# BGI-Qingdao/HAST

Hardware: AMD Instinct MI355X
Metric: classified read-bp/sec at k=21, 150bp reads, 200M unique-mers/hap (higher is better)
Workload: dtype u64; 1 GPU; C3 human-trio scale: 200M+200M synthetic 21-mers, 10M barcodes, 150bp reads; k=21, read_len=150, keys_per_hap=200000000, barcodes=10000000, batch_reads=48000000, reads_total=5760000000, minimizer=16, keys=random, collective=none (D2H of counters in timed region), resident_batches=12

## Files before the change

hast_amd/csrc/hast_api.cpp:

```cpp
#include <dlfcn.h>
#include <fcntl.h>
#include <sys/stat.h>
#include <unistd.h>
#include <hip/hip_runtime.h>

#include <algorithm>
#include <chrono>
#include <atomic>
#include <cstdarg>
#include <cstdio>
#include <cstdlib>
#include <cstring>
#include <functional>
#include <map>
#include <mutex>
#include <new>
#include <string>
#include <vector>

#include "../../include/hast.h"
#include "hast_common.h"
#include "hast_device.h"
#include "kc_device.h"
#include "fq_device.h"
#include "hast_internal.h"
#include "worker_pool.h"

using namespace hast;

namespace {

thread_local char g_err[512] = "";

struct Staging {
    uint8_t *h_bases = nullptr, *d_bases = nullptr;
    uint64_t *h_off = nullptr, *d_off = nullptr;
    uint32_t *h_ids = nullptr, *d_ids = nullptr;
    size_t cap_bases = 0, cap_reads = 0;
    hipEvent_t done = nullptr;
    bool in_flight = false;
};

}

struct hast_ctx {
    int device = 0;
    int k = 0;
    int m = 0;
    int n_cu = 256;
    hipStream_t stream = nullptr;
    uint64_t *d_slots = nullptr;
    uint32_t nbuckets = 0;
    unsigned long long *d_counts = nullptr;
    uint32_t *h_errword = nullptr;
    unsigned long long *d_pack = nullptr;
    size_t pack_words = 0;
    size_t n_barcodes = 0;
    bool counts_owned = false;
    uint32_t *d_err = nullptr;
    unsigned long long *d_cnt = nullptr;
    void *d_scratch = nullptr;
    size_t scratch_bytes = 0;
    Staging stage[2];
    unsigned batch_no = 0;
    void *d_seg = nullptr;
    size_t seg_bytes = 0;
    std::vector<hipEvent_t> t_ev;
    size_t t_slots = 0, t_next = 0, t_count = 0;
    uint32_t *d_votes_scratch = nullptr;
    size_t votes_bytes = 0;
    void *d_part = nullptr;
    size_t part_bytes = 0;
    char *sf_h[2] = {nullptr, nullptr}, *sf_d[2] = {nullptr, nullptr};
    hipEvent_t sf_done[2] = {nullptr, nullptr};
    void *d_filter = nullptr;
    size_t filter_bytes = 0;
    FilterGeom fg{};
    bool filter_valid = false;
    bool use_filter = true;
    size_t filter_fallback_bytes = 0;
    bool test_filter_oom = false;
    int filter_m = 0, filter_t = 0, filter_kp = 0;
    int filter_exact = -1;
    int text_acgt_only = 0;
    bool exact_env_off = false;
    bool exact_env_once = false;
    int commit_mode = 0;
    int kernel_geo = 1, kernel_rl = 1;
    size_t tile_lds = 0;
    bool part_oom = false;
};

namespace {

TableGeom geom(const hast_ctx *c) { return TableGeom{c->nbuckets, c->k, c->m, c->k == 32}; }
size_t table_slots(const hast_ctx *c) { return (size_t)c->nbuckets * kSlotsPerBucket * (c->k == 32 ? 2 : 1); }

int default_minimizer_plain(int k) { return k <= 16 ? k : std::max(16, k - 8); }
int default_minimizer(int k) {
    if (const char *e = getenv("HAST_MINIMIZER")) {
        int v = atoi(e);
        if (v >= 1 && v <= k) return v;
    }
    return default_minimizer_plain(k);
}

hast_status use(hast_ctx *c) {
    if (!c) return set_error(HAST_ERR_INVALID, "null context");
    HAST_HIP_TRY(hipSetDevice(c->device));
    return HAST_OK;
}

hast_status ensure_scratch(hast_ctx *c, size_t bytes) {
    if (c->scratch_bytes >= bytes) return HAST_OK;
    if (c->d_scratch) HAST_HIP_TRY(hipFree(c->d_scratch));
    c->d_scratch = nullptr;
    c->scratch_bytes = 0;
    HAST_HIP_TRY(dev_malloc(&c->d_scratch, bytes));
    c->scratch_bytes = bytes;
    return HAST_OK;
}

constexpr size_t kChunkBytes = 64u << 20;

hast_status check_err_word(hast_ctx *c, hipStream_t s) {
    uint32_t e = 0;
    HAST_HIP_TRY(hipMemcpyAsync(&e, c->d_err, sizeof(e), hipMemcpyDeviceToHost, s));
    HAST_HIP_TRY(hipStreamSynchronize(s));
    if (e) HAST_HIP_TRY(hipMemsetAsync(c->d_err, 0, sizeof(uint32_t), s));
    if (e & 2) return set_error(HAST_ERR_FORMAT, "k-mer text: a line is not exactly K=%d bytes", c->k);
    if (e & 4) return set_error(HAST_ERR_FORMAT, "k-mer text: a byte other than upper-case A/C/G/T");
    if (e & 1) return set_error(HAST_ERR_TABLE_FULL, "k-mer table full: reserve more keys");
    return HAST_OK;
}

hast_status check_classify_err(hast_ctx *c, hipStream_t hs) {
    if (!hs) hs = c->stream;
    *c->h_errword = 0;
    HAST_HIP_TRY(hipMemcpyAsync(c->h_errword, c->d_err + 1, sizeof(uint32_t), hipMemcpyDeviceToHost, hs));
    HAST_HIP_TRY(hipStreamSynchronize(hs));
    if (!*c->h_errword) return HAST_OK;
    HAST_HIP_TRY(hipMemsetAsync(c->d_err + 1, 0, sizeof(uint32_t), hs));
    HAST_HIP_TRY(hipStreamSynchronize(hs));
    return set_error(HAST_ERR_INVALID, "read offsets overlap or are not monotonic (their lengths add up to more than bases_bytes): rows were dropped");
}

SynthParams resolve(const hast_synth_params *p) {
    SynthParams r;
    r.seed_k = p->seed_k ? p->seed_k : 0x4841535401ull;
    r.seed_r = p->seed_r ? p->seed_r : 0x4841535402ull;
    r.seed_b = p->seed_b ? p->seed_b : 0x4841535403ull;
    r.n_keys_per_hap = p->n_keys_per_hap;
    r.n_barcodes = p->n_barcodes ? p->n_barcodes : 1;
    r.read_len = p->read_len;
    r.k = p->k;
    r.reserved = p->reserved;
    return r;
}

hast_status check_synth(const hast_synth_params *p) {
    if (!p) return set_error(HAST_ERR_INVALID, "null synth params");
    if (p->k < 1 || p->k > 32) return set_error(HAST_ERR_INVALID, "synth k=%u out of [1,32]", p->k);
    return HAST_OK;
}

}

namespace hast {
hast_status set_error(hast_status st, const char *fmt, ...) {
    va_list ap;
    va_start(ap, fmt);
    vsnprintf(g_err, sizeof(g_err), fmt, ap);
    va_end(ap);
    return st;
}
namespace {
struct Parked {
    std::mutex mu;
    std::vector<void *> device, pinned;
    size_t bytes = 0;
};
Parked &parked() {
    static Parked *p = new Parked();
    return *p;
}
size_t park_limit() {
    static const size_t limit = [] {
        const char *e = getenv("HAST_PARK_GB");
        return (size_t)((e ? atof(e) : 32.0) * 1073741824.0);
    }();
    return limit;
}
int park_sites() {
    static const int sites = [] {
        const char *e = getenv("HAST_PARK_SITES");
        return e ? atoi(e) : -1;
    }();
    return sites;
}
}
size_t parked_bytes() {
    Parked &pk = parked();
    std::lock_guard<std::mutex> lk(pk.mu);
    return pk.bytes;
}
hipError_t dev_malloc(void **p, size_t bytes) {
    hipError_t e = hipMalloc(p, bytes);
    if (e == hipErrorOutOfMemory && parked_bytes()) {
        (void)hipGetLastError();
        release_parked();
        e = hipMalloc(p, bytes);
    }
    return e;
}
hipError_t pinned_malloc(void **p, size_t bytes, unsigned flags) {
    hipError_t e = hipHostMalloc(p, bytes, flags);
    if (e == hipErrorOutOfMemory && parked_bytes()) {
        (void)hipGetLastError();
        release_parked();
        e = hipHostMalloc(p, bytes, flags);
    }
    return e;
}
void release_parked() {
    std::vector<void *> d, h;
    {
        Parked &pk = parked();
        std::lock_guard<std::mutex> lk(pk.mu);
        d.swap(pk.device);
        h.swap(pk.pinned);
        pk.bytes = 0;
    }
    for (void *p : d) (void)hipFree(p);
    for (void *p : h) (void)hipHostFree(p);
}
static void park(void *p, size_t bytes, bool pinned, int site) {
    if (!p) return;
    size_t limit = park_limit();
    if (!((park_sites() >> site) & 1)) limit = 0;
    if (limit == 0) {
        (void)(pinned ? hipHostFree(p) : hipFree(p));
        return;
    }
    bool over = false;
    {
        Parked &pk = parked();
        std::lock_guard<std::mutex> lk(pk.mu);
        (pinned ? pk.pinned : pk.device).push_back(p);
        pk.bytes += bytes;
        over = pk.bytes > limit;
    }
    if (over) release_parked();
}
void park_device(void *p, size_t bytes, int site) { park(p, bytes, false, site); }
void park_pinned(void *p, size_t bytes, int site) { park(p, bytes, true, site); }
int default_minimizer_for(int k) { return default_minimizer(k); }
}

extern "C" {

const char *hast_version(void) { return "hast-mi355x 0.1 (gfx950)"; }
const char *hast_last_error(void) { return g_err; }


hast_status hast_ctx_create(int device, int k, hast_ctx **out) {
    if (!out) return set_error(HAST_ERR_INVALID, "out is null");
    *out = nullptr;
    if (k < 1 || k > 32) return set_error(HAST_ERR_INVALID, "K=%d out of [1,32]", k);
    const bool trace = getenv("HAST_TRACE_INIT") != nullptr;
    auto now_s = [] { return std::chrono::duration<double>(std::chrono::steady_clock::now().time_since_epoch()).count(); };
    double t_tr = now_s();
    auto tr = [&](const char *what) {
        if (trace) fprintf(stderr, "__trace_init__ device %d: %s %.4f s\n", device, what, now_s() - t_tr);
        t_tr = now_s();
    };
    int n = 0;
    hipError_t e = hipGetDeviceCount(&n);
    tr("hipGetDeviceCount (loads the runtime)");
    if (e != hipSuccess || n <= 0)
        return set_error(HAST_ERR_NO_DEVICE, "no HIP device (%s); libhast has no CPU path", hipGetErrorString(e));
    if (device < 0 || device >= n) return set_error(HAST_ERR_NO_DEVICE, "device %d not in [0,%d)", device, n);
    HAST_HIP_TRY(hipSetDevice(device));
    tr("hipSetDevice");
    hast_ctx *c = new (std::nothrow) hast_ctx();
    if (!c) return set_error(HAST_ERR_OOM, "host allocation failed");
    c->device = device;
    c->k = k;
    c->m = default_minimizer(k);
    if (const char *e = getenv("HAST_CLASSIFY")) c->use_filter = strcmp(e, "exact") != 0;
    if (const char *e = getenv("HAST_TEST_FILTER_OOM")) c->test_filter_oom = atoi(e) != 0;
    if (const char *e = getenv("HAST_FILTER_M")) c->filter_m = atoi(e);
    if (const char *e = getenv("HAST_FILTER_T")) c->filter_t = atoi(e);
    if (const char *e = getenv("HAST_FILTER_KP")) c->filter_kp = atoi(e);
    if (const char *e = getenv("HAST_FILTER_EXACT")) {
        if (!strcmp(e, "once")) c->exact_env_once = true;
        else c->exact_env_off = atoi(e) == 0;
    }
    if (c->exact_env_off) c->filter_exact = 0;
    else if (c->exact_env_once) c->filter_exact = 1;
    if (const char *e = getenv("HAST_COMMIT")) c->commit_mode = !strcmp(e, "atomic") ? 1 : !strcmp(e, "partition") ? 2 : 0;
    if (const char *e = getenv("HAST_F_GEO")) c->kernel_geo = e[0] != '0';
    if (const char *e = getenv("HAST_F_RL")) c->kernel_rl = e[0] != '0';
    if (const char *e = getenv("HAST_TILE_LDS")) {
        const long v = atol(e);
        if (v >= 4096 && v <= 160 * 1024) c->tile_lds = (size_t)v;
    }
    hipDeviceProp_t prop;
    if (hipGetDeviceProperties(&prop, device) == hipSuccess) c->n_cu = prop.multiProcessorCount;
    tr("hipGetDeviceProperties");
    hast_status st = HAST_OK;
    auto bail = [&](hipError_t he, const char *what) {
        if (he != hipSuccess && st == HAST_OK) st = set_error(HAST_ERR_HIP, "%s: %s", what, hipGetErrorString(he));
    };
    bail(hipStreamCreateWithFlags(&c->stream, hipStreamNonBlocking), "hipStreamCreate");
    tr("hipStreamCreate");
    bail(dev_malloc(&c->d_err, 4 * sizeof(uint32_t)), "dev_malloc(err)");
    tr("first hipMalloc");
    bail(dev_malloc(&c->d_cnt, 8 * sizeof(unsigned long long)), "dev_malloc(cnt)");
    bail(pinned_malloc(reinterpret_cast<void **>(&c->h_errword), 64, hipHostMallocDefault), "pinned_malloc(err word)");
    if (st == HAST_OK) bail(hipMemsetAsync(c->d_err, 0, 4 * sizeof(uint32_t), c->stream), "hipMemset");
    if (st == HAST_OK) bail(hipStreamSynchronize(c->stream), "hipStreamSynchronize");
    tr("first fill + synchronize");
    for (auto &s : c->stage)
        if (st == HAST_OK) bail(hipEventCreateWithFlags(&s.done, hipEventDisableTiming), "hipEventCreate");
    tr("events");
    if (st != HAST_OK) {
        hast_ctx_destroy(c);
        return st;
    }
    *out = c;
    return HAST_OK;
}

void hast_release_parked(void) { release_parked(); }

void hast_ctx_destroy(hast_ctx *c) {
    if (!c) return;
    (void)hipSetDevice(c->device);
    if (c->stream) (void)hipStreamSynchronize(c->stream);
    release_parked();
    for (auto &s : c->stage) {
        if (s.h_bases) (void)hipHostFree(s.h_bases);
        if (s.h_off) (void)hipHostFree(s.h_off);
        if (s.h_ids) (void)hipHostFree(s.h_ids);
        if (s.d_bases) (void)hipFree(s.d_bases);
        if (s.d_off) (void)hipFree(s.d_off);
        if (s.d_ids) (void)hipFree(s.d_ids);
        if (s.done) (void)hipEventDestroy(s.done);
    }
    if (c->d_slots) (void)hipFree(c->d_slots);
    if (c->counts_owned && c->d_counts) (void)hipFree(c->d_counts);
    if (c->d_pack) (void)hipFree(c->d_pack);
    if (c->h_errword) (void)hipHostFree(c->h_errword);
    if (c->d_err) (void)hipFree(c->d_err);
    if (c->d_cnt) (void)hipFree(c->d_cnt);
    if (c->d_scratch) (void)hipFree(c->d_scratch);
    if (c->d_seg) (void)hipFree(c->d_seg);
    if (c->d_votes_scratch) (void)hipFree(c->d_votes_scratch);
    if (c->d_part) (void)hipFree(c->d_part);
    for (int i = 0; i < 2; ++i) {
        if (c->sf_done[i]) (void)hipEventDestroy(c->sf_done[i]);
        if (c->sf_d[i]) (void)hipFree(c->sf_d[i]);
        if (c->sf_h[i]) (void)hipHostFree(c->sf_h[i]);
    }
    if (c->d_filter) (void)hipFree(c->d_filter);
    for (hipEvent_t e : c->t_ev) (void)hipEventDestroy(e);
    if (c->stream) (void)hipStreamDestroy(c->stream);
    delete c;
}

int hast_ctx_k(const hast_ctx *c) { return c ? c->k : 0; }
int hast_ctx_minimizer(const hast_ctx *c) { return c ? c->m : 0; }

hast_status hast_ctx_set_minimizer(hast_ctx *c, int m) {
    if (!c) return set_error(HAST_ERR_INVALID, "null context");
    if (m < 1 || m > c->k) return set_error(HAST_ERR_INVALID, "minimizer length %d out of [1,%d]", m, c->k);
    if (c->d_slots) return set_error(HAST_ERR_INVALID, "minimizer length is fixed once the table exists");
    c->m = m;
    return HAST_OK;
}
int hast_ctx_device(const hast_ctx *c) { return c ? c->device : -1; }
hast_stream hast_ctx_stream(const hast_ctx *c) { return c ? (hast_stream)c->stream : nullptr; }

hast_status hast_stream_sync(hast_ctx *c, hast_stream s) {
    if (hast_status st = use(c)) return st;
    HAST_HIP_TRY(hipStreamSynchronize(s ? (hipStream_t)s : c->stream));
    return check_classify_err(c, s ? (hipStream_t)s : c->stream);
}

hast_status hast_dev_alloc(hast_ctx *c, size_t bytes, void **d_out) {
    if (hast_status st = use(c)) return st;
    if (!d_out) return set_error(HAST_ERR_INVALID, "d_out is null");
    HAST_HIP_TRY(dev_malloc(d_out, bytes ? bytes : 1));
    return HAST_OK;
}
hast_status hast_dev_free(hast_ctx *c, void *p) {
    if (hast_status st = use(c)) return st;
    if (p) HAST_HIP_TRY(hipFree(p));
    return HAST_OK;
}
hast_status hast_dev_mem_info(hast_ctx *c, size_t *free_bytes, size_t *total_bytes, size_t *parked) {
    if (hast_status st = use(c)) return st;
    size_t f = 0, t = 0;
    HAST_HIP_TRY(hipMemGetInfo(&f, &t));
    if (free_bytes) *free_bytes = f;
    if (total_bytes) *total_bytes = t;
    if (parked) *parked = parked_bytes();
    return HAST_OK;
}
hast_status hast_memcpy_h2d(hast_ctx *c, void *d, const void *s, size_t n) {
    if (hast_status st = use(c)) return st;
    if (n) HAST_HIP_TRY(hipMemcpy(d, s, n, hipMemcpyHostToDevice));
    return HAST_OK;
}
hast_status hast_memcpy_d2h(hast_ctx *c, void *d, const void *s, size_t n) {
    if (hast_status st = use(c)) return st;
    HAST_HIP_TRY(hipStreamSynchronize(c->stream));
    if (n) HAST_HIP_TRY(hipMemcpy(d, s, n, hipMemcpyDeviceToHost));
    return HAST_OK;
}
hast_status hast_memset_d(hast_ctx *c, void *d, int byte, size_t n, hast_stream s) {
    if (hast_status st = use(c)) return st;
    if (n) HAST_HIP_TRY(hipMemsetAsync(d, byte, n, s ? (hipStream_t)s : c->stream));
    return HAST_OK;
}

hast_status hast_table_reserve(hast_ctx *c, uint64_t max_keys, double lf) {
    if (hast_status st = use(c)) return st;
    if (lf <= 0) lf = 0.2;
    if (lf > 0.9) return set_error(HAST_ERR_INVALID, "load factor %.3f > 0.9", lf);
    double want = (double)(max_keys ? max_keys : 1) / lf / kSlotsPerBucket;
    uint64_t nb = (uint64_t)want + 1;
    if (nb < 64) nb = 64;
    nb += nb & 1;
    if (nb >= (1ull << 32)) return set_error(HAST_ERR_INVALID, "table of %llu buckets exceeds 2^32", (unsigned long long)nb);
    HAST_HIP_TRY(hipStreamSynchronize(c->stream));
    if (c->d_slots) HAST_HIP_TRY(hipFree(c->d_slots));
    c->d_slots = nullptr;
    c->nbuckets = 0;
    c->filter_valid = false;
    size_t bytes = (size_t)nb * kSlotsPerBucket * sizeof(uint64_t) * (c->k == 32 ? 2 : 1);
    HAST_HIP_TRY(dev_malloc(&c->d_slots, bytes));
    HAST_HIP_TRY(hipMemsetAsync(c->d_slots, 0xFF, bytes, c->stream));
    HAST_HIP_TRY(hipStreamSynchronize(c->stream));
    c->nbuckets = (uint32_t)nb;
    return HAST_OK;
}

static hast_status ensure_filter(hast_ctx *c, hipStream_t hs);
static void table_changed(hast_ctx *c) { c->filter_valid = false; }

static hast_status need_table(hast_ctx *c, int hap) {
    if (hast_status st = use(c)) return st;
    if (!c->d_slots) return set_error(HAST_ERR_INVALID, "call hast_table_reserve first");
    if (hap != 0 && hap != 1) return set_error(HAST_ERR_INVALID, "hap must be 0 or 1");
    return HAST_OK;
}

hast_status hast_ctx_set_text_check(hast_ctx *c, int acgt_only) {
    if (!c) return set_error(HAST_ERR_INVALID, "null context");
    c->text_acgt_only = acgt_only ? 1 : 0;
    return HAST_OK;
}

hast_status hast_table_insert_keys_device(hast_ctx *c, int hap, const uint64_t *d_keys, size_t n, hast_stream s) {
    if (hast_status st = need_table(c, hap)) return st;
    hipStream_t hs = s ? (hipStream_t)s : c->stream;
    table_changed(c);
    HAST_HIP_TRY(launch_insert_keys(c->d_slots, geom(c), d_keys, n, (uint32_t)hap, c->d_err, hs));
    return check_err_word(c, hs);
}

hast_status hast_table_insert_keys(hast_ctx *c, int hap, const uint64_t *keys, size_t n) {
    if (hast_status st = need_table(c, hap)) return st;
    if (n && !keys) return set_error(HAST_ERR_INVALID, "keys is null");
    table_changed(c);
    const size_t per = kChunkBytes / sizeof(uint64_t);
    if (hast_status st = ensure_scratch(c, std::min(n, per) * sizeof(uint64_t) + 16)) return st;
    for (size_t i = 0; i < n; i += per) {
        size_t m = std::min(per, n - i);
        HAST_HIP_TRY(hipMemcpyAsync(c->d_scratch, keys + i, m * sizeof(uint64_t), hipMemcpyHostToDevice, c->stream));
        HAST_HIP_TRY(launch_insert_keys(c->d_slots, geom(c), (const uint64_t *)c->d_scratch, m, (uint32_t)hap, c->d_err, c->stream));
        HAST_HIP_TRY(hipStreamSynchronize(c->stream));
    }
    return check_err_word(c, c->stream);
}

hast_status hast_table_insert_text(hast_ctx *c, int hap, const char *text, size_t nbytes, uint64_t *lines_out) {
    if (hast_status st = need_table(c, hap)) return st;
    if (lines_out) *lines_out = 0;
    if (nbytes && !text) return set_error(HAST_ERR_INVALID, "text is null");
    table_changed(c);
    const size_t stride = (size_t)c->k + 1;
    size_t n_lines = nbytes / stride;
    size_t rem = nbytes - n_lines * stride;
    if (rem && memchr(text + n_lines * stride, '\n', rem)) return set_error(HAST_ERR_FORMAT, "k-mer text: ragged last line");
    const size_t per = (kChunkBytes / stride);
    if (hast_status st = ensure_scratch(c, std::min(n_lines, per) * stride + 16)) return st;
    for (size_t i = 0; i < n_lines; i += per) {
        size_t m = std::min(per, n_lines - i);
        HAST_HIP_TRY(hipMemcpyAsync(c->d_scratch, text + i * stride, m * stride, hipMemcpyHostToDevice, c->stream));
        HAST_HIP_TRY(launch_insert_text(c->d_slots, geom(c), (const char *)c->d_scratch, m, (uint32_t)hap, c->text_acgt_only, c->d_err, c->stream));
        HAST_HIP_TRY(hipStreamSynchronize(c->stream));
    }
    if (hast_status st = check_err_word(c, c->stream)) return st;
    if (lines_out) *lines_out = n_lines;
    return HAST_OK;
}

static hast_status stream_file_region(hast_ctx *c, int fd, const char *path, uint64_t file_off, uint64_t n_units, size_t unit,
                                      const std::function<hipError_t(char *, size_t, uint64_t)> &use) {
    constexpr size_t kPieceBytes = 16u << 20;
    const uint64_t per = std::max<uint64_t>(1, kPieceBytes / unit);
    char **h_buf = c->sf_h, **d_buf = c->sf_d;
    hipEvent_t *done = c->sf_done;
    hipError_t e = hipSuccess;
    bool short_read = false;
    for (int i = 0; i < 2 && e == hipSuccess; ++i) {
        if (!h_buf[i]) e = pinned_malloc((void **)&h_buf[i], kPieceBytes, hipHostMallocDefault);
        if (e == hipSuccess && !d_buf[i]) e = dev_malloc((void **)&d_buf[i], kPieceBytes + 16);
        if (e == hipSuccess && !done[i]) e = hipEventCreateWithFlags(&done[i], hipEventDisableTiming);
    }
    if (e == hipSuccess) {
        const int nthreads = 8;
        WorkerPool pool(nthreads);
        size_t i = 0;
        for (uint64_t first = 0; first < n_units && e == hipSuccess; first += per, ++i) {
            const int b = (int)(i & 1);
            const size_t m = (size_t)std::min<uint64_t>(per, n_units - first), bytes = m * unit;
            if (i >= 2) e = hipEventSynchronize(done[b]);
            if (e != hipSuccess) break;
            const size_t share = ((bytes / nthreads) + 4095) & ~(size_t)4095;
            std::atomic<bool> bad{false};
            pool.run([&](int t) {
                const size_t from = std::min(bytes, share * (size_t)t), to = std::min(bytes, from + share);
                size_t got = 0;
                while (from + got < to) {
                    const ssize_t r = pread(fd, h_buf[b] + from + got, to - from - got, (off_t)(file_off + first * unit + from + got));
                    if (r <= 0) { bad = true; break; }
                    got += (size_t)r;
                }
            });
            if (bad) { short_read = true; break; }
            e = hipMemcpyAsync(d_buf[b], h_buf[b], bytes, hipMemcpyHostToDevice, c->stream);
            if (e == hipSuccess) e = use(d_buf[b], m, first);
            if (e == hipSuccess) e = hipEventRecord(done[b], c->stream);
        }
        const hipError_t e2 = hipStreamSynchronize(c->stream);
        if (e == hipSuccess) e = e2;
    }
    if (e != hipSuccess) return set_error(HAST_ERR_HIP, "%s: %s", path, hipGetErrorString(e));
    if (short_read) return set_error(HAST_ERR_IO, "%s is shorter than its size says (truncated, or changed while it was read)", path);
    return HAST_OK;
}

hast_status hast_table_insert_text_file(hast_ctx *c, int hap, const char *path, uint64_t *lines_out) {
    if (hast_status st = need_table(c, hap)) return st;
    if (lines_out) *lines_out = 0;
    if (!path) return set_error(HAST_ERR_INVALID, "path is null");
    const int fd = open(path, O_RDONLY);
    if (fd < 0) return set_error(HAST_ERR_IO, "cannot read %s", path);
    struct stat sb;
    if (fstat(fd, &sb) != 0 || !S_ISREG(sb.st_mode)) {
        close(fd);
        return set_error(HAST_ERR_IO, "%s is not a regular file", path);
    }
    const size_t nbytes = (size_t)sb.st_size, stride = (size_t)c->k + 1;
    const size_t n_lines = nbytes / stride, rem = nbytes - n_lines * stride;
    if (rem) {
        char tail[64];
        if (pread(fd, tail, rem, (off_t)(n_lines * stride)) != (ssize_t)rem) { close(fd); return set_error(HAST_ERR_IO, "cannot read %s", path); }
        if (memchr(tail, '\n', rem)) { close(fd); return set_error(HAST_ERR_FORMAT, "k-mer text: ragged last line"); }
    }
    table_changed(c);
    const hast_status st = stream_file_region(c, fd, path, 0, n_lines, stride, [&](char *d_piece, size_t m, uint64_t) {
        return launch_insert_text(c->d_slots, geom(c), d_piece, m, (uint32_t)hap, c->text_acgt_only, c->d_err, c->stream);
    });
    close(fd);
    if (st != HAST_OK) return st;
    if (hast_status s2 = check_err_word(c, c->stream)) return s2;
    if (lines_out) *lines_out = n_lines;
    return HAST_OK;
}

hast_status hast_table_erase(hast_ctx *c, const uint64_t *keys, size_t n, uint8_t *out_hit) {
    if (hast_status st = need_table(c, 0)) return st;
    if (n == 0) return HAST_OK;
    if (!keys) return set_error(HAST_ERR_INVALID, "keys is null");
    size_t kb = n * sizeof(uint64_t);
    if (hast_status st = ensure_scratch(c, kb + n + 16)) return st;
    uint8_t *d_hit = (uint8_t *)c->d_scratch + kb;
    HAST_HIP_TRY(hipMemcpyAsync(c->d_scratch, keys, kb, hipMemcpyHostToDevice, c->stream));
    HAST_HIP_TRY(launch_erase_keys(c->d_slots, geom(c), (const uint64_t *)c->d_scratch, n, d_hit, c->stream));
    table_changed(c);
    std::vector<uint8_t> hit(n);
    HAST_HIP_TRY(hipMemcpyAsync(hit.data(), d_hit, n, hipMemcpyDeviceToHost, c->stream));
    HAST_HIP_TRY(hipStreamSynchronize(c->stream));
    if (out_hit) memcpy(out_hit, hit.data(), n);
    return HAST_OK;
}

hast_status hast_table_lookup(hast_ctx *c, const uint64_t *keys, size_t n, uint8_t *out_tags) {
    if (hast_status st = need_table(c, 0)) return st;
    if (n == 0) return HAST_OK;
    if (!keys || !out_tags) return set_error(HAST_ERR_INVALID, "null argument");
    size_t kb = n * sizeof(uint64_t);
    if (hast_status st = ensure_scratch(c, kb + n + 16)) return st;
    uint8_t *d_tags = (uint8_t *)c->d_scratch + kb;
    HAST_HIP_TRY(hipMemcpyAsync(c->d_scratch, keys, kb, hipMemcpyHostToDevice, c->stream));
    HAST_HIP_TRY(launch_lookup_keys(c->d_slots, geom(c), (const uint64_t *)c->d_scratch, n, d_tags, c->stream));
    HAST_HIP_TRY(hipMemcpyAsync(out_tags, d_tags, n, hipMemcpyDeviceToHost, c->stream));
    HAST_HIP_TRY(hipStreamSynchronize(c->stream));
    return HAST_OK;
}

hast_status hast_table_sizes(hast_ctx *c, uint64_t *n0, uint64_t *n1) {
    if (hast_status st = need_table(c, 0)) return st;
    unsigned long long h[2] = {0, 0};
    HAST_HIP_TRY(hipMemsetAsync(c->d_cnt, 0, sizeof(h), c->stream));
    HAST_HIP_TRY(launch_count_tags(c->d_slots, geom(c), c->d_cnt, c->stream));
    HAST_HIP_TRY(hipMemcpyAsync(h, c->d_cnt, sizeof(h), hipMemcpyDeviceToHost, c->stream));
    HAST_HIP_TRY(hipStreamSynchronize(c->stream));
    if (n0) *n0 = h[0];
    if (n1) *n1 = h[1];
    return HAST_OK;
}

namespace {
struct CacheHeader {
    char magic[8];
    uint32_t version, k;
    uint64_t n_slots;
    uint64_t reserved;
};
}

hast_status hast_table_save(hast_ctx *c, const char *path) {
    if (hast_status st = need_table(c, 0)) return st;
    if (c->k == 32) return set_error(HAST_ERR_INVALID, "the key-set cache stores tag bits next to the key: not available for K=32");
    if (!path) return set_error(HAST_ERR_INVALID, "path is null");
    uint64_t n0 = 0, n1 = 0;
    if (hast_status st = hast_table_sizes(c, &n0, &n1)) return st;
    const size_t cap = (size_t)(n0 + n1) + 16;
    uint64_t *d_out = nullptr;
    HAST_HIP_TRY(dev_malloc((void **)&d_out, cap * sizeof(uint64_t)));
    unsigned long long n = 0;
    hipError_t e = hipMemsetAsync(c->d_cnt, 0, sizeof(unsigned long long), c->stream);
    if (e == hipSuccess) e = launch_export_slots(c->d_slots, (size_t)c->nbuckets * kSlotsPerBucket, d_out, cap, c->d_cnt, c->stream);
    if (e == hipSuccess) e = hipMemcpyAsync(&n, c->d_cnt, sizeof(n), hipMemcpyDeviceToHost, c->stream);
    if (e == hipSuccess) e = hipStreamSynchronize(c->stream);
    std::vector<uint64_t> host;
    if (e == hipSuccess && n <= cap) {
        uint64_t *d_sorted = nullptr;
        void *d_tmp = nullptr;
        size_t tmp_bytes = 0;
        if (n) e = kc_sort_keys(nullptr, &tmp_bytes, (unsigned long long *)d_out, nullptr, (size_t)n, 32, c->stream);
        if (e == hipSuccess && n) e = dev_malloc((void **)&d_sorted, (size_t)n * sizeof(uint64_t));
        if (e == hipSuccess && n) e = dev_malloc(&d_tmp, tmp_bytes ? tmp_bytes : 16);
        if (e == hipSuccess && n) e = kc_sort_keys(d_tmp, &tmp_bytes, (unsigned long long *)d_out, (unsigned long long *)d_sorted, (size_t)n, 32, c->stream);
        if (e == hipSuccess) e = hipStreamSynchronize(c->stream);
        host.resize((size_t)n);
        if (e == hipSuccess && n) e = hipMemcpy(host.data(), d_sorted, (size_t)n * sizeof(uint64_t), hipMemcpyDeviceToHost);
        (void)hipFree(d_sorted);
        (void)hipFree(d_tmp);
    }
    (void)hipFree(d_out);
    if (e != hipSuccess) return set_error(HAST_ERR_HIP, "table export: %s", hipGetErrorString(e));
    if (n > cap) return set_error(HAST_ERR_INVALID, "table export overflow");
    FILE *f = fopen(path, "wb");
    if (!f) return set_error(HAST_ERR_IO, "cannot write %s", path);
    CacheHeader h;
    memcpy(h.magic, "HASTKEYS", 8);
    h.version = 1;
    h.k = (uint32_t)c->k;
    h.n_slots = n;
    h.reserved = 0;
    bool ok = fwrite(&h, sizeof(h), 1, f) == 1 && (n == 0 || fwrite(host.data(), sizeof(uint64_t), (size_t)n, f) == (size_t)n);
    ok = (fclose(f) == 0) && ok;
    if (!ok) return set_error(HAST_ERR_IO, "short write to %s", path);
    return HAST_OK;
}

hast_status hast_table_file_info(const char *path, int *k_out, uint64_t *n_keys_out) {
    if (!path) return set_error(HAST_ERR_INVALID, "path is null");
    FILE *f = fopen(path, "rb");
    if (!f) return set_error(HAST_ERR_IO, "cannot read %s", path);
    CacheHeader h;
    const bool ok = fread(&h, sizeof(h), 1, f) == 1 && memcmp(h.magic, "HASTKEYS", 8) == 0 && h.version == 1;
    fclose(f);
    if (!ok) return set_error(HAST_ERR_FORMAT, "%s is not a HASTKEYS v1 file", path);
    if (k_out) *k_out = (int)h.k;
    if (n_keys_out) *n_keys_out = h.n_slots;
    return HAST_OK;
}

hast_status hast_table_load(hast_ctx *c, const char *path, double load_factor) {
    if (hast_status st = use(c)) return st;
    if (!path) return set_error(HAST_ERR_INVALID, "path is null");
    FILE *f = fopen(path, "rb");
    if (!f) return set_error(HAST_ERR_IO, "cannot read %s", path);
    CacheHeader h;
    if (fread(&h, sizeof(h), 1, f) != 1 || memcmp(h.magic, "HASTKEYS", 8) != 0 || h.version != 1) {
        fclose(f);
        return set_error(HAST_ERR_FORMAT, "%s is not a HASTKEYS v1 file", path);
    }
    if (h.k == 32 || (int)h.k != c->k) {
        fclose(f);
        return set_error(HAST_ERR_INVALID, "%s holds %u-mers, the context is K=%d", path, h.k, c->k);
    }
    hast_status st = hast_table_reserve(c, h.n_slots + 1, load_factor);
    struct stat sb;
    if (st == HAST_OK && fstat(fileno(f), &sb) == 0 && S_ISREG(sb.st_mode)) {
        st = stream_file_region(c, fileno(f), path, sizeof(CacheHeader), h.n_slots, sizeof(uint64_t), [&](char *d_piece, size_t m, uint64_t) {
            return launch_import_slots(c->d_slots, geom(c), (const uint64_t *)d_piece, m, c->d_err, c->stream);
        });
        if (st == HAST_ERR_IO) st = set_error(HAST_ERR_IO, "%s is truncated", path);
    } else {
        const size_t per = kChunkBytes / sizeof(uint64_t);
        std::vector<uint64_t> buf(std::min<uint64_t>(per, h.n_slots ? h.n_slots : 1));
        if (st == HAST_OK) st = ensure_scratch(c, buf.size() * sizeof(uint64_t) + 16);
        for (uint64_t i = 0; st == HAST_OK && i < h.n_slots; i += per) {
            const size_t m = (size_t)std::min<uint64_t>(per, h.n_slots - i);
            if (fread(buf.data(), sizeof(uint64_t), m, f) != m) { st = set_error(HAST_ERR_IO, "%s is truncated", path); break; }
            hipError_t e = hipMemcpyAsync(c->d_scratch, buf.data(), m * sizeof(uint64_t), hipMemcpyHostToDevice, c->stream);
            if (e == hipSuccess) e = launch_import_slots(c->d_slots, geom(c), (const uint64_t *)c->d_scratch, m, c->d_err, c->stream);
            if (e == hipSuccess) e = hipStreamSynchronize(c->stream);
            if (e != hipSuccess) st = set_error(HAST_ERR_HIP, "table import: %s", hipGetErrorString(e));
        }
    }
    fclose(f);
    if (st != HAST_OK) return st;
    return check_err_word(c, c->stream);
}

hast_status hast_table_clone(hast_ctx *dst, hast_ctx *src) {
    if (!dst || !src || dst == src) return set_error(HAST_ERR_INVALID, "clone needs two different contexts");
    if (dst->k != src->k) return set_error(HAST_ERR_INVALID, "clone: K differs (%d vs %d)", dst->k, src->k);
    if (hast_status st = need_table(src, 0)) return st;
    if (src->use_filter)
        if (hast_status st = ensure_filter(src, src->stream)) return st;
    HAST_HIP_TRY(hipStreamSynchronize(src->stream));
    if (hast_status st = use(dst)) return st;
    HAST_HIP_TRY(hipStreamSynchronize(dst->stream));
    if (dst->d_slots) HAST_HIP_TRY(hipFree(dst->d_slots));
    dst->d_slots = nullptr;
    dst->nbuckets = 0;
    dst->filter_valid = false;
    dst->m = src->m;
    const size_t bytes = table_slots(src) * sizeof(uint64_t);
    HAST_HIP_TRY(dev_malloc(&dst->d_slots, bytes));
    HAST_HIP_TRY(hipMemcpyPeerAsync(dst->d_slots, dst->device, src->d_slots, src->device, bytes, dst->stream));
    dst->nbuckets = src->nbuckets;
    if (src->filter_valid && dst->use_filter) {
        if (dst->filter_bytes != src->filter_bytes) {
            if (dst->d_filter) HAST_HIP_TRY(hipFree(dst->d_filter));
            dst->d_filter = nullptr;
            dst->filter_bytes = 0;
            if (dst->test_filter_oom || dev_malloc(&dst->d_filter, src->filter_bytes) != hipSuccess) {
                (void)hipGetLastError();
                dst->d_filter = nullptr;
                dst->use_filter = false;
                dst->filter_fallback_bytes = src->filter_bytes;
                HAST_HIP_TRY(hipStreamSynchronize(dst->stream));
                return HAST_OK;
            }
            dst->filter_bytes = src->filter_bytes;
        }
        HAST_HIP_TRY(hipMemcpyPeerAsync(dst->d_filter, dst->device, src->d_filter, src->device, src->filter_bytes, dst->stream));
        dst->fg = src->fg;
        dst->filter_m = src->filter_m;
        dst->filter_exact = src->filter_exact;
        dst->filter_t = src->filter_t;
        dst->filter_kp = src->filter_kp;
        dst->filter_valid = true;
    }
    HAST_HIP_TRY(hipStreamSynchronize(dst->stream));
    return HAST_OK;
}

hast_status hast_table_info(const hast_ctx *c, uint64_t *n_buckets, uint64_t *bytes) {
    if (!c) return set_error(HAST_ERR_INVALID, "null context");
    if (n_buckets) *n_buckets = c->nbuckets;
    if (bytes) *bytes = (uint64_t)table_slots(c) * sizeof(uint64_t);
    return HAST_OK;
}

hast_status hast_counts_resize(hast_ctx *c, size_t n) {
    if (hast_status st = use(c)) return st;
    HAST_HIP_TRY(hipStreamSynchronize(c->stream));
    if (c->counts_owned && c->d_counts) HAST_HIP_TRY(hipFree(c->d_counts));
    c->d_counts = nullptr;
    c->n_barcodes = 0;
    c->counts_owned = false;
    size_t bytes = (n ? n : 1) * 4 * sizeof(unsigned long long);
    HAST_HIP_TRY(dev_malloc(reinterpret_cast<void **>(&c->d_counts), bytes));
    c->counts_owned = true;
    c->n_barcodes = n;
    HAST_HIP_TRY(hipMemsetAsync(c->d_counts, 0, bytes, c->stream));
    HAST_HIP_TRY(hipStreamSynchronize(c->stream));
    return HAST_OK;
}

hast_status hast_counts_permute(hast_ctx *c, const uint32_t *perm, size_t n_perm, size_t n_new) {
    if (hast_status st = use(c)) return st;
    if (!c->d_counts || !c->counts_owned) return set_error(HAST_ERR_INVALID, "hast_counts_permute: library-owned counters only (hast_counts_resize)");
    if (n_perm > c->n_barcodes || (n_perm && !perm)) return set_error(HAST_ERR_INVALID, "hast_counts_permute: %zu ids > %zu counters", n_perm, c->n_barcodes);
    for (size_t i = 0; i < n_perm; i++)
        if (perm[i] >= n_new && perm[i] != 0xFFFFFFFFu) return set_error(HAST_ERR_INVALID, "hast_counts_permute: perm[%zu] = %u is outside the %zu new records", i, perm[i], n_new);
    HAST_HIP_TRY(hipStreamSynchronize(c->stream));
    unsigned long long *d_new = nullptr;
    uint32_t *d_perm = nullptr;
    const size_t bytes = (n_new ? n_new : 1) * 4 * sizeof(unsigned long long);
    HAST_HIP_TRY(dev_malloc(reinterpret_cast<void **>(&d_new), bytes));
    hipError_t e = dev_malloc(reinterpret_cast<void **>(&d_perm), (n_perm ? n_perm : 1) * sizeof(uint32_t));
    if (e == hipSuccess) e = hipMemsetAsync(d_new, 0, bytes, c->stream);
    if (e == hipSuccess && n_perm) e = hipMemcpyAsync(d_perm, perm, n_perm * sizeof(uint32_t), hipMemcpyHostToDevice, c->stream);
    if (e == hipSuccess) e = launch_counts_permute(d_new, c->d_counts, d_perm, n_perm, c->n_barcodes, n_new, c->stream);
    if (e == hipSuccess) e = hipStreamSynchronize(c->stream);
    if (d_perm) (void)hipFree(d_perm);
    if (e != hipSuccess) {
        (void)hipFree(d_new);
        return set_error(e == hipErrorOutOfMemory ? HAST_ERR_OOM : HAST_ERR_HIP, "hast_counts_permute: %s", hipGetErrorString(e));
    }
    HAST_HIP_TRY(hipFree(c->d_counts));
    c->d_counts = d_new;
    c->n_barcodes = n_new;
    return HAST_OK;
}

hast_status hast_counts_bind(hast_ctx *c, uint64_t *d_counts, size_t n) {
    if (hast_status st = use(c)) return st;
    if (!d_counts) return set_error(HAST_ERR_INVALID, "d_counts is null");
    if ((uintptr_t)d_counts & 31) return set_error(HAST_ERR_INVALID, "d_counts must be 32-byte aligned (one record = 4 x u64)");
    HAST_HIP_TRY(hipStreamSynchronize(c->stream));
    if (c->counts_owned && c->d_counts) HAST_HIP_TRY(hipFree(c->d_counts));
    c->d_counts = reinterpret_cast<unsigned long long *>(d_counts);
    c->counts_owned = false;
    c->n_barcodes = n;
    return HAST_OK;
}

hast_status hast_counts_zero(hast_ctx *c, hast_stream s) {
    if (hast_status st = use(c)) return st;
    if (!c->d_counts) return set_error(HAST_ERR_INVALID, "no counters: call hast_counts_resize/bind");
    HAST_HIP_TRY(hipMemsetAsync(c->d_counts, 0, c->n_barcodes * 4 * sizeof(unsigned long long), s ? (hipStream_t)s : c->stream));
    return HAST_OK;
}

static hast_status ensure_pack(hast_ctx *c, size_t n) {
    if (c->pack_words >= 3 * n) return HAST_OK;
    if (c->d_pack) HAST_HIP_TRY(hipFree(c->d_pack));
    c->d_pack = nullptr;
    c->pack_words = 0;
    HAST_HIP_TRY(dev_malloc((void **)&c->d_pack, std::max<size_t>(3 * n, 1) * sizeof(unsigned long long)));
    c->pack_words = 3 * n;
    return HAST_OK;
}

hast_status hast_counts_pack(hast_ctx *c, uint64_t *d_packed, size_t n, hast_stream s) {
    if (hast_status st = use(c)) return st;
    if (!c->d_counts || !d_packed) return set_error(HAST_ERR_INVALID, "no counters");
    if (n > c->n_barcodes) return set_error(HAST_ERR_INVALID, "n_barcodes %zu > %zu", n, c->n_barcodes);
    HAST_HIP_TRY(launch_counts_pack(c->d_counts, reinterpret_cast<unsigned long long *>(d_packed), n, s ? (hipStream_t)s : c->stream));
    return HAST_OK;
}
hast_status hast_counts_unpack(hast_ctx *c, const uint64_t *d_packed, size_t n, hast_stream s) {
    if (hast_status st = use(c)) return st;
    if (!c->d_counts || !d_packed) return set_error(HAST_ERR_INVALID, "no counters");
    if (n > c->n_barcodes) return set_error(HAST_ERR_INVALID, "n_barcodes %zu > %zu", n, c->n_barcodes);
    HAST_HIP_TRY(launch_counts_unpack(c->d_counts, reinterpret_cast<const unsigned long long *>(d_packed), n, s ? (hipStream_t)s : c->stream));
    return HAST_OK;
}

hast_status hast_counts_read_range(hast_ctx *c, size_t first, size_t n, uint64_t *c0, uint64_t *c1, uint64_t *neg) {
    if (hast_status st = use(c)) return st;
    if (!c->d_counts) return set_error(HAST_ERR_INVALID, "no counters");
    if (first > c->n_barcodes || n > c->n_barcodes - first) return set_error(HAST_ERR_INVALID, "records [%zu, %zu) of %zu counters", first, first + n, c->n_barcodes);
    HAST_HIP_TRY(hipStreamSynchronize(c->stream));
    if (hast_status st = check_classify_err(c, c->stream)) return st;
    if (!n) return HAST_OK;
    if (hast_status st = ensure_pack(c, n)) return st;
    HAST_HIP_TRY(launch_counts_pack(c->d_counts + 4 * first, c->d_pack, n, c->stream));
    uint64_t *dst[3] = {c0, c1, neg};
    for (int a = 0; a < 3; a++)
        if (dst[a]) HAST_HIP_TRY(hipMemcpyAsync(dst[a], c->d_pack + (size_t)a * n, n * sizeof(uint64_t), hipMemcpyDeviceToHost, c->stream));
    HAST_HIP_TRY(hipStreamSynchronize(c->stream));
    return HAST_OK;
}
hast_status hast_counts_read(hast_ctx *c, uint64_t *c0, uint64_t *c1, uint64_t *neg, size_t n) { return hast_counts_read_range(c, 0, n, c0, c1, neg); }

hast_status hast_counts_allreduce(hast_ctx *const *ctxs, int n) {
    if (!ctxs || n < 1) return set_error(HAST_ERR_INVALID, "no contexts");
    for (int i = 0; i < n; i++)
        if (!ctxs[i] || !ctxs[i]->d_counts || ctxs[i]->n_barcodes != ctxs[0]->n_barcodes) return set_error(HAST_ERR_INVALID, "contexts need equal-size counters");
    const size_t nbc = ctxs[0]->n_barcodes, nw = nbc * 4;
    std::vector<hast_ctx *> lead;
    std::vector<std::vector<hast_ctx *>> members;
    for (int i = 0; i < n; i++) {
        size_t l = 0;
        while (l < lead.size() && lead[l]->device != ctxs[i]->device) ++l;
        if (l == lead.size()) {
            lead.push_back(ctxs[i]);
            members.emplace_back();
        } else {
            for (hast_ctx *m : members[l]) if (m == ctxs[i]) return set_error(HAST_ERR_INVALID, "hast_counts_allreduce: a context is named twice");
            if (lead[l] == ctxs[i]) return set_error(HAST_ERR_INVALID, "hast_counts_allreduce: a context is named twice");
            members[l].push_back(ctxs[i]);
        }
    }
    for (size_t l = 0; l < lead.size(); l++) {
        if (members[l].empty()) continue;
        if (hast_status st = use(lead[l])) return st;
        HAST_HIP_TRY(hipStreamSynchronize(lead[l]->stream));
        for (hast_ctx *m : members[l]) HAST_HIP_TRY(hipStreamSynchronize(m->stream));
        for (hast_ctx *m : members[l]) HAST_HIP_TRY(launch_add_u64(lead[l]->d_counts, m->d_counts, nw, lead[l]->stream));
    }
    auto hand_back = [&]() -> hast_status {
        for (size_t l = 0; l < lead.size(); l++) {
            if (members[l].empty()) continue;
            if (hast_status st = use(lead[l])) return st;
            for (hast_ctx *m : members[l])
                HAST_HIP_TRY(hipMemcpyAsync(m->d_counts, lead[l]->d_counts, nw * sizeof(unsigned long long), hipMemcpyDeviceToDevice, lead[l]->stream));
            HAST_HIP_TRY(hipStreamSynchronize(lead[l]->stream));
        }
        return HAST_OK;
    };
    const int nl = (int)lead.size();
    if (nl == 1 && !getenv("HAST_FORCE_RCCL")) return hand_back();
    typedef void *comm_t;
    typedef int (*init_all_t)(comm_t *, int, const int *);
    typedef int (*allreduce_t)(const void *, void *, size_t, int, int, comm_t, hipStream_t);
    typedef int (*group_t)(void);
    typedef int (*destroy_t)(comm_t);
    static void *lib = nullptr;
    if (!lib) lib = dlopen("librccl.so.1", RTLD_NOW | RTLD_GLOBAL);
    if (!lib) lib = dlopen("librccl.so", RTLD_NOW | RTLD_GLOBAL);
    if (!lib) return set_error(HAST_ERR_RCCL, "cannot load librccl: %s", dlerror());
    auto init_all = (init_all_t)dlsym(lib, "ncclCommInitAll");
    auto allreduce = (allreduce_t)dlsym(lib, "ncclAllReduce");
    auto gstart = (group_t)dlsym(lib, "ncclGroupStart");
    auto gend = (group_t)dlsym(lib, "ncclGroupEnd");
    auto destroy = (destroy_t)dlsym(lib, "ncclCommDestroy");
    if (!init_all || !allreduce || !gstart || !gend || !destroy) return set_error(HAST_ERR_RCCL, "librccl lacks symbols");
    std::vector<int> devs(nl);
    for (int i = 0; i < nl; i++) devs[i] = lead[(size_t)i]->device;
    static std::mutex comm_mu;
    static std::map<std::vector<int>, std::vector<comm_t>> comm_cache;
    std::lock_guard<std::mutex> lock(comm_mu);
    auto it = comm_cache.find(devs);
    if (it == comm_cache.end()) {
        std::vector<comm_t> fresh(nl);
        if (int rc = init_all(fresh.data(), nl, devs.data())) return set_error(HAST_ERR_RCCL, "ncclCommInitAll failed (%d)", rc);
        it = comm_cache.emplace(devs, std::move(fresh)).first;
    }
    const std::vector<comm_t> &comms = it->second;
    const int kUint64 = 5, kSum = 0;
    for (int i = 0; i < nl; i++) {
        hast_ctx *c = lead[(size_t)i];
        if (hast_status st = use(c)) return st;
        if (hast_status st = ensure_pack(c, nbc)) return st;
        HAST_HIP_TRY(launch_counts_pack(c->d_counts, c->d_pack, nbc, c->stream));
    }
    int rc = gstart();
    for (int i = 0; i < nl && !rc; i++) {
        hast_ctx *c = lead[(size_t)i];
        (void)hipSetDevice(c->device);
        rc = allreduce(c->d_pack, c->d_pack, nbc * 3, kUint64, kSum, comms[(size_t)i], c->stream);
    }
    int rc2 = gend();
    for (int i = 0; i < nl; i++) {
        hast_ctx *c = lead[(size_t)i];
        (void)hipSetDevice(c->device);
        if (!rc && !rc2 && launch_counts_unpack(c->d_counts, c->d_pack, nbc, c->stream) != hipSuccess) rc2 = -1;
        (void)hipStreamSynchronize(c->stream);
    }
    if (rc || rc2) {
        for (auto cm : comms) destroy(cm);
        comm_cache.erase(it);
    }
    if (rc || rc2) return set_error(HAST_ERR_RCCL, "ncclAllReduce failed (%d/%d)", rc, rc2);
    return hand_back();
}

static hast_status ensure_filter(hast_ctx *c, hipStream_t hs) {
    if (c->filter_valid) return HAST_OK;
    unsigned long long h[2] = {0, 0};
    HAST_HIP_TRY(hipMemsetAsync(c->d_cnt, 0, sizeof(h), hs));
    HAST_HIP_TRY(launch_count_tags(c->d_slots, geom(c), c->d_cnt, hs));
    HAST_HIP_TRY(hipMemcpyAsync(h, c->d_cnt, sizeof(h), hipMemcpyDeviceToHost, hs));
    HAST_HIP_TRY(hipStreamSynchronize(hs));
    FilterGeom fg = filter_geom_for(c->k, h[0] + h[1], c->filter_m, c->filter_t, c->filter_kp, c->k == 32 ? 0 : c->filter_exact);
    size_t bytes = (size_t)filter_nblocks(fg) * 128;
    if (bytes != c->filter_bytes) {
        if (c->d_filter) HAST_HIP_TRY(hipFree(c->d_filter));
        c->d_filter = nullptr;
        c->filter_bytes = 0;
        hipError_t got = c->test_filter_oom ? hipErrorOutOfMemory : dev_malloc(&c->d_filter, bytes);
        if (got != hipSuccess && !c->filter_m && fg.m == kFilterMaxM) {
            (void)hipGetLastError();
            fg = filter_geom_for(c->k, h[0] + h[1], kFilterMaxM - 1, c->filter_t, c->filter_kp, c->k == 32 ? 0 : c->filter_exact);
            bytes = (size_t)filter_nblocks(fg) * 128;
            got = dev_malloc(&c->d_filter, bytes);
        }
        if (got != hipSuccess) {
            (void)hipGetLastError();
            c->d_filter = nullptr;
            c->use_filter = false;
            c->filter_fallback_bytes = bytes;
            return HAST_OK;
        }
        c->filter_bytes = bytes;
    }
    HAST_HIP_TRY(hipMemsetAsync(c->d_filter, 0, bytes, hs));
    HAST_HIP_TRY(launch_filter_build(c->d_slots, geom(c), c->d_filter, fg, hs));
    c->fg = fg;
    c->filter_valid = true;
    return HAST_OK;
}

static constexpr uint32_t kSegWindows = 482;
static constexpr uint32_t kLongRead = 4096;

static hast_status commit_votes(hast_ctx *c, const uint32_t *d_votes, const uint32_t *d_ids, size_t n_reads, uint32_t max_votes,
                                bool atomic_only, hipStream_t hs) {
    const int mode = c->commit_mode;
    if (mode != 1 && !atomic_only && !c->part_oom && commit_partition_usable(n_reads, c->n_barcodes, max_votes, mode == 2)) {
        const size_t need = commit_partition_scratch_bytes(n_reads, c->n_barcodes, nullptr, nullptr);
        if (c->part_bytes < need) {
            HAST_HIP_TRY(hipStreamSynchronize(hs));
            if (c->d_part) HAST_HIP_TRY(hipFree(c->d_part));
            c->d_part = nullptr;
            c->part_bytes = 0;
            if (dev_malloc(&c->d_part, need + need / 8) == hipSuccess) c->part_bytes = need + need / 8;
            else {
                (void)hipGetLastError();
                c->d_part = nullptr;
                c->part_oom = true;
            }
        }
        if (c->d_part) {
            HAST_HIP_TRY(launch_commit_partitioned(d_votes, d_ids, c->d_counts, c->n_barcodes, n_reads, c->d_part, hs));
            return HAST_OK;
        }
    }
    HAST_HIP_TRY(launch_commit_votes(d_votes, d_ids, c->d_counts, nullptr, n_reads, hs));
    return HAST_OK;
}

static hast_status classify_rows(hast_ctx *c, const uint8_t *d_bases, size_t bases_bytes, const uint64_t *d_offsets,
                                 const uint32_t *d_lens, const uint32_t *d_seg_read, int strict, uint32_t read_len,
                                 const uint32_t *d_barcode_ids, uint32_t *d_votes, size_t n_reads, hast_stream s,
                                 const unsigned long long *d_n_rows = nullptr) {
    if (hast_status st = need_table(c, 0)) return st;
    if (n_reads == 0) return HAST_OK;
    if (!d_bases) return set_error(HAST_ERR_INVALID, "d_bases is null");
    if (d_barcode_ids && !c->d_counts) return set_error(HAST_ERR_INVALID, "barcode ids given but no counters bound");
    if (read_len == 0 || read_len > (1u << 24)) return set_error(HAST_ERR_INVALID, "read_len %u out of range", read_len);
    if (read_len > kLongRead && c->use_filter) return set_error(HAST_ERR_INVALID, "internal: a row of %u bases reached the filter kernel", read_len);
    if (!d_offsets && (uint64_t)n_reads * read_len > bases_bytes)
        return set_error(HAST_ERR_INVALID, "bases_bytes too small for %zu reads of %u", n_reads, read_len);
    ClassifyArgs a;
    a.bases = d_bases;
    a.bases_bytes = bases_bytes;
    a.offsets = d_offsets;
    a.lens = d_lens;
    a.seg_read = d_seg_read;
    a.strict = strict;
    if (reinterpret_cast<uintptr_t>(d_votes) & 7) return set_error(HAST_ERR_INVALID, "d_votes must be 8-byte aligned (a row is stored as one 64-bit word)");
    uint32_t *votes_buf = d_votes;
    if (d_barcode_ids && !votes_buf) {
        const size_t need = n_reads * 2 * sizeof(uint32_t);
        if (c->votes_bytes < need) {
            HAST_HIP_TRY(hipStreamSynchronize(s ? (hipStream_t)s : c->stream));
            if (c->d_votes_scratch) HAST_HIP_TRY(hipFree(c->d_votes_scratch));
            c->d_votes_scratch = nullptr;
            c->votes_bytes = 0;
            HAST_HIP_TRY(dev_malloc(reinterpret_cast<void **>(&c->d_votes_scratch), need + need / 8));
            c->votes_bytes = need + need / 8;
        }
        votes_buf = c->d_votes_scratch;
    }
    a.votes = votes_buf;
    a.slots = c->d_slots;
    a.n_reads = n_reads;
    a.n_rows_ptr = d_n_rows;
    a.nbuckets = c->nbuckets;
    a.read_len = read_len;
    a.k = c->k;
    a.wide = c->k == 32;
    a.m = c->m;
    a.max_pos = read_len >= (uint32_t)c->k ? read_len - c->k + 1 : 0;
    a.mh_stride = read_len >= (uint32_t)c->m ? read_len - c->m + 1 : 0;
    a.w64 = (read_len + 31) / 32;
    hipStream_t hs = s ? (hipStream_t)s : c->stream;
    if (c->use_filter)
        if (hast_status st = ensure_filter(c, hs)) return st;
    const bool filt = c->use_filter;
    size_t per_read, pad;
    if (filt) {
        a.filter = c->d_filter;
        a.fg = c->fg;
        a.l1_stride = c->fg.dense ? 0 : ((read_len >= (uint32_t)c->fg.t ? read_len - (uint32_t)c->fg.t + 1 : 0) + 1 + 3) & ~3u;
        per_read = (size_t)(a.w64 + 1) * 8 + 8 + 8 + 4 + 4 + (size_t)a.l1_stride * 4 + (strict ? (size_t)(2 * a.w64 + 1) * 4 : 0);
        pad = 16 + classify_f_queue_bytes() + 64 * 4 + 64;
    } else {
        const uint32_t wlen = (uint32_t)(c->k - c->m + 1);
        a.filter = nullptr;
        a.fg = FilterGeom{};
        a.l1_stride = 0;
        per_read = (size_t)(a.w64 + 1) * 8 + 8 + 8 + 4 + 4 + (size_t)a.mh_stride * 4 + (strict ? (size_t)(2 * a.w64 + 1) * 4 : 0);
        pad = (size_t)wlen * 4 + 64 + 64 + 16;
    }
    const size_t lds_budget = c->tile_lds ? c->tile_lds : (filt ? (size_t)32000 - (size_t)kTmerLevelTableWords * 4 : (size_t)19968);
    const uint32_t tr_max = (uint32_t)std::min<size_t>(64, std::max<size_t>(1, lds_budget > pad + per_read ? (lds_budget - pad) / per_read : 1));
    uint32_t tr = tr_max;
    if (a.max_pos > 0) {
        double best = -1;
        for (uint32_t t = tr_max; t >= 1 && t + 8 > tr_max; --t) {
            const uint64_t q = (uint64_t)t * a.max_pos, blocks = (q + 63) / 64, slots = filt ? (blocks + 3) / 4 * 4 : (blocks + 7) / 8 * 8;
            const double eff = (double)q / (double)(slots * 64);
            if (eff > best + 1e-9) { best = eff; tr = t; }
        }
    }
    a.tile_reads = tr;
    const size_t smem = per_read * tr + pad;
    if (smem + (filt ? (size_t)kTmerLevelTableWords * 4 : 0) > (160u << 10)) return set_error(HAST_ERR_INVALID, "read_len %u needs %zu B of LDS", read_len, smem);
    auto magic = [](uint64_t qmax, uint32_t d) -> uint32_t {
        if (d <= 1 || qmax * d >= (1ull << 32)) return 0;
        return (uint32_t)((1ull << 32) / d) + 1;
    };
    a.div_magic = magic((uint64_t)tr * a.max_pos + 1024, a.max_pos);
    a.div_mh = magic((uint64_t)tr * a.mh_stride + 1024, a.mh_stride);
    a.div_hw = magic((uint64_t)tr * a.w64 * 2 + 1024, a.w64 * 2);
    a.div_l1g = magic((uint64_t)tr * (a.l1_stride / 4) + 1024, a.l1_stride / 4);
    const uint64_t n_tiles = (n_reads + tr - 1) / tr;
    const int grid = (int)std::min<uint64_t>(n_tiles, (uint64_t)c->n_cu * 8);
    a.tile_queue = c->d_cnt + 3;
    HAST_HIP_TRY(hipMemsetAsync(a.tile_queue, 0, sizeof(unsigned long long), hs));
    hipEvent_t *ev = c->t_slots ? &c->t_ev[3 * (c->t_next % c->t_slots)] : nullptr;
    if (ev) HAST_HIP_TRY(hipEventRecord(ev[0], hs));
    HAST_HIP_TRY(filt ? launch_classify_f(a, grid, smem, (c->kernel_geo ? 1 : 0) | (c->kernel_rl ? 2 : 0), hs) : launch_classify(a, grid, smem, hs));
    if (ev) HAST_HIP_TRY(hipEventRecord(ev[1], hs));
    if (d_barcode_ids) {
        if (hast_status st = commit_votes(c, votes_buf, d_barcode_ids, n_reads, a.max_pos, d_seg_read != nullptr, hs)) return st;
    }
    if (ev) {
        HAST_HIP_TRY(hipEventRecord(ev[2], hs));
        c->t_next++;
        c->t_count = std::min(c->t_count + 1, c->t_slots);
    }
    return HAST_OK;
}

static hast_status classify_segmented(hast_ctx *c, const uint8_t *d_bases, size_t bases_bytes, const uint64_t *d_offsets, const uint32_t *d_lens,
                                      uint32_t fixed_len, size_t n_reads, int strict, const uint32_t *d_barcode_ids, uint32_t *d_votes_out,
                                      hipStream_t hs);

hast_status hast_ctx_set_filter(hast_ctx *c, int enable, int m, int t, int kp) {
    if (!c) return set_error(HAST_ERR_INVALID, "null context");
    if (m < 0 || m > c->k || m > kFilterMaxM) return set_error(HAST_ERR_INVALID, "filter m=%d out of [0,%d]", m, std::min(c->k, kFilterMaxM));
    if (t < 0 || (m && t > m)) return set_error(HAST_ERR_INVALID, "filter t=%d out of [0,m]", t);
    if (kp < 0 || kp > c->k || (kp && m && (kp < m || kp - m >= 32))) return set_error(HAST_ERR_INVALID, "filter kp=%d out of [m,K]", kp);
    c->use_filter = enable != 0;
    c->filter_fallback_bytes = 0;
    c->filter_exact = (enable == 2 || c->exact_env_off) ? 0 : (c->exact_env_once || c->filter_exact == 1) ? 1 : -1;
    c->filter_m = m;
    c->filter_t = t;
    c->filter_kp = kp;
    c->filter_valid = false;
    return HAST_OK;
}

hast_status hast_ctx_set_option(hast_ctx *c, const char *name, long value) {
    if (!c || !name) return set_error(HAST_ERR_INVALID, "null argument");
    if (!strcmp(name, "commit")) {
        if (value < 0 || value > 2) return set_error(HAST_ERR_INVALID, "commit: 0 = by batch size, 1 = atomic, 2 = partitioned");
        c->commit_mode = (int)value;
    } else if (!strcmp(name, "kernel_geo")) c->kernel_geo = value != 0;
    else if (!strcmp(name, "kernel_rl")) c->kernel_rl = value != 0;
    else if (!strcmp(name, "tile_lds")) {
        if (value && (value < 4096 || value > 160 * 1024)) return set_error(HAST_ERR_INVALID, "tile_lds %ld out of [4096, 163840]", value);
        c->tile_lds = (size_t)value;
    } else if (!strcmp(name, "filter_exact_once")) {
        if (c->filter_exact != 0) c->filter_exact = value ? 1 : (c->exact_env_once ? 1 : -1);
        c->filter_valid = false;
    } else return set_error(HAST_ERR_INVALID, "unknown option %s", name);
    return HAST_OK;
}
hast_status hast_ctx_options(const hast_ctx *c, char *out, size_t cap) {
    if (!c || !out || !cap) return set_error(HAST_ERR_INVALID, "null argument");
    std::string s;
    auto add = [&](const char *n, long v) { s += (s.empty() ? "" : " "); s += n; s += "=" + std::to_string(v); };
    if (!c->use_filter) add("filter", 0);
    if (c->filter_fallback_bytes) add("filter_fallback_table_only_no_room_for_bytes", (long)c->filter_fallback_bytes);
    if (c->filter_exact == 0) add("filter_exact", 0);
    if (c->filter_exact == 1) add("filter_exact_once", 1);
    if (c->filter_m) add("filter_m", c->filter_m);
    if (c->filter_t) add("filter_t", c->filter_t);
    if (c->filter_kp) add("filter_kp", c->filter_kp);
    if (c->commit_mode) add("commit", c->commit_mode);
    if (!c->kernel_geo) add("kernel_geo", 0);
    if (!c->kernel_rl) add("kernel_rl", 0);
    if (c->tile_lds) add("tile_lds", (long)c->tile_lds);
    if (c->m != default_minimizer_plain(c->k)) add("minimizer", c->m);
    snprintf(out, cap, "%s", s.c_str());
    return HAST_OK;
}

hast_status hast_filter_build(hast_ctx *c) {
    if (hast_status st = need_table(c, 0)) return st;
    if (!c->use_filter) return HAST_OK;
    if (hast_status st = ensure_filter(c, c->stream)) return st;
    HAST_HIP_TRY(hipStreamSynchronize(c->stream));
    return HAST_OK;
}

hast_status hast_filter_info(const hast_ctx *c, int *enabled, int *m, int *t, int *kp, uint64_t *bytes) {
    if (!c) return set_error(HAST_ERR_INVALID, "null context");
    if (enabled) *enabled = !c->use_filter ? 0 : (c->filter_valid && c->fg.exact) ? 2 : 1;
    if (m) *m = c->filter_valid ? c->fg.m : 0;
    if (t) *t = c->filter_valid ? c->fg.t : 0;
    if (kp) *kp = c->filter_valid ? c->fg.kp : 0;
    if (bytes) *bytes = c->filter_valid ? c->filter_bytes : 0;
    return HAST_OK;
}

hast_status hast_filter_dense(const hast_ctx *c, int *dense) {
    if (!c || !dense) return set_error(HAST_ERR_INVALID, "null argument");
    *dense = (c->use_filter && c->filter_valid && c->fg.dense) ? 1 : 0;
    return HAST_OK;
}

hast_status hast_filter_request_ceiling(hast_ctx *c, double *requests_per_s) {
    if (hast_status st = need_table(c, 0)) return st;
    if (!requests_per_s) return set_error(HAST_ERR_INVALID, "null argument");
    if (!c->use_filter) return set_error(HAST_ERR_INVALID, "the filter is off");
    if (hast_status st = ensure_filter(c, c->stream)) return st;
    if (!c->use_filter || !c->d_filter) return set_error(HAST_ERR_INVALID, "no filter (HBM too small for it)");
    const uint64_t nblocks = filter_nblocks(c->fg);
    const int grid = c->n_cu * 8;
    const uint32_t iters = 256;
    uint32_t *d_sink = reinterpret_cast<uint32_t *>(c->d_cnt + 2);
    hipEvent_t e0 = nullptr, e1 = nullptr;
    hipError_t e = hipEventCreate(&e0);
    if (e == hipSuccess) e = hipEventCreate(&e1);
    float best = 0;
    for (int rep = 0; rep < 3 && e == hipSuccess; ++rep) {
        e = hipEventRecord(e0, c->stream);
        if (e == hipSuccess) e = launch_request_ceiling(c->d_filter, nblocks, iters, grid, d_sink, c->stream);
        if (e == hipSuccess) e = hipEventRecord(e1, c->stream);
        if (e == hipSuccess) e = hipEventSynchronize(e1);
        float ms = 0;
        if (e == hipSuccess) e = hipEventElapsedTime(&ms, e0, e1);
        if (e == hipSuccess && rep && (best == 0 || ms < best)) best = ms;
    }
    if (e0) (void)hipEventDestroy(e0);
    if (e1) (void)hipEventDestroy(e1);
    if (e != hipSuccess) return set_error(HAST_ERR_HIP, "request ceiling: %s", hipGetErrorString(e));
    *requests_per_s = (double)grid * 32.0 * 4.0 * (double)iters / ((double)best * 1e-3);
    return HAST_OK;
}

hast_status hast_classify_timing(hast_ctx *c, int n_slots) {
    if (hast_status st = use(c)) return st;
    for (hipEvent_t e : c->t_ev) (void)hipEventDestroy(e);
    c->t_ev.clear();
    c->t_slots = c->t_next = c->t_count = 0;
    if (n_slots <= 0) return HAST_OK;
    c->t_ev.resize(3 * (size_t)n_slots);
    for (hipEvent_t &e : c->t_ev) HAST_HIP_TRY(hipEventCreate(&e));
    c->t_slots = (size_t)n_slots;
    return HAST_OK;
}
hast_status hast_classify_times(hast_ctx *c, float *classify_ms, float *commit_ms, int max, int *n_out) {
    if (hast_status st = use(c)) return st;
    if (!n_out || (max > 0 && (!classify_ms || !commit_ms))) return set_error(HAST_ERR_INVALID, "null argument");
    int n = 0;
    const size_t first = c->t_next - c->t_count;
    for (size_t i = 0; i < c->t_count && n < max; ++i, ++n) {
        hipEvent_t *ev = &c->t_ev[3 * ((first + i) % c->t_slots)];
        HAST_HIP_TRY(hipEventSynchronize(ev[2]));
        HAST_HIP_TRY(hipEventElapsedTime(&classify_ms[n], ev[0], ev[1]));
        HAST_HIP_TRY(hipEventElapsedTime(&commit_ms[n], ev[1], ev[2]));
    }
    *n_out = n;
    c->t_count = 0;
    return HAST_OK;
}

hast_status hast_classify_device(hast_ctx *c, const uint8_t *d_bases, size_t bases_bytes, const uint64_t *d_offsets,
                                 uint32_t read_len, const uint32_t *d_barcode_ids, uint32_t *d_votes, size_t n_reads,
                                 hast_stream s) {
    if (read_len > kLongRead && c && c->d_slots && n_reads) {
        if (d_barcode_ids && !c->d_counts) return set_error(HAST_ERR_INVALID, "barcode ids given but no counters bound");
        if (!d_bases) return set_error(HAST_ERR_INVALID, "d_bases is null");
        if (!d_offsets && (uint64_t)n_reads * read_len > bases_bytes)
            return set_error(HAST_ERR_INVALID, "bases_bytes too small for %zu reads of %u", n_reads, read_len);
        if (hast_status st = use(c)) return st;
        return classify_segmented(c, d_bases, bases_bytes, d_offsets, nullptr, read_len, n_reads, 0, d_barcode_ids, d_votes, s ? (hipStream_t)s : c->stream);
    }
    return classify_rows(c, d_bases, bases_bytes, d_offsets, nullptr, nullptr, 0, read_len, d_barcode_ids, d_votes, n_reads, s);
}

hast_status hast_counts_add_votes(hast_ctx *c, const uint32_t *d_votes, const uint32_t *d_barcode_ids, size_t n_reads, uint32_t max_votes,
                                  hast_stream s) {
    if (hast_status st = use(c)) return st;
    if (!c->d_counts) return set_error(HAST_ERR_INVALID, "no counters: call hast_counts_resize/bind");
    if (n_reads == 0) return HAST_OK;
    if (!d_votes || !d_barcode_ids) return set_error(HAST_ERR_INVALID, "null argument");
    if (reinterpret_cast<uintptr_t>(d_votes) & 7) return set_error(HAST_ERR_INVALID, "d_votes must be 8-byte aligned");
    return commit_votes(c, d_votes, d_barcode_ids, n_reads, max_votes, false, s ? (hipStream_t)s : c->stream);
}

static hast_status classify_segmented(hast_ctx *c, const uint8_t *d_bases, size_t bases_bytes, const uint64_t *d_offsets, const uint32_t *d_lens,
                                      uint32_t fixed_len, size_t n_reads, int strict, const uint32_t *d_barcode_ids, uint32_t *d_votes_out,
                                      hipStream_t hs) {
    const size_t max_seg = n_reads + bases_bytes / kSegWindows + 1;
    const size_t votes_b = ((n_reads * 2 * sizeof(uint32_t) + 255) & ~(size_t)255), flags_b = ((n_reads + 255) & ~(size_t)255);
    const size_t need = max_seg * (sizeof(uint64_t) + 2 * sizeof(uint32_t)) + votes_b + flags_b + 256;
    if (c->seg_bytes < need) {
        HAST_HIP_TRY(hipStreamSynchronize(hs));
        if (c->d_seg) HAST_HIP_TRY(hipFree(c->d_seg));
        c->d_seg = nullptr;
        c->seg_bytes = 0;
        HAST_HIP_TRY(dev_malloc(&c->d_seg, need + need / 4));
        c->seg_bytes = need + need / 4;
    }
    uint32_t *acc = (uint32_t *)c->d_seg;
    uint8_t *has_n = (uint8_t *)c->d_seg + votes_b;
    const size_t cap = (c->seg_bytes - votes_b - flags_b - 256) / (sizeof(uint64_t) + 2 * sizeof(uint32_t));
    uint64_t *seg_off = (uint64_t *)((uint8_t *)c->d_seg + votes_b + flags_b);
    uint32_t *seg_len = (uint32_t *)(seg_off + cap);
    uint32_t *seg_read = seg_len + cap;
    uint32_t *target = strict ? d_votes_out : acc;
    unsigned long long *d_nseg = c->d_cnt + 4;
    HAST_HIP_TRY(hipMemsetAsync(d_nseg, 0, sizeof(unsigned long long), hs));
    HAST_HIP_TRY(hipMemsetAsync(target, 0, n_reads * 2 * sizeof(uint32_t), hs));
    if (!strict) HAST_HIP_TRY(launch_scan_n(d_bases, d_offsets, d_lens, fixed_len, n_reads, has_n, hs));
    HAST_HIP_TRY(launch_build_segments(d_offsets, d_lens, fixed_len, n_reads, c->k, kSegWindows, seg_off, seg_len, seg_read, d_nseg,
                                  strict ? nullptr : has_n, (uint64_t)max_seg, (uint64_t)bases_bytes, c->d_err + 1, hs));
    if (max_seg > cap) return set_error(HAST_ERR_INVALID, "segment table too small (%zu > %zu)", max_seg, cap);
    if (hast_status st = classify_rows(c, d_bases, bases_bytes, seg_off, seg_len, seg_read, strict, kSegWindows + (uint32_t)c->k - 1,
                                       nullptr, target, max_seg, hs, d_nseg))
        return st;
    if (!strict) HAST_HIP_TRY(launch_commit_votes(acc, d_barcode_ids, c->d_counts, d_votes_out, n_reads, hs));
    return HAST_OK;
}

hast_status hast_classify_perread_device(hast_ctx *c, const uint8_t *d_bases, size_t bases_bytes, const uint64_t *d_offsets,
                                         size_t n_reads, uint32_t *d_votes, hast_stream s) {
    if (hast_status st = need_table(c, 0)) return st;
    if (n_reads == 0) return HAST_OK;
    if (!d_bases || !d_offsets || !d_votes) return set_error(HAST_ERR_INVALID, "null argument");
    return classify_segmented(c, d_bases, bases_bytes, d_offsets, nullptr, 0, n_reads, 1, nullptr, d_votes, s ? (hipStream_t)s : c->stream);
}

hast_status hast_classify_perread(hast_ctx *c, const uint8_t *bases, const uint64_t *offsets, size_t n_reads,
                                  uint32_t *votes_out) {
    if (hast_status st = need_table(c, 0)) return st;
    if (n_reads == 0) return HAST_OK;
    if (!bases || !offsets || !votes_out) return set_error(HAST_ERR_INVALID, "null argument");
    const size_t nbytes = offsets[n_reads] - offsets[0];
    const size_t ob = (n_reads + 1) * sizeof(uint64_t), vb = n_reads * 2 * sizeof(uint32_t);
    const size_t total = ((nbytes + 255) & ~(size_t)255) + ((ob + 255) & ~(size_t)255) + vb + 256;
    if (hast_status st = ensure_scratch(c, total)) return st;
    uint8_t *d_b = (uint8_t *)c->d_scratch;
    uint64_t *d_o = (uint64_t *)(d_b + ((nbytes + 255) & ~(size_t)255));
    uint32_t *d_v = (uint32_t *)((uint8_t *)d_o + ((ob + 255) & ~(size_t)255));
    std::vector<uint64_t> rel(n_reads + 1);
    for (size_t i = 0; i <= n_reads; i++) rel[i] = offsets[i] - offsets[0];
    if (nbytes) HAST_HIP_TRY(hipMemcpyAsync(d_b, bases + offsets[0], nbytes, hipMemcpyHostToDevice, c->stream));
    HAST_HIP_TRY(hipMemcpyAsync(d_o, rel.data(), ob, hipMemcpyHostToDevice, c->stream));
    HAST_HIP_TRY(hipStreamSynchronize(c->stream));
    if (hast_status st = hast_classify_perread_device(c, d_b, nbytes ? nbytes : 1, d_o, n_reads, d_v, c->stream)) return st;
    HAST_HIP_TRY(hipMemcpyAsync(votes_out, d_v, vb, hipMemcpyDeviceToHost, c->stream));
    HAST_HIP_TRY(hipStreamSynchronize(c->stream));
    return check_classify_err(c, c->stream);
}

static hast_status stage_reserve(hast_ctx *c, Staging &s, size_t nbytes, size_t nreads) {
    (void)c;
    if (s.cap_bases < nbytes) {
        if (s.h_bases) HAST_HIP_TRY(hipHostFree(s.h_bases));
        if (s.d_bases) HAST_HIP_TRY(hipFree(s.d_bases));
        s.h_bases = s.d_bases = nullptr;
        s.cap_bases = 0;
        size_t cap = nbytes + nbytes / 4 + 64;
        HAST_HIP_TRY(pinned_malloc((void **)&s.h_bases, cap, hipHostMallocDefault));
        HAST_HIP_TRY(dev_malloc((void **)&s.d_bases, cap));
        s.cap_bases = cap;
    }
    if (s.cap_reads < nreads) {
        if (s.h_off) HAST_HIP_TRY(hipHostFree(s.h_off));
        if (s.h_ids) HAST_HIP_TRY(hipHostFree(s.h_ids));
        if (s.d_off) HAST_HIP_TRY(hipFree(s.d_off));
        if (s.d_ids) HAST_HIP_TRY(hipFree(s.d_ids));
        s.h_off = s.d_off = nullptr;
        s.h_ids = s.d_ids = nullptr;
        s.cap_reads = 0;
        size_t cap = nreads + nreads / 4 + 16;
        HAST_HIP_TRY(pinned_malloc((void **)&s.h_off, (cap + 1) * sizeof(uint64_t), hipHostMallocDefault));
        HAST_HIP_TRY(pinned_malloc((void **)&s.h_ids, cap * sizeof(uint32_t), hipHostMallocDefault));
        HAST_HIP_TRY(dev_malloc((void **)&s.d_off, (cap + 1) * sizeof(uint64_t)));
        HAST_HIP_TRY(dev_malloc((void **)&s.d_ids, cap * sizeof(uint32_t)));
        s.cap_reads = cap;
    }
    return HAST_OK;
}

hast_status hast_batch_begin(hast_ctx *c, size_t bases_capacity, size_t reads_capacity, uint8_t **bases,
                             uint64_t **offsets, uint32_t **ids) {
    if (hast_status st = need_table(c, 0)) return st;
    if (!bases || !offsets || !ids) return set_error(HAST_ERR_INVALID, "null argument");
    if (!c->d_counts) return set_error(HAST_ERR_INVALID, "no counters bound");
    Staging &s = c->stage[c->batch_no & 1];
    if (s.in_flight) {
        HAST_HIP_TRY(hipEventSynchronize(s.done));
        s.in_flight = false;
    }
    if (hast_status st = stage_reserve(c, s, bases_capacity, reads_capacity)) return st;
    *bases = s.h_bases;
    *offsets = s.h_off;
    *ids = s.h_ids;
    return HAST_OK;
}

hast_status hast_batch_submit(hast_ctx *c, size_t n_reads, uint32_t max_read_len) {
    if (hast_status st = need_table(c, 0)) return st;
    Staging &s = c->stage[c->batch_no & 1];
    if (n_reads == 0) return HAST_OK;
    if (n_reads > s.cap_reads) return set_error(HAST_ERR_INVALID, "batch of %zu reads exceeds the staged capacity", n_reads);
    const size_t nbytes = s.h_off[n_reads];
    if (nbytes > s.cap_bases || s.h_off[0] != 0) return set_error(HAST_ERR_INVALID, "bad staged offsets");
    c->batch_no++;
    if (nbytes) HAST_HIP_TRY(hipMemcpyAsync(s.d_bases, s.h_bases, nbytes, hipMemcpyHostToDevice, c->stream));
    HAST_HIP_TRY(hipMemcpyAsync(s.d_off, s.h_off, (n_reads + 1) * sizeof(uint64_t), hipMemcpyHostToDevice, c->stream));
    HAST_HIP_TRY(hipMemcpyAsync(s.d_ids, s.h_ids, n_reads * sizeof(uint32_t), hipMemcpyHostToDevice, c->stream));
    hast_status st = hast_classify_device(c, s.d_bases, nbytes ? nbytes : 1, s.d_off, max_read_len ? max_read_len : 1, s.d_ids,
                                          nullptr, n_reads, c->stream);
    HAST_HIP_TRY(hipEventRecord(s.done, c->stream));
    s.in_flight = true;
    return st;
}

hast_status hast_classify_batch(hast_ctx *c, const uint8_t *bases, const uint64_t *offsets, const uint32_t *ids,
                                size_t n_reads, uint32_t max_read_len) {
    if (n_reads == 0) return c ? HAST_OK : set_error(HAST_ERR_INVALID, "null context");
    if (!bases || !offsets || !ids) return set_error(HAST_ERR_INVALID, "null argument");
    const size_t nbytes = offsets[n_reads] - offsets[0];
    uint8_t *hb;
    uint64_t *ho;
    uint32_t *hi;
    if (hast_status st = hast_batch_begin(c, nbytes, n_reads, &hb, &ho, &hi)) return st;
    memcpy(hb, bases + offsets[0], nbytes);
    const uint64_t o0 = offsets[0];
    for (size_t i = 0; i <= n_reads; i++) ho[i] = offsets[i] - o0;
    memcpy(hi, ids, n_reads * sizeof(uint32_t));
    return hast_batch_submit(c, n_reads, max_read_len);
}

}

namespace hast {
hast_status classify_framed(hast_ctx *c, const uint8_t *d_buf, size_t buf_bytes, const uint64_t *d_off, const uint32_t *d_len, uint32_t max_len,
                            uint32_t *d_votes, size_t n_reads, hipStream_t hs) {
    if (hast_status st = need_table(c, 0)) return st;
    if (n_reads == 0) return HAST_OK;
    if (max_len > kLongRead) return classify_segmented(c, d_buf, buf_bytes, d_off, d_len, 0, n_reads, 0, nullptr, d_votes, hs);
    return classify_rows(c, d_buf, buf_bytes, d_off, d_len, nullptr, 0, max_len ? max_len : 1, nullptr, d_votes, n_reads, hs);
}
hast_status commit_framed(hast_ctx *c, const uint32_t *d_votes, const uint32_t *d_ids, size_t n_reads, hipStream_t hs) {
    if (hast_status st = use(c)) return st;
    if (!c->d_counts) return set_error(HAST_ERR_INVALID, "no counters bound");
    HAST_HIP_TRY(launch_commit_votes(d_votes, d_ids, c->d_counts, nullptr, n_reads, hs));
    return HAST_OK;
}
hipStream_t ctx_stream_of(hast_ctx *c) { return c->stream; }
size_t ctx_n_barcodes(const hast_ctx *c) { return c->n_barcodes; }
}

extern "C" {

void hast_parse_barcode(const char *head, size_t len, size_t *start, size_t *n) {
    ptrdiff_t s = -1, e = -1;
    for (size_t i = 0; i < len; i++) {
        if (head[i] == '#') s = (ptrdiff_t)i;
        else if (head[i] == '/') e = (ptrdiff_t)i;
    }
    size_t pos = (size_t)(s + 1);
    size_t avail = len - pos;
    ptrdiff_t cnt = e - s - 1;
    *start = pos;
    *n = (cnt < 0 || (size_t)cnt > avail) ? avail : (size_t)cnt;
}

int hast_get_hap(const char *bc, size_t blen, uint64_t c0, uint64_t c1, uint64_t n0, uint64_t n1, double w0, double w1) {
    if ((blen == 5 && !memcmp(bc, "0_0_0", 5)) || (blen == 3 && !memcmp(bc, "0_0", 3)) || (blen == 1 && bc[0] == '0'))
        return -1;
    if (c0 > 0 && c1 > 0) {
        double df0 = double(c0) / double(n0);
        double df1 = double(c1) / double(n1);
        df0 *= w0;
        df1 *= w1;
        if (df0 > df1) return 0;
        if (df1 > df0) return 1;
        return -1;
    }
    if (c0 > 0) return 0;
    if (c1 > 0) return 1;
    return -1;
}

uint64_t hast_canon_kmer(const char *s, int k) { return kmer_canon(kmer_pack(s, k), k); }

size_t hast_chop_read(const char *seq, size_t len, int k, uint64_t *out) {
    if (k < 1 || k > 32 || len < (size_t)k) return 0;
    const uint64_t mask = kmer_mask(k);
    uint64_t w = kmer_pack(seq, k);
    size_t n = 0;
    out[n++] = kmer_canon(w, k);
    for (size_t i = (size_t)k; i < len; i++) {
        w = ((w << 2) & mask) | base_code((uint8_t)seq[i]);
        out[n++] = kmer_canon(w, k);
    }
    return n;
}

void hast_kmer_to_str(uint64_t kmer, int k, char *out) {
    for (int i = 0; i < k; i++) {
        out[k - 1 - i] = "ACTG"[kmer & 3];
        kmer >>= 2;
    }
    out[k] = 0;
}

hast_status hast_synth_keys_host(const hast_synth_params *p, int hap, uint64_t first, size_t n, uint64_t *out) {
    if (hast_status st = check_synth(p)) return st;
    SynthParams sp = resolve(p);
    for (size_t i = 0; i < n; i++) out[i] = synth_key(sp, hap, first + i);
    return HAST_OK;
}

hast_status hast_synth_reads_host(const hast_synth_params *p, uint64_t first, size_t n, uint8_t *bases, uint32_t *ids) {
    if (hast_status st = check_synth(p)) return st;
    SynthParams sp = resolve(p);
    if (sp.read_len == 0) return set_error(HAST_ERR_INVALID, "read_len is 0");
    for (size_t i = 0; i < n; i++) {
        uint32_t bc;
        synth_read(sp, first + i, bases + i * (size_t)sp.read_len, &bc);
        if (ids) ids[i] = bc;
    }
    return HAST_OK;
}

hast_status hast_synth_keys_device(hast_ctx *c, const hast_synth_params *p, int hap, uint64_t first, size_t n,
                                   uint64_t *d_out, hast_stream s) {
    if (hast_status st = use(c)) return st;
    if (hast_status st = check_synth(p)) return st;
    HAST_HIP_TRY(launch_synth_keys(resolve(p), hap, first, n, d_out, s ? (hipStream_t)s : c->stream));
    return HAST_OK;
}

hast_status hast_synth_reads_device(hast_ctx *c, const hast_synth_params *p, uint64_t first, size_t n, uint8_t *d_bases,
                                    uint32_t *d_ids, hast_stream s) {
    if (hast_status st = use(c)) return st;
    if (hast_status st = check_synth(p)) return st;
    if (p->read_len == 0) return set_error(HAST_ERR_INVALID, "read_len is 0");
    HAST_HIP_TRY(launch_synth_reads(resolve(p), first, n, d_bases, d_ids, s ? (hipStream_t)s : c->stream));
    return HAST_OK;
}

hast_status hast_synth_table_build(hast_ctx *c, const hast_synth_params *p) {
    if (hast_status st = need_table(c, 0)) return st;
    if (hast_status st = check_synth(p)) return st;
    if ((int)p->k != c->k) return set_error(HAST_ERR_INVALID, "synth k=%u != context K=%d", p->k, c->k);
    table_changed(c);
    SynthParams sp = resolve(p);
    const size_t per = kChunkBytes / sizeof(uint64_t);
    if (hast_status st = ensure_scratch(c, std::min<uint64_t>(sp.n_keys_per_hap, per) * sizeof(uint64_t) + 16)) return st;
    for (int hap = 0; hap < 2; hap++)
        for (uint64_t i = 0; i < sp.n_keys_per_hap; i += per) {
            size_t m = (size_t)std::min<uint64_t>(per, sp.n_keys_per_hap - i);
            HAST_HIP_TRY(launch_synth_keys(sp, hap, i, m, (uint64_t *)c->d_scratch, c->stream));
            HAST_HIP_TRY(launch_insert_keys(c->d_slots, geom(c), (const uint64_t *)c->d_scratch, m, (uint32_t)hap, c->d_err, c->stream));
        }
    return check_err_word(c, c->stream);
}

}
```

hast_amd/csrc/hast_device.h:

```cpp
#pragma once
#include <hip/hip_runtime.h>
#include <stddef.h>
#include <stdint.h>
#include "hast_common.h"

namespace hast {

struct TableGeom {
    uint32_t nbuckets;
    int k;
    int m;
    int wide;
};

struct ClassifyArgs {
    const uint8_t *bases;
    uint64_t bases_bytes;
    const uint64_t *offsets;
    const uint32_t *lens;
    const uint32_t *seg_read;
    uint32_t *votes;
    unsigned long long *tile_queue;
    const uint64_t *slots;
    uint64_t n_reads;
    const unsigned long long *n_rows_ptr;
    uint32_t nbuckets;
    uint32_t read_len;
    uint32_t max_pos;
    uint32_t w64;
    uint32_t tile_reads;
    uint32_t div_magic;
    uint32_t mh_stride;
    uint32_t div_mh;
    uint32_t div_hw;
    int k;
    int m;
    int wide;
    int strict;
    const void *filter;
    FilterGeom fg;
    uint32_t l1_stride;
    uint32_t div_l1g;
};

hipError_t launch_insert_keys(uint64_t *slots, TableGeom g, const uint64_t *d_keys, size_t n, uint32_t hap,
                              uint32_t *d_err, hipStream_t s);
hipError_t launch_insert_text(uint64_t *slots, TableGeom g, const char *d_text, size_t n_lines,
                              uint32_t hap, int acgt_only, uint32_t *d_err, hipStream_t s);
hipError_t launch_erase_keys(uint64_t *slots, TableGeom g, const uint64_t *d_keys, size_t n, uint8_t *d_hit, hipStream_t s);
hipError_t launch_lookup_keys(uint64_t *slots, TableGeom g, const uint64_t *d_keys, size_t n, uint8_t *d_tags, hipStream_t s);
hipError_t launch_export_slots(const uint64_t *slots, size_t nslots, uint64_t *d_out, size_t cap, unsigned long long *d_counter, hipStream_t s);
hipError_t launch_import_slots(uint64_t *slots, TableGeom g, const uint64_t *d_in, size_t n, uint32_t *d_err, hipStream_t s);
hipError_t launch_count_tags(const uint64_t *slots, TableGeom g, unsigned long long *d_out, hipStream_t s);
hipError_t launch_classify(const ClassifyArgs &a, int grid, size_t smem, hipStream_t s);
hipError_t launch_filter_build(const uint64_t *slots, TableGeom g, void *filter, FilterGeom fg, hipStream_t s);
hipError_t launch_classify_f(const ClassifyArgs &a, int grid, size_t smem, int variants, hipStream_t s);
hipError_t launch_request_ceiling(const void *filter, uint64_t nblocks, uint32_t iters, int grid, uint32_t *d_sink, hipStream_t s);
size_t classify_f_queue_bytes();
hipError_t launch_build_segments(const uint64_t *d_offsets, const uint32_t *d_lens, uint64_t fixed_len, size_t n_reads, int k, uint32_t seg_windows, uint64_t *seg_off,
                                 uint32_t *seg_len, uint32_t *seg_read, unsigned long long *d_counter, const uint8_t *d_skip,
                                 uint64_t cap, uint64_t bases_bytes, uint32_t *d_err, hipStream_t s);
hipError_t launch_scan_n(const uint8_t *d_bases, const uint64_t *d_offsets, const uint32_t *d_lens, uint64_t fixed_len, size_t n_reads, uint8_t *d_has_n, hipStream_t s);
hipError_t launch_commit_votes(const uint32_t *d_votes, const uint32_t *d_barcode_ids, unsigned long long *d_counts, uint32_t *d_votes_out,
                               size_t n_reads, hipStream_t s);
bool commit_partition_usable(size_t n_reads, size_t n_barcodes, uint32_t max_votes, bool forced);
size_t commit_partition_scratch_bytes(size_t n_reads, size_t n_barcodes, uint32_t *n_bins_out, uint32_t *cap_out);
hipError_t launch_commit_partitioned(const uint32_t *d_votes, const uint32_t *d_barcode_ids, unsigned long long *d_counts, size_t n_barcodes, size_t n_reads,
                                     void *d_scratch, hipStream_t s);
hipError_t launch_add_u64(unsigned long long *d_dst, const unsigned long long *d_src, size_t n, hipStream_t s);
hipError_t launch_counts_pack(const unsigned long long *d_counts, unsigned long long *d_packed, size_t n, hipStream_t s);
hipError_t launch_counts_unpack(unsigned long long *d_counts, const unsigned long long *d_packed, size_t n, hipStream_t s);
hipError_t launch_synth_keys(const SynthParams &p, int hap, uint64_t first, size_t n, uint64_t *d_out, hipStream_t s);
hipError_t launch_synth_reads(const SynthParams &p, uint64_t first, size_t n, uint8_t *d_bases, uint32_t *d_bc, hipStream_t s);

}
```

hast_amd/csrc/hast_filter.hip:

```cpp
#include "hast_common.h"
#include "hast_device.h"
#include "hast_devutil.h"

namespace hast {

__device__ __forceinline__ uint32_t sub_load(const uint32_t *w) {
    uint32_t n = 0;
    for (int i = 0; i < kFilterPrints / 2; ++i) {
        const uint32_t v = __hip_atomic_load(&w[i], __ATOMIC_RELAXED, __HIP_MEMORY_SCOPE_AGENT);
        n += (v & 0xFFFFu) != 0;
        n += (v >> 16) != 0;
    }
    return n;
}
__device__ __forceinline__ bool sub_insert(uint32_t *w, uint32_t fp) {
    for (int i = 0; i < kFilterPrints / 2;) {
        const uint32_t v = __hip_atomic_load(&w[i], __ATOMIC_RELAXED, __HIP_MEMORY_SCOPE_AGENT);
        const uint32_t lo = v & 0xFFFFu, hi = v >> 16;
        if (lo == fp || hi == fp) return true;
        uint32_t nv;
        if (lo == 0) nv = v | fp;
        else if (hi == 0) nv = v | (fp << 16);
        else { ++i; continue; }
        if (atomicCAS(&w[i], v, nv) == v) return true;
    }
    return false;
}
__device__ __forceinline__ void sub_mark_overflow(uint32_t *w) {
    uint32_t v = __hip_atomic_load(&w[kFilterPrints / 2 - 1], __ATOMIC_RELAXED, __HIP_MEMORY_SCOPE_AGENT);
    while ((v >> 16) != kFilterOverflowMark) {
        const uint32_t old = atomicCAS(&w[kFilterPrints / 2 - 1], v, (v & 0xFFFFu) | (kFilterOverflowMark << 16));
        if (old == v) break;
        v = old;
    }
}
__device__ __forceinline__ void filter_insert(uint32_t *filt, const FilterGeom g, uint64_t key, uint32_t tags) {
    for (int o = 0; o < 2; ++o) {
        const uint64_t s = o ? kmer_revcomp(key, g.k) : key;
        if (o && s == key) break;
        if (g.exact) {
            const uint32_t pm0 = g.dense ? 0u : filter_sample_pos(s, g), pm1 = g.dense ? filter_w(g) : pm0 + 1u;
            for (uint32_t pm = pm0; pm < pm1; ++pm) {
                const uint32_t blk = filter_block_of((uint32_t)(s >> (2 * (g.k - g.m - (int)pm))) & (uint32_t)kmer_mask(g.m), g.m);
                const uint32_t c17 = filter_exact_code(s, pm, g);
                uint32_t *w = filt + (size_t)blk * (kFilterSubs * kFilterPrints / 2) + filter_exact_sub(c17) * (kFilterPrints / 2);
                if (!sub_insert(w, filter_exact_entry(c17, tags))) sub_mark_overflow(w);
            }
            continue;
        }
        const uint32_t blk = filter_block_of_string(s, g);
        const uint32_t h = filter_keyhash(s), fp = filter_print_of(h);
        uint32_t *b = filt + (size_t)blk * (kFilterSubs * kFilterPrints / 2);
        uint32_t *w1 = b + filter_sub_of(h) * (kFilterPrints / 2), *w2 = b + filter_sub2_of(h) * (kFilterPrints / 2);
        if (g.choices == 1) {
            (void)sub_insert(w1, fp);
            continue;
        }
        bool there = false;
        for (int i = 0; i < kFilterPrints / 2 && !there; ++i) {
            const uint32_t v = __hip_atomic_load(&w2[i], __ATOMIC_RELAXED, __HIP_MEMORY_SCOPE_AGENT);
            there = (v & 0xFFFFu) == fp || (v >> 16) == fp;
        }
        if (there) continue;
        if (w1 != w2 && sub_load(w2) < sub_load(w1)) { uint32_t *t = w1; w1 = w2; w2 = t; }
        if (!sub_insert(w1, fp) && w1 != w2) (void)sub_insert(w2, fp);
    }
}

__global__ void __launch_bounds__(256) k_filter_build(const uint64_t *slots, size_t nslots, uint32_t *filt, FilterGeom g, int wide) {
    for (size_t i = blockIdx.x * (size_t)blockDim.x + threadIdx.x; i < nslots; i += (size_t)gridDim.x * blockDim.x) {
        const uint64_t s = slots[i];
        if (wide) {
            if (s < kTombSlot) filter_insert(filt, g, s, 0);
        } else if (s != kEmptySlot && (s & 3)) filter_insert(filt, g, s >> 2, (uint32_t)(s & 3));
    }
}

hipError_t launch_filter_build(const uint64_t *slots, TableGeom tg, void *filter, FilterGeom fg, hipStream_t s) {
    const size_t nslots = (size_t)tg.nbuckets * kSlotsPerBucket * (tg.wide ? 2 : 1);
    size_t grid = (nslots + 255) / 256;
    if (grid > 256 * 32) grid = 256 * 32;
    hipLaunchKernelGGL(k_filter_build, dim3((unsigned)grid), dim3(256), 0, s, slots, nslots, (uint32_t *)filter, fg, tg.wide);
    return hipGetLastError();
}

constexpr int kThreadsF = 256;
constexpr int kQCap = 128;
#ifndef HAST_F_MINWAVES
#define HAST_F_MINWAVES 5
#endif
#ifndef HAST_F_MINWAVES_DENSE
#define HAST_F_MINWAVES_DENSE 5
#endif
typedef unsigned long long u64x2f __attribute__((ext_vector_type(2)));
typedef unsigned int u32x4f __attribute__((ext_vector_type(4)));
typedef unsigned short u16x2f __attribute__((ext_vector_type(2)));

size_t classify_f_queue_bytes() { return (size_t)4 * kQCap * 3 * sizeof(uint32_t); }

__device__ __forceinline__ uint32_t pk_min_u16(uint32_t a, uint32_t b) {
    const u16x2f r = __builtin_elementwise_min(__builtin_bit_cast(u16x2f, a), __builtin_bit_cast(u16x2f, b));
    return __builtin_bit_cast(uint32_t, r);
}
__device__ __forceinline__ unsigned long long ballot64(bool p) { return __builtin_amdgcn_ballot_w64(p); }
__device__ __forceinline__ uint32_t pk_max_u16(uint32_t a, uint32_t b) {
    const u16x2f r = __builtin_elementwise_max(__builtin_bit_cast(u16x2f, a), __builtin_bit_cast(u16x2f, b));
    return __builtin_bit_cast(uint32_t, r);
}
__device__ __forceinline__ uint32_t tmer_level_of_word(uint32_t word, uint32_t tm) { return __builtin_amdgcn_ubfe(word, tm << 2, 4u); }
__device__ __forceinline__ uint32_t tmer_order_lds(const uint32_t *lvl, uint32_t tm, uint32_t pos) {
    return tmer_order_lvl(tm, pos, tmer_level_of_word(lvl[(tm >> 3) & 0x1FFu], tm));
}
__device__ __forceinline__ uint32_t lanes_below(unsigned long long mask) {
    return __builtin_amdgcn_mbcnt_hi((uint32_t)(mask >> 32), __builtin_amdgcn_mbcnt_lo((uint32_t)mask, 0u));
}

template <int GEO> struct GeoConst { static constexpr int k = 0, m = 0, t = 0, kp = 0; };
template <> struct GeoConst<1> { static constexpr int k = 21, m = 14, t = 6, kp = 21; };
template <> struct GeoConst<2> { static constexpr int k = 31, m = 15, t = 6, kp = 23; };

template <int NTC, bool FAST, bool STRICT, bool WIDE, bool EXACT, bool TWO, int GEO = 0, int RL = 0, bool DENSE = false>
__global__ void __launch_bounds__(kThreadsF, DENSE ? HAST_F_MINWAVES_DENSE : HAST_F_MINWAVES) k_classify_f(ClassifyArgs a) {
    static_assert(!DENSE || EXACT, "dense filing is a property of exact entries");
    extern __shared__ __align__(16) unsigned char smem[];
    __shared__ uint32_t s_lvl[kTmerLevelTableWords];
    typedef GeoConst<GEO> GC0;
    constexpr bool RLC = RL != 0 && GEO != 0;
    const uint32_t TR = a.tile_reads;
    const uint32_t W64 = RLC ? (uint32_t)((RL + 31) / 32) : a.w64;
    const uint32_t WS = W64 + 1;
    const uint32_t L1S = DENSE ? 0u : RLC ? (uint32_t)((RL - GC0::t + 1 + 1 + 3) & ~3) : a.l1_stride;
    unsigned long long *s_tile = reinterpret_cast<unsigned long long *>(smem);
    uint32_t *s_dirty = reinterpret_cast<uint32_t *>(s_tile + 1);
    uint32_t *s_l1 = reinterpret_cast<uint32_t *>(s_tile + 2);
    unsigned long long *s_pack = reinterpret_cast<unsigned long long *>(s_l1 + (size_t)TR * L1S + 64);
    unsigned long long *s_vote = s_pack + (size_t)TR * WS;
    unsigned long long *s_off = s_vote + TR;
    uint32_t *s_len = reinterpret_cast<uint32_t *>(s_off + TR);
    uint32_t *s_flag = s_len + TR;
    uint32_t *s_q = s_flag + TR;
    const uint32_t IW = 2 * W64 + 1;
    uint32_t *s_inv = s_q + 4 * 3 * kQCap;

    const uint32_t tid = threadIdx.x;
    const uint32_t lane = tid & 63;
    const uint32_t wave = (uint32_t)__builtin_amdgcn_readfirstlane((int)(tid >> 6));
    uint32_t *q_lo = s_q + wave * 3 * kQCap, *q_hi = q_lo + kQCap, *q_rd = q_hi + kQCap;
    typedef GeoConst<GEO> GC;
    FilterGeom fg = a.fg;
    if (GEO) {
        fg.k = GC::k; fg.m = GC::m; fg.t = GC::t; fg.kp = GC::kp;
        fg.g = 4;
        fg.wdiv = 65536u / (uint32_t)(GC::kp - GC::m + 1) + 1u;
    }
    const int K = GEO ? GC::k : a.k, M = fg.m, T = fg.t;
    const uint32_t G = (uint32_t)fg.g, W = filter_w(fg), NT = filter_nt(fg);
    const uint32_t ntc = NTC ? (uint32_t)NTC : (NT + G - 1) / G;
    const uint32_t kshift = 64 - 2 * K, tshift = 64 - 2 * T;
    const uint32_t mmask = (uint32_t)kmer_mask(M);
    const uint32_t nb = a.nbuckets;
    const uint64_t n_rows = a.n_rows_ptr ? min((uint64_t)*a.n_rows_ptr, (uint64_t)a.n_reads) : a.n_reads;
    const uint64_t n_tiles = (n_rows + TR - 1) / TR;
    const uintptr_t base_addr = reinterpret_cast<uintptr_t>(a.bases);
    const uintptr_t end_addr = (base_addr + a.bases_bytes + 3) & ~(uintptr_t)3;
    const u32x4f *filt = reinterpret_cast<const u32x4f *>(a.filter);
    const u64x2f *tab0 = reinterpret_cast<const u64x2f *>(a.slots);

    if (!DENSE)
        for (uint32_t i = tid; i < kTmerLevelTableWords; i += kThreadsF) s_lvl[i] = kTmerLevelWords[i];
    if (tid == 0) *s_tile = atomicAdd(a.tile_queue, 1ull);
    __syncthreads();
    for (;;) {
        const uint64_t tile = *s_tile;
        if (tile >= n_tiles) break;
        const uint64_t r0 = tile * TR;
        const uint32_t tra = (uint32_t)((n_rows - r0 < TR) ? (n_rows - r0) : TR);

        if (STRICT && tid == 0) *s_dirty = 0;
        if (tid < tra) {
            uint64_t off, len;
            const uint32_t rlen = RLC ? (uint32_t)RL : a.read_len;
            if (a.offsets) { off = a.offsets[r0 + tid]; len = a.lens ? a.lens[r0 + tid] : a.offsets[r0 + tid + 1] - off; }
            else           { off = (r0 + tid) * (uint64_t)rlen; len = rlen; }
            if (len > rlen) len = rlen;
            if (a.offsets && off > a.bases_bytes) len = 0;
            s_off[tid] = off;
            s_len[tid] = (uint32_t)len;
            s_flag[tid] = 0;
            s_vote[tid] = 0;
        }
        __syncthreads();
        if (tid == 0) *s_tile = atomicAdd(a.tile_queue, 1ull);

        const uint32_t HW = W64 * 2;
        for (uint32_t t = tid; t < tra * HW; t += kThreadsF) {
            const uint32_t r = RLC ? (t / HW) : FAST ? __umulhi(t, a.div_hw) : (t / HW);
            const uint32_t j = t - r * HW;
            const uint32_t len = s_len[r];
            if (16 * j >= len) continue;
            const uint32_t nbases = (len - 16 * j < 16) ? (len - 16 * j) : 16;
            const uintptr_t addr = base_addr + s_off[r] + 16 * j;
            const uintptr_t a4 = addr & ~(uintptr_t)3;
            const uint32_t bsh = (uint32_t)(addr & 3);
            uint32_t d[5];
#pragma unroll
            for (int i = 0; i < 5; ++i) {
                uintptr_t p = a4 + 4 * i;
                d[i] = (p < end_addr) ? *reinterpret_cast<const uint32_t *>(p) : 0x41414141u;
            }
            uint32_t packed = 0, nflag = 0, invalid = 0;
#pragma unroll
            for (int i = 0; i < 4; ++i) {
                uint32_t x = __builtin_amdgcn_alignbyte(d[i + 1], d[i], bsh);
                int vb = (int)nbases - 4 * i;
                if (vb < 4) {
                    uint32_t m = (vb <= 0) ? 0u : ((1u << (8 * vb)) - 1u);
                    x = (x & m) | (0x41414141u & ~m);
                }
                if (STRICT) invalid = (invalid << 4) | not_acgt4(x);
                else nflag |= has_byte_N(x);
                packed = (packed << 8) | pack4(x);
            }
            uint32_t *dst = reinterpret_cast<uint32_t *>(s_pack + (size_t)r * WS + (j >> 1)) + (1 - (j & 1));
            *dst = packed;
            if (STRICT) {
                uint16_t *di = reinterpret_cast<uint16_t *>(s_inv + (size_t)r * IW + (j >> 1)) + (1 - (j & 1));
                *di = (uint16_t)invalid;
                if (invalid) {
                    atomicOr(&s_flag[r], 1u);
                    *s_dirty = 1;
                }
            } else if (nflag) atomicOr(&s_flag[r], 1u);
        }
        __syncthreads();

        if (DENSE) {
        } else if (G == 4) {
            const uint32_t gpr = L1S >> 2, total = tra * gpr;
            const uint32_t t3shift = 64 - 2 * ((uint32_t)T + 3), tmask = (uint32_t)kmer_mask(T);
            for (uint32_t b0 = wave * 63; b0 < total; b0 += 4 * 63) {
                const uint32_t gi = b0 + lane;
                const bool in = gi < total;
                uint32_t r = RLC ? (gi / gpr) : FAST ? __umulhi(gi, a.div_l1g) : (gi / gpr);
                r = in ? r : 0;
                const uint32_t q0 = in ? 4 * (gi - r * gpr) : 0;
                const int nv = in ? (int)s_len[r] - T + 1 - (int)q0 : 0;
                const unsigned long long bits = window_bits(s_pack + (size_t)r * WS, nv > 0 ? q0 : 0, t3shift);
                uint32_t tm[4], lw[4], e[4];
#pragma unroll
                for (int i = 0; i < 4; ++i) {
                    tm[i] = (uint32_t)(bits >> (2 * (3 - i))) & tmask;
                    lw[i] = s_lvl[(tm[i] >> 3) & 0x1FFu];
                }
#pragma unroll
                for (int i = 0; i < 4; ++i) {
                    const uint32_t o = tmer_order_lvl(tm[i], q0 + i, tmer_level_of_word(lw[i], tm[i]));
                    e[i] = i < nv ? o : 0xFFFFFFFFu;
                }
                const uint32_t s2 = min(e[2], e[3]), s1 = min(e[1], s2), s0 = min(e[0], s1);
                const uint32_t p1 = min(e[0], e[1]), p2 = min(p1, e[2]);
                const uint32_t n0 = (uint32_t)__builtin_amdgcn_update_dpp(-1, (int)e[0], 0x130, 0xF, 0xF, false);
                const uint32_t n1 = (uint32_t)__builtin_amdgcn_update_dpp(-1, (int)p1, 0x130, 0xF, 0xF, false);
                const uint32_t n2 = (uint32_t)__builtin_amdgcn_update_dpp(-1, (int)p2, 0x130, 0xF, 0xF, false);
                if (lane < 63 && in)
                    *reinterpret_cast<u32x4f *>(s_l1 + (size_t)r * L1S + q0) = u32x4f{s0, min(s1, n0), min(s2, n1), min(e[3], n2)};
            }
        } else {
            const uint32_t total = tra * L1S, step = 64 - (G - 1);
            for (uint32_t b0 = wave * step; b0 < total; b0 += 4 * step) {
                const uint32_t idx = b0 + lane;
                uint32_t r = idx / L1S;
                uint32_t q = idx - r * L1S;
                const bool in = idx < total;
                r = in ? r : 0;
                const bool valid = in && (q + T <= s_len[r]);
                q = valid ? q : 0;
                const uint32_t tm = (uint32_t)window_bits(s_pack + (size_t)r * WS, q, tshift);
                const uint32_t e = valid ? tmer_order_lds(s_lvl, tm, q) : 0xFFFFFFFFu;
                uint32_t mn = e;
                if (G >= 2) mn = min(mn, (uint32_t)__shfl_down((int)e, 1));
                if (G >= 3) mn = min(mn, (uint32_t)__shfl_down((int)e, 2));
                if (lane < step && in) s_l1[idx] = mn;
            }
        }
        if (!DENSE) __syncthreads();
        if (!STRICT) {
            if (tid < tra && s_flag[tid]) s_len[tid] = 0;
            __syncthreads();
        }

        const uint32_t P = RLC ? (uint32_t)(RL - GC0::k + 1) : a.max_pos;
        const bool tile_dirty = STRICT && __builtin_amdgcn_readfirstlane((int)*s_dirty) != 0;
        uint32_t qn = 0;
        auto drain = [&](uint32_t cnt) {
            const bool act = lane < cnt;
            const uint32_t e = act ? qn - cnt + lane : 0;
            const unsigned long long key = kmer_canon(((unsigned long long)q_hi[e] << 32) | q_lo[e], K);
            const uint32_t rd = q_rd[e];
            qn -= cnt;
            for (int pass = 0; pass < (WIDE ? 2 : 1); ++pass) {
                const u64x2f *tab = tab0 + (WIDE ? (size_t)pass * nb * kPieces : 0);
                const unsigned long long want = WIDE ? key : (key << 2);
                uint32_t b = act ? home_bucket(key, K, a.m, nb) : 0;
                bool pending = act;
                uint32_t step = 0;
                while (__any(pending)) {
                    u64x2f s[kPieces];
#pragma unroll
                    for (int l = 0; l < kPieces; ++l) s[l] = u64x2f{kEmptySlot, kEmptySlot};
                    if (pending) {
#pragma unroll
                        for (int l = 0; l < kPieces; ++l) s[l] = tab[(size_t)b * kPieces + l];
                    }
                    unsigned long long hit_slot = 0;
                    bool hit = false;
#pragma unroll
                    for (int l = 0; l < kPieces; ++l) {
                        if ((WIDE ? s[l].x : (s[l].x & ~3ull)) == want) { hit_slot = s[l].x; hit = true; }
                        if ((WIDE ? s[l].y : (s[l].y & ~3ull)) == want) { hit_slot = s[l].y; hit = true; }
                    }
                    hit = hit && pending;
                    if (hit) {
                        const uint32_t tags = WIDE ? (1u << pass) : (uint32_t)(hit_slot & 3);
                        if (tags) atomicAdd(&s_vote[rd], (unsigned long long)(tags & 1) | ((unsigned long long)(tags >> 1) << 32));
                    }
                    if (pending && (hit || s[kPieces - 1].y == kEmptySlot || ++step >= nb)) pending = false;
                    if (pending) b = next_bucket(b, step, key, nb);
                }
            }
        };
        struct Blk {
            u32x4f v, v2;
            uint32_t klo, khi, fpw, meta;
        };
        uint32_t pos = 0, q_end = 0, last_fb = 0;
        uint32_t cr = 0, cp = 0;
        auto locate = [&]() {
            const uint32_t q = pos + lane;
            cr = RLC ? (q / P) : FAST ? __umulhi(q, a.div_magic) : (q / P);
            cp = q - cr * P;
        };
        auto start = [&](Blk &B) {
            const bool inq = lane < q_end - pos;
            const uint32_t r = min(cr, TR - 1), p = cp;
            const uint32_t len = s_len[r];
            const bool fits = p + K <= len;
            bool ok = inq & fits;
            unsigned long long okm = ballot64(inq) & ballot64(fits);
            if (STRICT) {
                if (tile_dirty && ballot64(s_flag[r] != 0)) {
                    const uint32_t *iw = s_inv + mul24(r, IW) + (p >> 5);
                    const unsigned long long bits = (((unsigned long long)iw[0] << 32) | iw[1]) << (p & 31);
                    const bool clean = (bits >> (64 - K)) == 0;
                    ok = ok & clean;
                    okm &= ballot64(clean);
                }
            }
            const unsigned long long fwd = window_bits(s_pack + mul24(r, WS), p, kshift);
            uint32_t pm;
            if (DENSE) {
                pm = filter_dense_pm(p, W);
            } else {
                const uint32_t *l1 = s_l1 + mul24(r, L1S) + p;
                uint32_t x = l1[0];
                if (NTC) {
#pragma unroll
                    for (int c = 1; c + 1 < (NTC ? NTC : 1); ++c) x = min(x, l1[c * 4]);
                } else {
                    for (uint32_t c = 1; c + 1 < ntc; ++c) x = min(x, l1[c * G]);
                }
                if (ntc > 1) x = min(x, l1[NT - G]);
                const uint32_t xr = ((x & 0xFFFu) - p) & 63u;
                pm = (GEO && (W & (W - 1)) == 0) ? (xr & (W - 1)) : xr - mul24(mul24(xr, fg.wdiv) >> 16, W);
            }
            const uint32_t mm = (uint32_t)(fwd >> (2 * ((uint32_t)(K - M) - pm))) & mmask;
            uint32_t fb = ok ? filter_block_of(mm, M) : 0xFFFFFFFFu;
            const uint32_t h = EXACT ? filter_exact_code(fwd, pm, fg) : filter_keyhash(fwd);
            const uint32_t anchor = okm ? (uint32_t)__builtin_amdgcn_readlane((int)fb, (int)__builtin_ctzll(okm)) : last_fb;
            last_fb = anchor;
            fb = ok ? fb : anchor;
            if (EXACT) {
                B.v = filt[(fb << 3) | filter_exact_sub(h)];
                B.fpw = mul24((h & 0x3FFFu) ^ 0x3FFFu, 0x00040004u);
            } else {
                B.v = filt[(size_t)fb * kFilterSubs + filter_sub_of(h)];
                if (TWO) B.v2 = filt[(size_t)fb * kFilterSubs + filter_sub2_of(h)];
                const uint32_t fp = filter_print_of(h);
                B.fpw = fp | (fp << 16);
            }
            B.klo = (uint32_t)fwd;
            B.khi = (uint32_t)(fwd >> 32);
            B.meta = r | (ok ? 0x80000000u : 0u);
            pos = pos + 64 < q_end ? pos + 64 : q_end;
            if (P >= 64) {
                cp += 64;
                const bool wrap = cp >= P;
                cp -= wrap ? P : 0u;
                cr += wrap ? 1u : 0u;
            } else locate();
        };
        auto finish = [&](Blk &B) {
            bool pos;
            if (EXACT) {
                const uint32_t mx = pk_max_u16(pk_max_u16(B.v.x ^ B.fpw, B.v.y ^ B.fpw), pk_max_u16(B.v.z ^ B.fpw, B.v.w ^ B.fpw));
                const uint32_t m16 = max(mx >> 16, mx & 0xFFFFu);
                const bool valid = (int)B.meta < 0;
                const bool hit = valid && m16 >= 0xFFFDu;
                if (hit) atomicAdd(&s_vote[B.meta & 0xFFFFu], (unsigned long long)(m16 & 1u) | ((unsigned long long)((m16 >> 1) & 1u) << 32));
                pos = valid && !hit && (B.v.w >> 16) == kFilterOverflowMark;
            } else {
            uint32_t acc = pk_min_u16(pk_min_u16(B.v.x ^ B.fpw, B.v.y ^ B.fpw), pk_min_u16(B.v.z ^ B.fpw, B.v.w ^ B.fpw));
            bool full = (B.v.w >> 16) != 0;
            if (TWO) {
                acc = pk_min_u16(acc, pk_min_u16(pk_min_u16(B.v2.x ^ B.fpw, B.v2.y ^ B.fpw), pk_min_u16(B.v2.z ^ B.fpw, B.v2.w ^ B.fpw)));
                full = full && (B.v2.w >> 16) != 0;
            }
            const bool match = ((acc - 0x00010001u) & ~acc & 0x80008000u) != 0;
            pos = (int)B.meta < 0 && (match || full);
            }
            const unsigned long long pmask = ballot64(pos);
            if (pmask) {
                const uint32_t at = qn + lanes_below(pmask);
                if (pos) {
                    q_lo[at] = B.klo;
                    q_hi[at] = B.khi;
                    q_rd[at] = B.meta & 0xFFFFu;
                }
                qn += (uint32_t)__popcll(pmask);
                if (qn >= 64) drain(64);
            }
        };
        {
            const uint32_t rpw = (tra + 3) >> 2;
            const uint32_t r_first = wave * rpw < tra ? wave * rpw : tra, r_last = r_first + rpw < tra ? r_first + rpw : tra;
            pos = r_first * P;
            q_end = r_last * P;
            locate();
            if (pos < q_end) {
                Blk A, B;
                start(A);
                while (pos < q_end) {
                    start(B);
                    finish(A);
                    start(A);
                    finish(B);
                }
                finish(A);
            }
            while (qn) drain(qn < 64 ? qn : 64);
        }
        __syncthreads();

        if (tid < tra) {
            const unsigned long long v = s_vote[tid];
            if (a.votes) {
                if (a.seg_read) {
                    uint32_t *row = a.votes + 2 * (size_t)a.seg_read[r0 + tid];
                    if ((uint32_t)v) atomicAdd(row, (uint32_t)v);
                    if ((uint32_t)(v >> 32)) atomicAdd(row + 1, (uint32_t)(v >> 32));
                } else {
                    reinterpret_cast<unsigned long long *>(a.votes)[r0 + tid] = v;
                }
            }
        }
    }
}

__global__ void __launch_bounds__(256) k_request_ceiling(const u32x4f *filt, uint64_t nblocks, uint32_t iters, uint32_t *sink) {
    const uint64_t gid = (blockIdx.x * (uint64_t)blockDim.x + threadIdx.x) >> 3;
    const uint32_t sub = threadIdx.x & 7;
    u32x4f acc = {0, 0, 0, 0};
    for (uint32_t it = 0; it < iters; ++it) {
        u32x4f v[4];
#pragma unroll
        for (int u = 0; u < 4; ++u) {
            const uint64_t h = splitmix64(gid * 0x10001ull + (uint64_t)it * 4 + (uint64_t)u);
            const uint64_t blk = (uint64_t)(((unsigned __int128)h * nblocks) >> 64);
            v[u] = filt[blk * kFilterSubs + sub];
        }
#pragma unroll
        for (int u = 0; u < 4; ++u) acc ^= v[u];
    }
    if ((acc.x ^ acc.y ^ acc.z ^ acc.w) == 0x9E3779B9u) sink[0] = 1;
}
hipError_t launch_request_ceiling(const void *filter, uint64_t nblocks, uint32_t iters, int grid, uint32_t *d_sink, hipStream_t s) {
    hipLaunchKernelGGL(k_request_ceiling, dim3(grid), dim3(256), 0, s, reinterpret_cast<const u32x4f *>(filter), nblocks, iters, d_sink);
    return hipGetLastError();
}

template <int NTC, bool FAST, bool STRICT, bool WIDE, bool EXACT, bool TWO, int GEO = 0, int RL = 0, bool DENSE = false>
static hipError_t launch_f_t(const ClassifyArgs &a, int grid, size_t smem, hipStream_t s) {
    if (smem > (48u << 10)) {
        hipError_t e = hipFuncSetAttribute(reinterpret_cast<const void *>(k_classify_f<NTC, FAST, STRICT, WIDE, EXACT, TWO, GEO, RL, DENSE>),
                                           hipFuncAttributeMaxDynamicSharedMemorySize, (int)smem);
        if (e != hipSuccess) return e;
    }
    hipLaunchKernelGGL((k_classify_f<NTC, FAST, STRICT, WIDE, EXACT, TWO, GEO, RL, DENSE>), dim3(grid), dim3(kThreadsF), smem, s, a);
    return hipGetLastError();
}
static bool rows_are(const ClassifyArgs &a, uint32_t rl, int k, int t) {
    return a.read_len == rl && a.w64 == (rl + 31) / 32 && a.max_pos == rl - (uint32_t)k + 1 &&
           a.l1_stride == (a.fg.dense ? 0u : ((rl - (uint32_t)t + 1 + 1 + 3) & ~3u));
}
static bool geo_is(const ClassifyArgs &a, int k, int m, int t, int kp) {
    return a.k == k && a.fg.k == k && a.fg.m == m && a.fg.t == t && a.fg.kp == kp && a.fg.g == 4;
}

template <bool STRICT>
static hipError_t launch_f_dense(const ClassifyArgs &a, int grid, size_t smem, int variants, hipStream_t s) {
    const bool fast = a.div_magic && a.div_hw;
    const bool geo_on = (variants & 1) != 0, rl_on = (variants & 2) != 0;
    if (fast && geo_on && !STRICT && geo_is(a, 21, 14, 6, 21)) {
        if (rl_on && rows_are(a, 150, 21, 6)) return launch_f_t<4, true, false, false, true, false, 1, 150, true>(a, grid, smem, s);
        if (rl_on && rows_are(a, 100, 21, 6)) return launch_f_t<4, true, false, false, true, false, 1, 100, true>(a, grid, smem, s);
        return launch_f_t<4, true, false, false, true, false, 1, 0, true>(a, grid, smem, s);
    }
    return fast ? launch_f_t<0, true, STRICT, false, true, false, 0, 0, true>(a, grid, smem, s)
                : launch_f_t<0, false, STRICT, false, true, false, 0, 0, true>(a, grid, smem, s);
}

template <bool STRICT, bool EXACT, bool TWO>
static hipError_t launch_f_s(const ClassifyArgs &a, int grid, size_t smem, int variants, hipStream_t s) {
    const bool fast = a.div_magic && a.div_l1g && a.div_hw;
    if (a.wide) return fast ? launch_f_t<0, true, STRICT, true, false, TWO>(a, grid, smem, s) : launch_f_t<0, false, STRICT, true, false, TWO>(a, grid, smem, s);
    if (!fast || a.fg.g != 4) return fast ? launch_f_t<0, true, STRICT, false, EXACT, TWO>(a, grid, smem, s) : launch_f_t<0, false, STRICT, false, EXACT, TWO>(a, grid, smem, s);
    const bool geo_on = (variants & 1) != 0, rl_on = (variants & 2) != 0;
    if (geo_on && !STRICT && EXACT && !TWO && geo_is(a, 21, 14, 6, 21)) {
        if (rl_on && rows_are(a, 150, 21, 6)) return launch_f_t<4, true, false, false, true, false, 1, 150>(a, grid, smem, s);
        if (rl_on && rows_are(a, 100, 21, 6)) return launch_f_t<4, true, false, false, true, false, 1, 100>(a, grid, smem, s);
        return launch_f_t<4, true, false, false, true, false, 1>(a, grid, smem, s);
    }
    if (geo_on && STRICT && !EXACT && !TWO && geo_is(a, 31, 15, 6, 23)) {
        if (rl_on && rows_are(a, 512, 31, 6)) return launch_f_t<5, true, true, false, false, false, 2, 512>(a, grid, smem, s);
        return launch_f_t<5, true, true, false, false, false, 2>(a, grid, smem, s);
    }
    switch ((filter_nt(a.fg) + 3) / 4) {
    case 1: return launch_f_t<1, true, STRICT, false, EXACT, TWO>(a, grid, smem, s);
    case 2: return launch_f_t<2, true, STRICT, false, EXACT, TWO>(a, grid, smem, s);
    case 3: return launch_f_t<3, true, STRICT, false, EXACT, TWO>(a, grid, smem, s);
    case 4: return launch_f_t<4, true, STRICT, false, EXACT, TWO>(a, grid, smem, s);
    case 5: return launch_f_t<5, true, STRICT, false, EXACT, TWO>(a, grid, smem, s);
    case 6: return launch_f_t<6, true, STRICT, false, EXACT, TWO>(a, grid, smem, s);
    default: return launch_f_t<0, true, STRICT, false, EXACT, TWO>(a, grid, smem, s);
    }
}

hipError_t launch_classify_f(const ClassifyArgs &a, int grid, size_t smem, int variants, hipStream_t s) {
    if (a.n_reads == 0) return hipSuccess;
    if (a.fg.exact && a.fg.dense && !a.wide) {
        const uint32_t w = filter_w(a.fg);
        if (a.l1_stride != 0 || (w & (w - 1)) != 0) return hipErrorInvalidValue;
        return a.strict ? launch_f_dense<true>(a, grid, smem, variants, s) : launch_f_dense<false>(a, grid, smem, variants, s);
    }
    if (a.fg.exact && !a.wide) return a.strict ? launch_f_s<true, true, false>(a, grid, smem, variants, s) : launch_f_s<false, true, false>(a, grid, smem, variants, s);
    if (a.fg.choices == 1) return a.strict ? launch_f_s<true, false, false>(a, grid, smem, variants, s) : launch_f_s<false, false, false>(a, grid, smem, variants, s);
    return a.strict ? launch_f_s<true, false, true>(a, grid, smem, variants, s) : launch_f_s<false, false, true>(a, grid, smem, variants, s);
}

}
```

hast_amd/csrc/hast_kernels.hip:

```cpp
#include "hast_common.h"
#include "hast_device.h"
#include "hast_devutil.h"

namespace hast {

__device__ __forceinline__ uint64_t *hap_table(uint64_t *slots, const TableGeom g, uint32_t hap) {
    return g.wide ? slots + (size_t)hap * g.nbuckets * kSlotsPerBucket : slots;
}
__device__ __forceinline__ bool slot_has_key(unsigned long long slot, uint64_t key, int wide) {
    return wide ? slot == key : (slot >> 2) == key;
}

__device__ __forceinline__ bool table_insert(uint64_t *slots, const TableGeom g, uint64_t key, uint32_t hap) {
    const uint32_t nbuckets = g.nbuckets;
    const uint32_t tag = 1u << hap;
    const uint64_t want = g.wide ? key : ((key << 2) | tag);
    uint64_t *tab = hap_table(slots, g, hap);
    uint32_t b = home_bucket(key, g.k, g.m, nbuckets);
    for (uint32_t probe = 0; probe < nbuckets; ++probe) {
        unsigned long long *bs = reinterpret_cast<unsigned long long *>(tab) + (size_t)b * kSlotsPerBucket;
        for (int i = 0; i < kSlotsPerBucket; ++i) {
            unsigned long long cur = __hip_atomic_load(&bs[i], __ATOMIC_RELAXED, __HIP_MEMORY_SCOPE_AGENT);
            for (;;) {
                if (cur == kEmptySlot) {
                    unsigned long long old = atomicCAS(&bs[i], (unsigned long long)kEmptySlot, (unsigned long long)want);
                    if (old == kEmptySlot) return true;
                    cur = old;
                    continue;
                }
                if (slot_has_key(cur, key, g.wide)) {
                    if (!g.wide && (cur & tag) == 0) atomicOr(&bs[i], (unsigned long long)tag);
                    return true;
                }
                break;
            }
        }
        b = next_bucket(b, probe + 1, key, nbuckets);
    }
    return false;
}

__device__ __forceinline__ unsigned long long *table_find(uint64_t *tab, const TableGeom g, uint64_t key) {
    const uint32_t nbuckets = g.nbuckets;
    uint32_t b = home_bucket(key, g.k, g.m, nbuckets);
    for (uint32_t probe = 0; probe < nbuckets; ++probe) {
        unsigned long long *bs = reinterpret_cast<unsigned long long *>(tab) + (size_t)b * kSlotsPerBucket;
        bool any_empty = false;
        for (int i = 0; i < kSlotsPerBucket; ++i) {
            unsigned long long cur = bs[i];
            if (cur == kEmptySlot) any_empty = true;
            else if (slot_has_key(cur, key, g.wide)) return &bs[i];
        }
        if (any_empty) return nullptr;
        b = next_bucket(b, probe + 1, key, nbuckets);
    }
    return nullptr;
}

__global__ void __launch_bounds__(256) k_insert_keys(uint64_t *slots, TableGeom g, const uint64_t *keys,
                                                     size_t n, uint32_t hap, uint32_t *err) {
    for (size_t i = blockIdx.x * (size_t)blockDim.x + threadIdx.x; i < n; i += (size_t)gridDim.x * blockDim.x)
        if (!table_insert(slots, g, keys[i], hap)) atomicOr(&err[0], 1u);
}

__global__ void __launch_bounds__(256) k_insert_text(uint64_t *slots, TableGeom g, const char *text,
                                                     size_t n_lines, uint32_t hap, int acgt_only, uint32_t *err) {
    const int k = g.k;
    for (size_t i = blockIdx.x * (size_t)blockDim.x + threadIdx.x; i < n_lines; i += (size_t)gridDim.x * blockDim.x) {
        const char *s = text + i * (size_t)(k + 1);
        uint64_t w = 0;
        bool bad = s[k] != '\n', other = false;
        for (int j = 0; j < k; ++j) {
            uint32_t c = (uint8_t)s[j];
            bad |= (c == '\n');
            other |= !(c == 'A' || c == 'C' || c == 'G' || c == 'T');
            w = (w << 2) | base_code(c);
        }
        if (bad) { atomicOr(&err[0], 2u); continue; }
        if (acgt_only && other) { atomicOr(&err[0], 4u); continue; }
        if (!table_insert(slots, g, kmer_canon(w, k), hap)) atomicOr(&err[0], 1u);
    }
}

__global__ void k_erase_keys(uint64_t *slots, TableGeom g, const uint64_t *keys, size_t n, uint8_t *hit) {
    size_t i = blockIdx.x * (size_t)blockDim.x + threadIdx.x;
    if (i >= n) return;
    if (!g.wide) {
        unsigned long long *p = table_find(slots, g, keys[i]);
        unsigned long long old = p ? atomicAnd(p, ~3ull) : 0ull;
        hit[i] = (uint8_t)(old & 3);
        return;
    }
    uint32_t h = 0;
    for (uint32_t hap = 0; hap < 2; ++hap) {
        unsigned long long *p = table_find(hap_table(slots, g, hap), g, keys[i]);
        if (p && atomicCAS(p, (unsigned long long)keys[i], (unsigned long long)kTombSlot) == keys[i]) h |= 1u << hap;
    }
    hit[i] = (uint8_t)h;
}

__global__ void k_lookup_keys(uint64_t *slots, TableGeom g, const uint64_t *keys, size_t n, uint8_t *tags) {
    size_t i = blockIdx.x * (size_t)blockDim.x + threadIdx.x;
    if (i >= n) return;
    if (!g.wide) {
        unsigned long long *p = table_find(slots, g, keys[i]);
        tags[i] = p ? (uint8_t)(*p & 3) : 0;
        return;
    }
    uint32_t t = 0;
    for (uint32_t hap = 0; hap < 2; ++hap)
        if (table_find(hap_table(slots, g, hap), g, keys[i])) t |= 1u << hap;
    tags[i] = (uint8_t)t;
}

__global__ void __launch_bounds__(256) k_export_slots(const uint64_t *slots, size_t nslots, uint64_t *out, size_t cap,
                                                      unsigned long long *counter) {
    for (size_t i = blockIdx.x * (size_t)blockDim.x + threadIdx.x; i < nslots; i += (size_t)gridDim.x * blockDim.x) {
        const uint64_t s = slots[i];
        if (s != kEmptySlot && (s & 3)) {
            const unsigned long long at = atomicAdd(counter, 1ull);
            if (at < cap) out[at] = s;
        }
    }
}
__global__ void __launch_bounds__(256) k_import_slots(uint64_t *slots, TableGeom g, const uint64_t *in, size_t n, uint32_t *err) {
    for (size_t i = blockIdx.x * (size_t)blockDim.x + threadIdx.x; i < n; i += (size_t)gridDim.x * blockDim.x) {
        const uint64_t s = in[i];
        if ((s & 3) == 0 || (s >> 2) >> (2 * g.k)) { atomicOr(&err[0], 2u); continue; }
        bool ok = true;
        if (s & 1) ok = table_insert(slots, g, s >> 2, 0);
        if (ok && (s & 2)) ok = table_insert(slots, g, s >> 2, 1);
        if (!ok) atomicOr(&err[0], 1u);
    }
}

__global__ void __launch_bounds__(256) k_count_tags(const uint64_t *slots, size_t nslots, unsigned long long *out, int wide) {
    unsigned long long c0 = 0, c1 = 0;
    const ulonglong2 *v = reinterpret_cast<const ulonglong2 *>(slots);
    size_t n2 = nslots / 2;
    for (size_t i = blockIdx.x * (size_t)blockDim.x + threadIdx.x; i < n2; i += (size_t)gridDim.x * blockDim.x) {
        ulonglong2 s = v[i];
        if (wide) {
            const unsigned long long live = (unsigned long long)(s.x < kTombSlot) + (unsigned long long)(s.y < kTombSlot);
            if (2 * i < nslots / 2) c0 += live; else c1 += live;
            continue;
        }
        if (s.x != kEmptySlot) { c0 += s.x & 1; c1 += (s.x >> 1) & 1; }
        if (s.y != kEmptySlot) { c0 += s.y & 1; c1 += (s.y >> 1) & 1; }
    }
    for (int off = 32; off > 0; off >>= 1) {
        c0 += __shfl_down(c0, off, 64);
        c1 += __shfl_down(c1, off, 64);
    }
    if ((threadIdx.x & 63) == 0) {
        if (c0) atomicAdd(&out[0], c0);
        if (c1) atomicAdd(&out[1], c1);
    }
}

constexpr int kThreads = 256;
#ifndef HAST_MINWAVES
#define HAST_MINWAVES 5
#endif
#ifndef HAST_LPB
#define HAST_LPB 2
#endif
constexpr int kLPB = HAST_LPB;
constexpr int kRounds = kLPB;
constexpr int kNLd = kPieces / kLPB;
constexpr uint32_t kGrpMask = (1u << kLPB) - 1;
typedef unsigned long long u64x2 __attribute__((ext_vector_type(2)));

template <int J>
__device__ __forceinline__ uint32_t group_bcast(uint32_t v) {
    constexpr int ctrl = kLPB == 4 ? J * 0x55 : (J | (J << 2) | ((2 + J) << 4) | ((2 + J) << 6));
    return (uint32_t)__builtin_amdgcn_mov_dpp((int)v, ctrl, 0xF, 0xF, true);
}

template <int WT, bool FAST, bool STRICT, bool WIDE>
__global__ void __launch_bounds__(kThreads, HAST_MINWAVES) k_classify(ClassifyArgs a) {
    extern __shared__ __align__(16) unsigned char smem[];
    const uint32_t TR = a.tile_reads;
    const uint32_t WS = a.w64 + 1;
    const uint32_t MS = a.mh_stride;
    unsigned long long *s_tile = reinterpret_cast<unsigned long long *>(smem);
    unsigned long long *s_pack = s_tile + 2;
    unsigned long long *s_vote = s_pack + (size_t)TR * WS;
    unsigned long long *s_off = s_vote + TR;
    uint32_t *s_len = reinterpret_cast<uint32_t *>(s_off + TR);
    uint32_t *s_flag = s_len + TR;
    uint32_t *s_mh = s_flag + TR;
    const uint32_t IW = 2 * a.w64 + 1;
    uint32_t *s_inv = s_mh + (size_t)TR * MS + 16;

    const uint32_t tid = threadIdx.x;
    const uint32_t lane = tid & 63;
    const uint32_t wave = tid >> 6;
    const uint32_t sub = tid & (kLPB - 1);
    const uint32_t wofs = 32 * (lane >> 5) + (32 / kLPB) * sub + ((lane & 31) / kLPB);
    const uint32_t gsh = lane & ~(uint32_t)(kLPB - 1);
    const int K = a.k, M = a.m;
    const uint32_t W = WT ? (uint32_t)WT : (uint32_t)(K - M + 1);
    const uint32_t kshift = 64 - 2 * K, mshift = 64 - 2 * M;
    const uint32_t nb = a.nbuckets;
    const uint64_t n_rows = a.n_rows_ptr ? min((uint64_t)*a.n_rows_ptr, (uint64_t)a.n_reads) : a.n_reads;
    const uint64_t n_tiles = (n_rows + TR - 1) / TR;
    const uintptr_t base_addr = reinterpret_cast<uintptr_t>(a.bases);
    const uintptr_t end_addr = (base_addr + a.bases_bytes + 3) & ~(uintptr_t)3;
    const u64x2 *tab0 = reinterpret_cast<const u64x2 *>(a.slots) + sub;

    if (tid == 0) *s_tile = atomicAdd(a.tile_queue, 1ull);
    __syncthreads();
    for (;;) {
        const uint64_t tile = *s_tile;
        if (tile >= n_tiles) break;
        const uint64_t r0 = tile * TR;
        const uint32_t tra = (uint32_t)((n_rows - r0 < TR) ? (n_rows - r0) : TR);

        if (tid < tra) {
            uint64_t off, len;
            if (a.offsets) { off = a.offsets[r0 + tid]; len = a.lens ? a.lens[r0 + tid] : a.offsets[r0 + tid + 1] - off; }
            else           { off = (r0 + tid) * (uint64_t)a.read_len; len = a.read_len; }
            if (len > a.read_len) len = a.read_len;
            if (a.offsets && off > a.bases_bytes) len = 0;
            s_off[tid] = off;
            s_len[tid] = (uint32_t)len;
            s_flag[tid] = 0;
            s_vote[tid] = 0;
        }
        __syncthreads();
        if (tid == 0) *s_tile = atomicAdd(a.tile_queue, 1ull);

        const uint32_t HW = a.w64 * 2;
        for (uint32_t t = tid; t < tra * HW; t += kThreads) {
            const uint32_t r = FAST ? __umulhi(t, a.div_hw) : (t / HW);
            const uint32_t j = t - r * HW;
            const uint32_t len = s_len[r];
            if (16 * j >= len) continue;
            const uint32_t nbases = (len - 16 * j < 16) ? (len - 16 * j) : 16;
            const uintptr_t addr = base_addr + s_off[r] + 16 * j;
            const uintptr_t a4 = addr & ~(uintptr_t)3;
            const uint32_t bsh = (uint32_t)(addr & 3);
            uint32_t d[5];
#pragma unroll
            for (int i = 0; i < 5; ++i) {
                uintptr_t p = a4 + 4 * i;
                d[i] = (p < end_addr) ? *reinterpret_cast<const uint32_t *>(p) : 0x41414141u;
            }
            uint32_t packed = 0, nflag = 0, invalid = 0;
#pragma unroll
            for (int i = 0; i < 4; ++i) {
                uint32_t x = __builtin_amdgcn_alignbyte(d[i + 1], d[i], bsh);
                int vb = (int)nbases - 4 * i;
                if (vb < 4) {
                    uint32_t m = (vb <= 0) ? 0u : ((1u << (8 * vb)) - 1u);
                    x = (x & m) | (0x41414141u & ~m);
                }
                if (STRICT) invalid = (invalid << 4) | not_acgt4(x);
                else nflag |= has_byte_N(x);
                packed = (packed << 8) | pack4(x);
            }
            uint32_t *dst = reinterpret_cast<uint32_t *>(s_pack + (size_t)r * WS + (j >> 1)) + (1 - (j & 1));
            *dst = packed;
            if (STRICT) {
                uint16_t *di = reinterpret_cast<uint16_t *>(s_inv + (size_t)r * IW + (j >> 1)) + (1 - (j & 1));
                *di = (uint16_t)invalid;
            } else if (nflag) atomicOr(&s_flag[r], 1u);
        }
        __syncthreads();

        for (uint32_t t = tid; t < tra * MS; t += kThreads) {
            const uint32_t r = FAST ? __umulhi(t, a.div_mh) : (t / MS);
            const uint32_t q = t - r * MS;
            const uint64_t mm = window_bits(s_pack + (size_t)r * WS, q, mshift);
            const uint32_t h = mmer_hash32(kmer_canon(mm, M));
            s_mh[t] = (q + M <= s_len[r]) ? h : 0xFFFFFFFFu;
        }
        __syncthreads();
        if (!STRICT) {
            if (tid < tra && s_flag[tid]) s_len[tid] = 0;
            __syncthreads();
        }

        const uint32_t P = a.max_pos;
        const uint32_t Q = tra * P;
        const uint32_t nblk = (Q + 63) >> 6;
        const u64x2 *tab = tab0;
        uint32_t pass_tags = 0;
        struct Blk {
            uint32_t klo, khi, bkt, meta;
            u64x2 sl[kRounds][kNLd];
        };
        auto start = [&](Blk &B, uint32_t blk) {
            const uint32_t q = blk * 64 + wofs;
            uint32_t r = FAST ? __umulhi(q, a.div_magic) : (q / P);
            const bool inq = q < Q;
            r = inq ? r : 0;
            const uint32_t p = inq ? q - r * P : 0;
            bool ok = inq && (p + K <= s_len[r]);
            if (STRICT) {
                const uint32_t *iw = s_inv + r * IW + (p >> 5);
                const unsigned long long bits = (((unsigned long long)iw[0] << 32) | iw[1]) << (p & 31);
                ok = ok && (bits >> (64 - K)) == 0;
            }
            const uint64_t ck = kmer_canon(window_bits(s_pack + (size_t)r * WS, p, kshift), K);
            const uint32_t *mh = s_mh + r * MS + p;
            uint32_t mn = mh[0];
            if (WT) {
#pragma unroll
                for (int j = 1; j < (WT ? WT : 1); ++j) mn = min(mn, mh[j]);
            } else {
                for (uint32_t j = 1; j < W; ++j) mn = min(mn, mh[j]);
            }
            B.klo = WIDE ? (uint32_t)ck : (uint32_t)(ck << 2);
            B.khi = WIDE ? (uint32_t)(ck >> 32) : (uint32_t)(ck >> 30);
            B.bkt = ok ? bucket_of(mn, ck, nb) : 0;
            B.meta = r | (ok ? 0x80000000u : 0u);
            uint32_t bk[kRounds];
            bk[0] = group_bcast<0>(B.bkt);
            bk[1] = group_bcast<1>(B.bkt);
            if (kRounds == 4) {
                bk[kRounds - 2] = group_bcast<kRounds == 4 ? 2 : 0>(B.bkt);
                bk[kRounds - 1] = group_bcast<kRounds == 4 ? 3 : 1>(B.bkt);
            }
#pragma unroll
            for (int j = 0; j < kRounds; ++j)
#pragma unroll
                for (int l = 0; l < kNLd; ++l) B.sl[j][l] = tab[(size_t)bk[j] * kPieces + l * kLPB];
        };
        auto finish = [&](Blk &B) {
            uint32_t kl[kRounds], kh[kRounds], mt[kRounds];
            kl[0] = group_bcast<0>(B.klo); kh[0] = group_bcast<0>(B.khi); mt[0] = group_bcast<0>(B.meta);
            kl[1] = group_bcast<1>(B.klo); kh[1] = group_bcast<1>(B.khi); mt[1] = group_bcast<1>(B.meta);
            if (kRounds == 4) {
                constexpr int J2 = kRounds == 4 ? 2 : 0, J3 = kRounds == 4 ? 3 : 1;
                kl[kRounds - 2] = group_bcast<J2>(B.klo); kh[kRounds - 2] = group_bcast<J2>(B.khi); mt[kRounds - 2] = group_bcast<J2>(B.meta);
                kl[kRounds - 1] = group_bcast<J3>(B.klo); kh[kRounds - 1] = group_bcast<J3>(B.khi); mt[kRounds - 1] = group_bcast<J3>(B.meta);
            }
            uint32_t hitmask = 0, fullmask = 0;
#pragma unroll
            for (int j = 0; j < kRounds; ++j) {
                const unsigned long long kq = ((unsigned long long)kh[j] << 32) | kl[j];
                const bool valid = (int)mt[j] < 0;
                bool m = false;
#pragma unroll
                for (int l = 0; l < kNLd; ++l) m = m || (WIDE ? B.sl[j][l].x : (B.sl[j][l].x & ~3ull)) == kq || (WIDE ? B.sl[j][l].y : (B.sl[j][l].y & ~3ull)) == kq;
                if (valid && m) hitmask |= 1u << j;
                if (valid && B.sl[j][kNLd - 1].y != kEmptySlot && sub == kLPB - 1) fullmask |= 1u << j;
            }
            if (hitmask) {
#pragma unroll
                for (int j = 0; j < kRounds; ++j)
                    if (hitmask & (1u << j)) {
                        const unsigned long long kq = ((unsigned long long)kh[j] << 32) | kl[j];
                        unsigned long long hit_slot = 0;
#pragma unroll
                        for (int l = 0; l < kNLd; ++l) {
                            if ((WIDE ? B.sl[j][l].x : (B.sl[j][l].x & ~3ull)) == kq) hit_slot = B.sl[j][l].x;
                            if ((WIDE ? B.sl[j][l].y : (B.sl[j][l].y & ~3ull)) == kq) hit_slot = B.sl[j][l].y;
                        }
                        const uint32_t tags = WIDE ? pass_tags : (uint32_t)(hit_slot & 3);
                        atomicAdd(&s_vote[mt[j] & 0xFFFF], (unsigned long long)(tags & 1) | ((unsigned long long)(tags >> 1) << 32));
                    }
            }
            if (__any(fullmask != 0)) {
                uint32_t moremask = 0;
#pragma unroll
                for (int j = 0; j < kRounds; ++j) {
                    const unsigned long long f = __ballot((fullmask >> j) & 1), h = __ballot((hitmask >> j) & 1);
                    if (((f >> gsh) & kGrpMask) != 0 && ((h >> gsh) & kGrpMask) == 0) moremask |= 1u << j;
                }
                while (__any(moremask != 0)) {
                    const bool act = moremask != 0;
                    const uint32_t j = act ? (uint32_t)__ffs(moremask) - 1 : 0;
                    const int src = (int)(gsh | j);
                    const unsigned long long kq = ((unsigned long long)__shfl((int)B.khi, src) << 32) | (uint32_t)__shfl((int)B.klo, src);
                    uint32_t b = (uint32_t)__shfl((int)B.bkt, src);
                    const uint32_t rd = (uint32_t)__shfl((int)B.meta, src) & 0xFFFF;
                    bool pending = act;
                    uint32_t guard = 0;
                    while (__any(pending)) {
                        u64x2 s2[kNLd];
#pragma unroll
                        for (int l = 0; l < kNLd; ++l) s2[l] = u64x2{kEmptySlot, kEmptySlot};
                        if (pending) {
                            b = next_bucket(b, guard + 1, WIDE ? kq : (kq >> 2), nb);
#pragma unroll
                            for (int l = 0; l < kNLd; ++l) s2[l] = tab[(size_t)b * kPieces + l * kLPB];
                        }
                        unsigned long long hit_slot = 0;
                        bool h2 = false;
#pragma unroll
                        for (int l = 0; l < kNLd; ++l) {
                            if ((WIDE ? s2[l].x : (s2[l].x & ~3ull)) == kq) { hit_slot = s2[l].x; h2 = true; }
                            if ((WIDE ? s2[l].y : (s2[l].y & ~3ull)) == kq) { hit_slot = s2[l].y; h2 = true; }
                        }
                        h2 = h2 && pending;
                        const unsigned long long m2 = __ballot(h2 || (pending && s2[kNLd - 1].y == kEmptySlot));
                        if (h2) {
                            const uint32_t tags = WIDE ? pass_tags : (uint32_t)(hit_slot & 3);
                            atomicAdd(&s_vote[rd], (unsigned long long)(tags & 1) | ((unsigned long long)(tags >> 1) << 32));
                        }
                        if (((m2 >> gsh) & kGrpMask) != 0 || ++guard >= nb) pending = false;
                    }
                    moremask &= moremask - 1;
                }
            }
        };
        for (int pass = 0; pass < (WIDE ? 2 : 1); ++pass) {
            if (WIDE) {
                tab = tab0 + (size_t)pass * nb * kPieces;
                pass_tags = 1u << pass;
            }
            Blk A, B;
            uint32_t blk = wave;
            bool va = blk < nblk;
            if (va) start(A, blk);
            blk += 4;
            while (va) {
                const bool vb = blk < nblk;
                if (vb) start(B, blk);
                blk += 4;
                finish(A);
                if (!vb) break;
                va = blk < nblk;
                if (va) start(A, blk);
                blk += 4;
                finish(B);
            }
        }
        __syncthreads();

        if (tid < tra) {
            const unsigned long long v = s_vote[tid];
            if (a.votes) {
                if (a.seg_read) {
                    uint32_t *row = a.votes + 2 * (size_t)a.seg_read[r0 + tid];
                    if ((uint32_t)v) atomicAdd(row, (uint32_t)v);
                    if ((uint32_t)(v >> 32)) atomicAdd(row + 1, (uint32_t)(v >> 32));
                } else {
                    reinterpret_cast<unsigned long long *>(a.votes)[r0 + tid] = v;
                }
            }
        }
    }
}

__global__ void k_synth_keys(SynthParams p, int hap, uint64_t first, size_t n, uint64_t *out) {
    for (size_t i = blockIdx.x * (size_t)blockDim.x + threadIdx.x; i < n; i += (size_t)gridDim.x * blockDim.x)
        out[i] = synth_key(p, hap, first + i);
}

__global__ void k_synth_reads(SynthParams p, uint64_t first, size_t n, uint8_t *bases, uint32_t *barcodes) {
    for (size_t i = blockIdx.x * (size_t)blockDim.x + threadIdx.x; i < n; i += (size_t)gridDim.x * blockDim.x) {
        uint32_t bc;
        synth_read(p, first + i, bases + i * (size_t)p.read_len, &bc);
        if (barcodes) barcodes[i] = bc;
    }
}

static inline int grid_for(size_t n, int block, int cap) {
    size_t g = (n + block - 1) / block;
    if (g < 1) g = 1;
    return (int)(g > (size_t)cap ? (size_t)cap : g);
}

hipError_t launch_insert_keys(uint64_t *slots, TableGeom g, const uint64_t *d_keys, size_t n, uint32_t hap,
                              uint32_t *d_err, hipStream_t s) {
    if (n == 0) return hipSuccess;
    hipLaunchKernelGGL(k_insert_keys, dim3(grid_for(n, 256, 256 * 32)), dim3(256), 0, s, slots, g, d_keys, n, hap, d_err);
    return hipGetLastError();
}
hipError_t launch_insert_text(uint64_t *slots, TableGeom g, const char *d_text, size_t n_lines,
                              uint32_t hap, int acgt_only, uint32_t *d_err, hipStream_t s) {
    if (n_lines == 0) return hipSuccess;
    hipLaunchKernelGGL(k_insert_text, dim3(grid_for(n_lines, 256, 256 * 32)), dim3(256), 0, s, slots, g, d_text, n_lines, hap, acgt_only, d_err);
    return hipGetLastError();
}
hipError_t launch_erase_keys(uint64_t *slots, TableGeom g, const uint64_t *d_keys, size_t n, uint8_t *d_hit, hipStream_t s) {
    if (n == 0) return hipSuccess;
    hipLaunchKernelGGL(k_erase_keys, dim3((unsigned)((n + 63) / 64)), dim3(64), 0, s, slots, g, d_keys, n, d_hit);
    return hipGetLastError();
}
hipError_t launch_lookup_keys(uint64_t *slots, TableGeom g, const uint64_t *d_keys, size_t n, uint8_t *d_tags, hipStream_t s) {
    if (n == 0) return hipSuccess;
    hipLaunchKernelGGL(k_lookup_keys, dim3((unsigned)((n + 255) / 256)), dim3(256), 0, s, slots, g, d_keys, n, d_tags);
    return hipGetLastError();
}
hipError_t launch_export_slots(const uint64_t *slots, size_t nslots, uint64_t *d_out, size_t cap, unsigned long long *d_counter, hipStream_t s) {
    hipLaunchKernelGGL(k_export_slots, dim3(grid_for(nslots, 256, 256 * 16)), dim3(256), 0, s, slots, nslots, d_out, cap, d_counter);
    return hipGetLastError();
}
hipError_t launch_import_slots(uint64_t *slots, TableGeom g, const uint64_t *d_in, size_t n, uint32_t *d_err, hipStream_t s) {
    if (n == 0) return hipSuccess;
    hipLaunchKernelGGL(k_import_slots, dim3(grid_for(n, 256, 256 * 32)), dim3(256), 0, s, slots, g, d_in, n, d_err);
    return hipGetLastError();
}
hipError_t launch_count_tags(const uint64_t *slots, TableGeom g, unsigned long long *d_out, hipStream_t s) {
    const size_t nslots = (size_t)g.nbuckets * kSlotsPerBucket * (g.wide ? 2 : 1);
    hipLaunchKernelGGL(k_count_tags, dim3(grid_for(nslots / 2, 256, 256 * 8)), dim3(256), 0, s, slots, nslots, d_out, g.wide);
    return hipGetLastError();
}
template <int WT, bool FAST, bool STRICT, bool WIDE = false>
static hipError_t launch_classify_t(const ClassifyArgs &a, int grid, size_t smem, hipStream_t s) {
    if (smem > (48u << 10)) {
        hipError_t e = hipFuncSetAttribute(reinterpret_cast<const void *>(k_classify<WT, FAST, STRICT, WIDE>),
                                           hipFuncAttributeMaxDynamicSharedMemorySize, (int)smem);
        if (e != hipSuccess) return e;
    }
    hipLaunchKernelGGL((k_classify<WT, FAST, STRICT, WIDE>), dim3(grid), dim3(kThreads), smem, s, a);
    return hipGetLastError();
}

template <bool STRICT>
static hipError_t launch_classify_s(const ClassifyArgs &a, int grid, size_t smem, hipStream_t s) {
    const int w = a.k - a.m + 1;
    const bool fast = a.div_magic && a.div_mh && a.div_hw;
    if (a.wide) return fast ? launch_classify_t<0, true, STRICT, true>(a, grid, smem, s) : launch_classify_t<0, false, STRICT, true>(a, grid, smem, s);
    if (!fast) return launch_classify_t<0, false, STRICT>(a, grid, smem, s);
    switch (w) {
    case 1: return launch_classify_t<1, true, STRICT>(a, grid, smem, s);
    case 2: return launch_classify_t<2, true, STRICT>(a, grid, smem, s);
    case 3: return launch_classify_t<3, true, STRICT>(a, grid, smem, s);
    case 4: return launch_classify_t<4, true, STRICT>(a, grid, smem, s);
    case 5: return launch_classify_t<5, true, STRICT>(a, grid, smem, s);
    case 6: return launch_classify_t<6, true, STRICT>(a, grid, smem, s);
    case 7: return launch_classify_t<7, true, STRICT>(a, grid, smem, s);
    case 8: return launch_classify_t<8, true, STRICT>(a, grid, smem, s);
    case 9: return launch_classify_t<9, true, STRICT>(a, grid, smem, s);
    default: return launch_classify_t<0, true, STRICT>(a, grid, smem, s);
    }
}

hipError_t launch_classify(const ClassifyArgs &a, int grid, size_t smem, hipStream_t s) {
    if (a.n_reads == 0) return hipSuccess;
    return a.strict ? launch_classify_s<true>(a, grid, smem, s) : launch_classify_s<false>(a, grid, smem, s);
}

__global__ void __launch_bounds__(256) k_build_segments(const uint64_t *offsets, const uint32_t *lens, size_t n_reads, int k, uint32_t seg_windows,
                                                        uint64_t *seg_off, uint32_t *seg_len, uint32_t *seg_read, unsigned long long *counter,
                                                        const uint8_t *skip, uint64_t fixed_len, uint64_t cap, uint64_t bases_bytes, uint32_t *err) {
    __shared__ unsigned long long s_off[256], s_len[256], s_first[256];
    __shared__ uint32_t s_nseg[256], s_wave[4];
    __shared__ unsigned long long s_base;
    const uint32_t tid = threadIdx.x, lane = tid & 63;
    const size_t i = blockIdx.x * (size_t)256 + tid;
    uint64_t off = 0, len = 0;
    uint32_t nseg = 0;
    if (i < n_reads) {
        off = offsets ? offsets[i] : i * fixed_len;
        len = (skip && skip[i]) ? 0 : !offsets ? fixed_len : (lens ? (uint64_t)lens[i] : offsets[i + 1] - off);
        if (off > bases_bytes || len > bases_bytes - off) { atomicOr(err, 1u); len = 0; }
        const uint64_t nwin = len >= (uint64_t)k ? len - k + 1 : 0;
        nseg = (uint32_t)(nwin ? (nwin + seg_windows - 1) / seg_windows : 1);
    }
    uint32_t incl = nseg;
    for (int o = 1; o < 64; o <<= 1) {
        const uint32_t t = __shfl_up(incl, o, 64);
        if (lane >= (uint32_t)o) incl += t;
    }
    if (lane == 63) s_wave[tid >> 6] = incl;
    __syncthreads();
    uint32_t before = incl - nseg;
    for (uint32_t w = 0; w < (tid >> 6); ++w) before += s_wave[w];
    if (tid == 255) s_base = atomicAdd(counter, (unsigned long long)(before + nseg));
    __syncthreads();
    s_off[tid] = off;
    s_len[tid] = len;
    s_nseg[tid] = nseg;
    s_first[tid] = s_base + before;
    __syncthreads();
    const uint32_t grp = tid >> 4, gl = tid & 15;
    for (uint32_t r = grp; r < 256; r += 16) {
        const uint32_t ns = s_nseg[r];
        const uint64_t o = s_off[r], l = s_len[r], first = s_first[r];
        const uint32_t read = (uint32_t)(blockIdx.x * (size_t)256 + r);
        for (uint32_t j = gl; j < ns; j += 16) {
            const uint64_t start = (uint64_t)j * seg_windows;
            const uint64_t rest = l - start;
            const uint64_t sl = rest < (uint64_t)seg_windows + k - 1 ? rest : (uint64_t)seg_windows + k - 1;
            if (first + j >= cap) { atomicOr(err, 1u); break; }
            seg_off[first + j] = o + start;
            seg_len[first + j] = (uint32_t)sl;
            seg_read[first + j] = read;
        }
    }
}

__global__ void __launch_bounds__(256) k_scan_n(const uint8_t *bases, const uint64_t *offsets, const uint32_t *lens, size_t n_reads, uint8_t *has_n, uint64_t fixed_len) {
    const size_t wave = (blockIdx.x * (size_t)blockDim.x + threadIdx.x) >> 6;
    const uint32_t lane = threadIdx.x & 63;
    if (wave >= n_reads) return;
    const uint64_t off = offsets ? offsets[wave] : wave * fixed_len, len = !offsets ? fixed_len : lens ? (uint64_t)lens[wave] : offsets[wave + 1] - off;
    bool found = false;
    for (uint64_t i = lane; i < len && !found; i += 64) found = bases[off + i] == 'N';
    const bool any = __any(found);
    if (lane == 0) has_n[wave] = any ? 1 : 0;
}
constexpr int kCommitSlots = 128;
constexpr uint32_t kCommitSpan = 8192, kCommitFlush = 2048, kNoBarcode = 0xFFFFFFFFu;
__global__ void __launch_bounds__(256) k_commit_votes(const uint32_t *votes, const uint32_t *barcode_ids, unsigned long long *counts,
                                                      uint32_t *votes_out, size_t n_reads_arg, const unsigned long long *n_ptr) {
    const size_t n_reads = n_ptr ? (size_t)*n_ptr : n_reads_arg;
    if ((size_t)blockIdx.x * kCommitSpan >= n_reads) return;
    __shared__ unsigned long long s_v0[kCommitSlots], s_v1[kCommitSlots];
    __shared__ uint32_t s_neg[kCommitSlots], s_id[kCommitSlots];
    const uint32_t tid = threadIdx.x;
    auto flush = [&]() {
        if (tid < kCommitSlots) {
            if (s_id[tid] != kNoBarcode) {
                unsigned long long *rec = counts + 4 * (size_t)s_id[tid];
                if (s_v0[tid]) atomicAdd(rec, s_v0[tid]);
                if (s_v1[tid]) atomicAdd(rec + 1, s_v1[tid]);
                if (s_neg[tid]) atomicAdd(rec + 2, (unsigned long long)s_neg[tid]);
            }
            s_id[tid] = kNoBarcode;
            s_v0[tid] = 0;
            s_v1[tid] = 0;
            s_neg[tid] = 0;
        }
    };
    if (tid < kCommitSlots) {
        s_id[tid] = kNoBarcode;
        s_v0[tid] = 0;
        s_v1[tid] = 0;
        s_neg[tid] = 0;
    }
    __syncthreads();
    const size_t span0 = (size_t)blockIdx.x * kCommitSpan;
    for (uint32_t j = 0; j < kCommitSpan; j += 256) {
        const size_t i = span0 + j + tid;
        if (i < n_reads) {
            const unsigned long long v = reinterpret_cast<const unsigned long long *>(votes)[i];
            if (votes_out) reinterpret_cast<unsigned long long *>(votes_out)[i] = v;
            if (barcode_ids) {
                const uint32_t id = barcode_ids[i];
                const unsigned long long v0 = (uint32_t)v, v1 = v >> 32;
                const uint32_t h = id * 0x9E3779B1u;
                uint32_t slot = h >> (32 - 7);
                uint32_t owner = atomicCAS(&s_id[slot], kNoBarcode, id);
                if (owner != kNoBarcode && owner != id) {
                    slot = (h >> 11) & (kCommitSlots - 1);
                    owner = atomicCAS(&s_id[slot], kNoBarcode, id);
                }
                if (owner == kNoBarcode || owner == id) {
                    if (v0) atomicAdd(&s_v0[slot], v0);
                    if (v1) atomicAdd(&s_v1[slot], v1);
                    if (!v) atomicAdd(&s_neg[slot], 1u);
                } else {
                    unsigned long long *rec = counts + 4 * (size_t)id;
                    if (v0) atomicAdd(rec, v0);
                    if (v1) atomicAdd(rec + 1, v1);
                    if (!v) atomicAdd(rec + 2, 1ull);
                }
            }
        }
        if (barcode_ids && (j + 256) % kCommitFlush == 0) {
            __syncthreads();
            flush();
            __syncthreads();
        }
    }
}
constexpr uint32_t kPartMaxSpanBits = 13;
constexpr uint32_t kPartRecs = 16384;
constexpr int kPartThreads = 1024;
constexpr uint32_t kPartMaxBins = 4096;
__global__ void __launch_bounds__(kPartThreads) k_commit_partition(const unsigned long long *votes, const uint32_t *ids, size_t n, uint32_t n_bins,
                                                                  uint32_t span_bits, uint32_t cap, uint32_t *bin_fill, uint32_t *bin_valid, uint32_t *bin_recs,
                                                                  unsigned long long *over_n, uint32_t *over_ids, unsigned long long *over_votes) {
    extern __shared__ __align__(16) unsigned char smem[];
    uint32_t *s_cnt = reinterpret_cast<uint32_t *>(smem);
    uint32_t *s_off = s_cnt + n_bins;
    uint32_t *s_dst = s_off + n_bins;
    uint32_t *s_rec = s_dst + n_bins;
    __shared__ uint32_t s_scan[kPartThreads / 64];
    const uint32_t tid = threadIdx.x;
    const uint32_t kPartSpanBits = span_bits, kPartSpan = 1u << span_bits;
    const size_t r0 = (size_t)blockIdx.x * kPartRecs;
    const uint32_t nr = (uint32_t)(n - r0 < kPartRecs ? n - r0 : kPartRecs);
    for (uint32_t b = tid; b < n_bins; b += kPartThreads) s_cnt[b] = 0;
    __syncthreads();
    constexpr int PER = kPartRecs / kPartThreads;
    uint32_t rec[PER], rank[PER];
    uint32_t bin_of[PER];
#pragma unroll
    for (int q = 0; q < PER; ++q) {
        const uint32_t i = (uint32_t)q * kPartThreads + tid;
        bin_of[q] = 0xFFFFFFFFu;
        if (i < nr) {
            const uint32_t id = ids[r0 + i];
            const unsigned long long v = votes[r0 + i];
            bin_of[q] = id >> kPartSpanBits;
            if (bin_of[q] >= n_bins) { bin_of[q] = 0xFFFFFFFFu; continue; }
            rec[q] = (id & (kPartSpan - 1)) | ((uint32_t)v & 0xFFu) << 13 | ((uint32_t)(v >> 32) & 0xFFu) << 21;
            rank[q] = atomicAdd(&s_cnt[bin_of[q]], 1u);
        }
    }
    __syncthreads();
    {
        uint32_t c[4], sum = 0;
#pragma unroll
        for (int q = 0; q < 4; ++q) {
            const uint32_t b = tid * 4 + q;
            c[q] = b < n_bins ? s_cnt[b] : 0;
            sum += c[q];
        }
        uint32_t incl = sum;
        const uint32_t lane = tid & 63;
        for (int off = 1; off < 64; off <<= 1) {
            const uint32_t t = __shfl_up(incl, off, 64);
            if (lane >= (uint32_t)off) incl += t;
        }
        if (lane == 63) s_scan[tid >> 6] = incl;
        __syncthreads();
        uint32_t base = incl - sum;
        for (uint32_t w = 0; w < (tid >> 6); ++w) base += s_scan[w];
#pragma unroll
        for (int q = 0; q < 4; ++q) {
            const uint32_t b = tid * 4 + q;
            if (b < n_bins) {
                s_off[b] = base;
                base += c[q];
                uint32_t dst = 0;
                if (c[q]) {
                    const uint32_t g = atomicAdd(&bin_fill[b], c[q]);
                    if (g + c[q] <= cap) dst = g;
                    else {
                        atomicMin(&bin_valid[b], g);
                        dst = 0x80000000u | (uint32_t)atomicAdd(over_n, (unsigned long long)c[q]);
                    }
                }
                s_dst[b] = dst;
            }
        }
    }
    __syncthreads();
#pragma unroll
    for (int q = 0; q < PER; ++q)
        if (bin_of[q] != 0xFFFFFFFFu) s_rec[s_off[bin_of[q]] + rank[q]] = rec[q] | 0u;
    __syncthreads();
    const uint32_t grp = tid >> 4, gl = tid & 15;
    for (uint32_t b = grp; b < n_bins; b += kPartThreads / 16) {
        const uint32_t cnt = s_cnt[b];
        if (!cnt) continue;
        const uint32_t dst = s_dst[b], off = s_off[b];
        if (!(dst & 0x80000000u)) {
            uint32_t *out = bin_recs + (size_t)b * cap + dst;
            for (uint32_t j = gl; j < cnt; j += 16) out[j] = s_rec[off + j];
        } else {
            const uint32_t o = dst & 0x7FFFFFFFu;
            for (uint32_t j = gl; j < cnt; j += 16) {
                const uint32_t r = s_rec[off + j];
                over_ids[o + j] = (b << kPartSpanBits) | (r & (kPartSpan - 1));
                over_votes[o + j] = (unsigned long long)((r >> 13) & 0xFFu) | ((unsigned long long)((r >> 21) & 0xFFu) << 32);
            }
        }
    }
}

constexpr int kBinThreads = 1024;
__global__ void __launch_bounds__(kBinThreads) k_commit_bins(const uint32_t *bin_recs, const uint32_t *bin_fill, const uint32_t *bin_valid, uint32_t cap,
                                                     uint32_t span_bits, unsigned long long *counts, size_t n_barcodes) {
    extern __shared__ __align__(16) unsigned char smem[];
    const uint32_t kPartSpanBits = span_bits, kPartSpan = 1u << span_bits;
    unsigned long long *s_vote = reinterpret_cast<unsigned long long *>(smem);
    uint32_t *s_neg = reinterpret_cast<uint32_t *>(s_vote + kPartSpan);
    const uint32_t b = blockIdx.x, tid = threadIdx.x;
    const uint32_t fill = bin_fill[b], valid = bin_valid[b];
    const uint32_t n = fill < valid ? (fill < cap ? fill : cap) : valid;
    if (n == 0) return;
    for (uint32_t j = tid; j < kPartSpan; j += kBinThreads) {
        s_vote[j] = 0;
        s_neg[j] = 0;
    }
    __syncthreads();
    const uint32_t *recs = bin_recs + (size_t)b * cap;
    for (uint32_t i = tid; i < n; i += kBinThreads) {
        const uint32_t r = recs[i];
        const uint32_t id = r & (kPartSpan - 1), v0 = (r >> 13) & 0xFFu, v1 = (r >> 21) & 0xFFu;
        if (v0 | v1) atomicAdd(&s_vote[id], (unsigned long long)v0 | ((unsigned long long)v1 << 32));
        else atomicAdd(&s_neg[id], 1u);
    }
    __syncthreads();
    const size_t first = (size_t)b << kPartSpanBits;
    for (uint32_t j = tid; j < kPartSpan && first + j < n_barcodes; j += kBinThreads) {
        const unsigned long long v = s_vote[j];
        const uint32_t g = s_neg[j];
        if (v | g) {
            unsigned long long *rec = counts + 4 * (first + j);
            if (v) {
                ulonglong2 c = *reinterpret_cast<ulonglong2 *>(rec);
                c.x += (uint32_t)v;
                c.y += v >> 32;
                *reinterpret_cast<ulonglong2 *>(rec) = c;
            }
            if (g) rec[2] += g;
        }
    }
}

static uint32_t part_span_bits(size_t n_barcodes) {
    uint32_t lg = 0;
    while (((size_t)1 << lg) < n_barcodes) ++lg;
    const uint32_t want = lg > 10 ? lg - 10 : 0;
    return want < 8 ? 8u : (want > kPartMaxSpanBits ? kPartMaxSpanBits : want);
}
size_t commit_partition_scratch_bytes(size_t n_reads, size_t n_barcodes, uint32_t *n_bins_out, uint32_t *cap_out) {
    const uint32_t sb = part_span_bits(n_barcodes);
    const uint32_t n_bins = (uint32_t)((n_barcodes + ((size_t)1 << sb) - 1) >> sb);
    const uint64_t mean = n_bins ? (n_reads + n_bins - 1) / n_bins : 0;
    const uint32_t cap = (uint32_t)std::min<uint64_t>(0x7FFFFFFFull, mean + mean / 2 + 2048);
    if (n_bins_out) *n_bins_out = n_bins;
    if (cap_out) *cap_out = cap;
    return 256 + (size_t)n_bins * 8 + 256 + (size_t)n_bins * cap * 4 + 256 + n_reads * 4 + 256 + n_reads * 8;
}
bool commit_partition_usable(size_t n_reads, size_t n_barcodes, uint32_t max_votes, bool forced) {
    uint32_t n_bins, cap;
    (void)commit_partition_scratch_bytes(n_reads, n_barcodes, &n_bins, &cap);
    if (max_votes > 255 || n_bins < 1 || n_bins > kPartMaxBins || n_reads < 1 || n_reads >= (1ull << 31)) return false;
    if ((uint64_t)cap * 255u >= (1ull << 32)) return false;
    return forced || (n_bins >= 128 && n_reads >= (1u << 21));
}
hipError_t launch_commit_partitioned(const uint32_t *d_votes, const uint32_t *d_barcode_ids, unsigned long long *d_counts, size_t n_barcodes, size_t n_reads,
                                     void *d_scratch, hipStream_t s) {
    uint32_t n_bins, cap;
    (void)commit_partition_scratch_bytes(n_reads, n_barcodes, &n_bins, &cap);
    const uint32_t sb = part_span_bits(n_barcodes);
    unsigned char *p = reinterpret_cast<unsigned char *>(d_scratch);
    unsigned long long *over_n = reinterpret_cast<unsigned long long *>(p);
    uint32_t *bin_fill = reinterpret_cast<uint32_t *>(p + 256);
    uint32_t *bin_valid = bin_fill + n_bins;
    size_t at = 256 + (size_t)n_bins * 8;
    at = (at + 255) & ~(size_t)255;
    uint32_t *bin_recs = reinterpret_cast<uint32_t *>(p + at);
    at += (size_t)n_bins * cap * 4;
    at = (at + 255) & ~(size_t)255;
    uint32_t *over_ids = reinterpret_cast<uint32_t *>(p + at);
    at += n_reads * 4;
    at = (at + 255) & ~(size_t)255;
    unsigned long long *over_votes = reinterpret_cast<unsigned long long *>(p + at);
    hipError_t e = hipMemsetAsync(p, 0, 256 + (size_t)n_bins * 4, s);
    if (e != hipSuccess) return e;
    e = hipMemsetAsync(bin_valid, 0xFF, (size_t)n_bins * 4, s);
    if (e != hipSuccess) return e;
    const size_t lds1 = (size_t)n_bins * 12 + (size_t)kPartRecs * 4, lds2 = ((size_t)12 << sb);
    e = hipFuncSetAttribute(reinterpret_cast<const void *>(k_commit_partition), hipFuncAttributeMaxDynamicSharedMemorySize, (int)lds1);
    if (e != hipSuccess) return e;
    e = hipFuncSetAttribute(reinterpret_cast<const void *>(k_commit_bins), hipFuncAttributeMaxDynamicSharedMemorySize, (int)lds2);
    if (e != hipSuccess) return e;
    hipLaunchKernelGGL(k_commit_partition, dim3((unsigned)((n_reads + kPartRecs - 1) / kPartRecs)), dim3(kPartThreads), lds1, s,
                       reinterpret_cast<const unsigned long long *>(d_votes), d_barcode_ids, n_reads, n_bins, sb, cap, bin_fill, bin_valid, bin_recs,
                       over_n, over_ids, over_votes);
    hipLaunchKernelGGL(k_commit_bins, dim3(n_bins), dim3(kBinThreads), lds2, s, bin_recs, bin_fill, bin_valid, cap, sb, d_counts, n_barcodes);
    hipLaunchKernelGGL(k_commit_votes, dim3((unsigned)((n_reads + kCommitSpan - 1) / kCommitSpan)), dim3(256), 0, s,
                       reinterpret_cast<const uint32_t *>(over_votes), over_ids, d_counts, (uint32_t *)nullptr, (size_t)0, over_n);
    return hipGetLastError();
}

hipError_t launch_scan_n(const uint8_t *d_bases, const uint64_t *d_offsets, const uint32_t *d_lens, uint64_t fixed_len, size_t n_reads, uint8_t *d_has_n, hipStream_t s) {
    if (n_reads == 0) return hipSuccess;
    hipLaunchKernelGGL(k_scan_n, dim3((unsigned)((n_reads * 64 + 255) / 256)), dim3(256), 0, s, d_bases, d_offsets, d_lens, n_reads, d_has_n, fixed_len);
    return hipGetLastError();
}
hipError_t launch_commit_votes(const uint32_t *d_votes, const uint32_t *d_barcode_ids, unsigned long long *d_counts, uint32_t *d_votes_out,
                               size_t n_reads, hipStream_t s) {
    if (n_reads == 0) return hipSuccess;
    hipLaunchKernelGGL(k_commit_votes, dim3((unsigned)((n_reads + kCommitSpan - 1) / kCommitSpan)), dim3(256), 0, s, d_votes, d_barcode_ids,
                       d_counts, d_votes_out, n_reads, (const unsigned long long *)nullptr);
    return hipGetLastError();
}

hipError_t launch_build_segments(const uint64_t *d_offsets, const uint32_t *d_lens, uint64_t fixed_len, size_t n_reads, int k, uint32_t seg_windows, uint64_t *seg_off,
                                 uint32_t *seg_len, uint32_t *seg_read, unsigned long long *d_counter, const uint8_t *d_skip,
                                 uint64_t cap, uint64_t bases_bytes, uint32_t *d_err, hipStream_t s) {
    if (n_reads == 0) return hipSuccess;
    hipLaunchKernelGGL(k_build_segments, dim3((unsigned)((n_reads + 255) / 256)), dim3(256), 0, s, d_offsets, d_lens, n_reads, k,
                       seg_windows, seg_off, seg_len, seg_read, d_counter, d_skip, fixed_len, cap, bases_bytes, d_err);
    return hipGetLastError();
}

__global__ void __launch_bounds__(256) k_add_u64(unsigned long long *dst, const unsigned long long *src, size_t n) {
    for (size_t i = blockIdx.x * (size_t)blockDim.x + threadIdx.x; i < n; i += (size_t)gridDim.x * blockDim.x) dst[i] += src[i];
}
hipError_t launch_add_u64(unsigned long long *d_dst, const unsigned long long *d_src, size_t n, hipStream_t s) {
    if (n == 0) return hipSuccess;
    hipLaunchKernelGGL(k_add_u64, dim3(grid_for(n, 256, 256 * 16)), dim3(256), 0, s, d_dst, d_src, n);
    return hipGetLastError();
}

__global__ void __launch_bounds__(256) k_counts_pack(const unsigned long long *counts, unsigned long long *packed, size_t n) {
    for (size_t i = blockIdx.x * (size_t)blockDim.x + threadIdx.x; i < n; i += (size_t)gridDim.x * blockDim.x) {
        const ulonglong2 a = *reinterpret_cast<const ulonglong2 *>(counts + 4 * i);
        packed[i] = a.x;
        packed[n + i] = a.y;
        packed[2 * n + i] = counts[4 * i + 2];
    }
}
__global__ void __launch_bounds__(256) k_counts_unpack(unsigned long long *counts, const unsigned long long *packed, size_t n) {
    for (size_t i = blockIdx.x * (size_t)blockDim.x + threadIdx.x; i < n; i += (size_t)gridDim.x * blockDim.x) {
        ulonglong2 a;
        a.x = packed[i];
        a.y = packed[n + i];
        *reinterpret_cast<ulonglong2 *>(counts + 4 * i) = a;
        counts[4 * i + 2] = packed[2 * n + i];
    }
}
hipError_t launch_counts_pack(const unsigned long long *d_counts, unsigned long long *d_packed, size_t n, hipStream_t s) {
    if (n == 0) return hipSuccess;
    hipLaunchKernelGGL(k_counts_pack, dim3(grid_for(n, 256, 256 * 16)), dim3(256), 0, s, d_counts, d_packed, n);
    return hipGetLastError();
}
hipError_t launch_counts_unpack(unsigned long long *d_counts, const unsigned long long *d_packed, size_t n, hipStream_t s) {
    if (n == 0) return hipSuccess;
    hipLaunchKernelGGL(k_counts_unpack, dim3(grid_for(n, 256, 256 * 16)), dim3(256), 0, s, d_counts, d_packed, n);
    return hipGetLastError();
}

hipError_t launch_synth_keys(const SynthParams &p, int hap, uint64_t first, size_t n, uint64_t *d_out, hipStream_t s) {
    if (n == 0) return hipSuccess;
    hipLaunchKernelGGL(k_synth_keys, dim3(grid_for(n, 256, 256 * 16)), dim3(256), 0, s, p, hap, first, n, d_out);
    return hipGetLastError();
}
hipError_t launch_synth_reads(const SynthParams &p, uint64_t first, size_t n, uint8_t *d_bases, uint32_t *d_bc, hipStream_t s) {
    if (n == 0) return hipSuccess;
    hipLaunchKernelGGL(k_synth_reads, dim3(grid_for(n, 256, 256 * 16)), dim3(256), 0, s, p, first, n, d_bases, d_bc);
    return hipGetLastError();
}

}
```

Baseline: 383.1 billion bp/s.

## Compact commit votes to 16 bits and drop per-batch scratch memsets in partitioned commit

```diff
diff --git a/hast_amd/csrc/commit_plan.h b/hast_amd/csrc/commit_plan.h
--- /dev/null
+++ b/hast_amd/csrc/commit_plan.h
@@ -0,0 +1,58 @@
+#pragma once
+#include <stddef.h>
+#include <stdint.h>
+
+namespace hast {
+namespace commit {
+
+constexpr uint32_t kMinSpanBits = 8, kMaxSpanBits = 13;
+constexpr uint32_t kMaxBins = 4096;
+constexpr uint32_t kGroupRecs = 16384;
+constexpr uint32_t kMaxVotes = 255;
+constexpr size_t kLine = 128, kLineWords = kLine / 4, kAlign = 256;
+
+inline uint32_t span_bits_for(size_t n_barcodes, uint32_t span_override = 0) {
+    if (span_override >= kMinSpanBits && span_override <= kMaxSpanBits) return span_override;
+    uint32_t lg = 0;
+    while (lg < 63 && ((size_t)1 << lg) < n_barcodes) ++lg;
+    const uint32_t want = lg > 10 ? lg - 10 : 0;
+    return want < kMinSpanBits ? kMinSpanBits : (want > kMaxSpanBits ? kMaxSpanBits : want);
+}
+
+struct Plan {
+    uint32_t span_bits, n_bins, cap;
+    size_t over_n_at, lines_at, recs_at, over_ids_at, over_votes_at, bytes;
+    size_t lds_partition, lds_bins;
+};
+
+inline size_t align_up(size_t x) { return (x + kAlign - 1) & ~(kAlign - 1); }
+
+inline Plan plan_for(size_t n_reads, size_t n_barcodes, uint32_t span_override = 0) {
+    Plan p;
+    p.span_bits = span_bits_for(n_barcodes, span_override);
+    const uint64_t bins = ((uint64_t)n_barcodes + ((uint64_t)1 << p.span_bits) - 1) >> p.span_bits;
+    p.n_bins = (uint32_t)(bins < 0xFFFFFFFFull ? bins : 0xFFFFFFFFull);
+    const uint64_t mean = p.n_bins ? ((uint64_t)n_reads + p.n_bins - 1) / p.n_bins : 0;
+    const uint64_t cap = mean + mean / 2 + 2048;
+    p.cap = (uint32_t)(cap < 0x7FFFFFFFull ? cap : 0x7FFFFFFFull);
+    p.over_n_at = 0;
+    p.lines_at = kAlign;
+    p.recs_at = align_up(p.lines_at + (size_t)p.n_bins * kLine);
+    p.over_ids_at = align_up(p.recs_at + (size_t)p.n_bins * p.cap * 4);
+    p.over_votes_at = align_up(p.over_ids_at + n_reads * 4);
+    p.bytes = align_up(p.over_votes_at + n_reads * 8);
+    p.lds_partition = (size_t)p.n_bins * 12 + (size_t)kGroupRecs * 4;
+    p.lds_bins = (size_t)12 << p.span_bits;
+    return p;
+}
+
+inline bool usable(const Plan &p, size_t n_reads, uint32_t max_votes, bool forced) {
+    if (max_votes > kMaxVotes || p.n_bins < 1 || p.n_bins > kMaxBins || n_reads < 1 || n_reads >= ((size_t)1 << 31)) return false;
+    if ((uint64_t)p.cap * kMaxVotes >= ((uint64_t)1 << 32)) return false;
+    return forced || (p.n_bins >= 128 && n_reads >= ((size_t)1 << 21));
+}
+
+constexpr size_t kMaxLdsPartition = (size_t)kMaxBins * 12 + (size_t)kGroupRecs * 4, kMaxLdsBins = (size_t)12 << kMaxSpanBits;
+
+}
+}
diff --git a/hast_amd/csrc/hast_api.cpp b/hast_amd/csrc/hast_api.cpp
--- a/hast_amd/csrc/hast_api.cpp
+++ b/hast_amd/csrc/hast_api.cpp
@@ -69,8 +69,7 @@
     size_t t_slots = 0, t_next = 0, t_count = 0;
     uint32_t *d_votes_scratch = nullptr;
     size_t votes_bytes = 0;
-    void *d_part = nullptr;
-    size_t part_bytes = 0;
+    CommitScratch part;
     char *sf_h[2] = {nullptr, nullptr}, *sf_d[2] = {nullptr, nullptr};
     hipEvent_t sf_done[2] = {nullptr, nullptr};
     void *d_filter = nullptr;
@@ -88,6 +87,7 @@
     int commit_mode = 0;
     int kernel_geo = 1, kernel_rl = 1;
     size_t tile_lds = 0;
+    uint32_t part_span = 0;
     bool part_oom = false;
 };
 
@@ -299,6 +299,7 @@
     if (c->exact_env_off) c->filter_exact = 0;
     else if (c->exact_env_once) c->filter_exact = 1;
     if (const char *e = getenv("HAST_COMMIT")) c->commit_mode = !strcmp(e, "atomic") ? 1 : !strcmp(e, "partition") ? 2 : 0;
+    if (const char *e = getenv("HAST_PART_SPAN")) c->part_span = (uint32_t)atoi(e);
     if (const char *e = getenv("HAST_F_GEO")) c->kernel_geo = e[0] != '0';
     if (const char *e = getenv("HAST_F_RL")) c->kernel_rl = e[0] != '0';
     if (const char *e = getenv("HAST_TILE_LDS")) {
@@ -357,7 +358,7 @@
     if (c->d_scratch) (void)hipFree(c->d_scratch);
     if (c->d_seg) (void)hipFree(c->d_seg);
     if (c->d_votes_scratch) (void)hipFree(c->d_votes_scratch);
-    if (c->d_part) (void)hipFree(c->d_part);
+    if (c->part.d) (void)hipFree(c->part.d);
     for (int i = 0; i < 2; ++i) {
         if (c->sf_done[i]) (void)hipEventDestroy(c->sf_done[i]);
         if (c->sf_d[i]) (void)hipFree(c->sf_d[i]);
@@ -1021,30 +1022,39 @@
 static constexpr uint32_t kSegWindows = 482;
 static constexpr uint32_t kLongRead = 4096;
 
+static hast_status commit_prepare(hast_ctx *c, size_t n_reads, uint32_t max_votes, bool atomic_only, hipStream_t hs, commit::Plan *pl, bool *partitioned) {
+    *partitioned = false;
+    const int mode = c->commit_mode;
+    if (mode == 1 || atomic_only || c->part_oom) return HAST_OK;
+    *pl = commit::plan_for(n_reads, c->n_barcodes, c->part_span);
+    if (!commit::usable(*pl, n_reads, max_votes, mode == 2)) return HAST_OK;
+    if (c->part.bytes < pl->bytes) {
+        HAST_HIP_TRY(hipStreamSynchronize(hs));
+        if (c->part.d) HAST_HIP_TRY(hipFree(c->part.d));
+        c->part = CommitScratch{};
+        if (dev_malloc(&c->part.d, pl->bytes + pl->bytes / 8) == hipSuccess) c->part.bytes = pl->bytes + pl->bytes / 8;
+        else {
+            (void)hipGetLastError();
+            c->part.d = nullptr;
+            c->part_oom = true;
+        }
+    }
+    *partitioned = c->part.d != nullptr;
+    return HAST_OK;
+}
+static hast_status commit_run(hast_ctx *c, const void *d_votes, bool votes16, const uint32_t *d_ids, size_t n_reads, const commit::Plan &pl, bool partitioned,
+                              hipStream_t hs) {
+    if (partitioned) HAST_HIP_TRY(launch_commit_partitioned(d_votes, votes16, d_ids, c->d_counts, c->n_barcodes, n_reads, pl, c->part, hs));
+    else if (votes16) return set_error(HAST_ERR_INVALID, "internal: compact votes reached the atomic commit");
+    else HAST_HIP_TRY(launch_commit_votes(reinterpret_cast<const uint32_t *>(d_votes), d_ids, c->d_counts, nullptr, n_reads, hs));
+    return HAST_OK;
+}
 static hast_status commit_votes(hast_ctx *c, const uint32_t *d_votes, const uint32_t *d_ids, size_t n_reads, uint32_t max_votes,
                                 bool atomic_only, hipStream_t hs) {
-    const int mode = c->commit_mode;
-    if (mode != 1 && !atomic_only && !c->part_oom && commit_partition_usable(n_reads, c->n_barcodes, max_votes, mode == 2)) {
-        const size_t need = commit_partition_scratch_bytes(n_reads, c->n_barcodes, nullptr, nullptr);
-        if (c->part_bytes < need) {
-            HAST_HIP_TRY(hipStreamSynchronize(hs));
-            if (c->d_part) HAST_HIP_TRY(hipFree(c->d_part));
-            c->d_part = nullptr;
-            c->part_bytes = 0;
-            if (dev_malloc(&c->d_part, need + need / 8) == hipSuccess) c->part_bytes = need + need / 8;
-            else {
-                (void)hipGetLastError();
-                c->d_part = nullptr;
-                c->part_oom = true;
-            }
-        }
-        if (c->d_part) {
-            HAST_HIP_TRY(launch_commit_partitioned(d_votes, d_ids, c->d_counts, c->n_barcodes, n_reads, c->d_part, hs));
-            return HAST_OK;
-        }
-    }
-    HAST_HIP_TRY(launch_commit_votes(d_votes, d_ids, c->d_counts, nullptr, n_reads, hs));
-    return HAST_OK;
+    commit::Plan pl{};
+    bool partitioned = false;
+    if (hast_status st = commit_prepare(c, n_reads, max_votes, atomic_only, hs, &pl, &partitioned)) return st;
+    return commit_run(c, d_votes, false, d_ids, n_reads, pl, partitioned, hs);
 }
 
 static hast_status classify_rows(hast_ctx *c, const uint8_t *d_bases, size_t bases_bytes, const uint64_t *d_offsets,
@@ -1067,11 +1077,18 @@
     a.seg_read = d_seg_read;
     a.strict = strict;
     if (reinterpret_cast<uintptr_t>(d_votes) & 7) return set_error(HAST_ERR_INVALID, "d_votes must be 8-byte aligned (a row is stored as one 64-bit word)");
+    hipStream_t hs = s ? (hipStream_t)s : c->stream;
+    const uint32_t max_pos = read_len >= (uint32_t)c->k ? read_len - c->k + 1 : 0;
+    commit::Plan pl{};
+    bool partitioned = false;
+    if (d_barcode_ids)
+        if (hast_status st = commit_prepare(c, n_reads, max_pos, d_seg_read != nullptr, hs, &pl, &partitioned)) return st;
+    const bool votes16 = partitioned && !d_votes && !d_seg_read && max_pos <= commit::kMaxVotes;
     uint32_t *votes_buf = d_votes;
     if (d_barcode_ids && !votes_buf) {
-        const size_t need = n_reads * 2 * sizeof(uint32_t);
+        const size_t need = n_reads * (votes16 ? sizeof(uint16_t) : 2 * sizeof(uint32_t));
         if (c->votes_bytes < need) {
-            HAST_HIP_TRY(hipStreamSynchronize(s ? (hipStream_t)s : c->stream));
+            HAST_HIP_TRY(hipStreamSynchronize(hs));
             if (c->d_votes_scratch) HAST_HIP_TRY(hipFree(c->d_votes_scratch));
             c->d_votes_scratch = nullptr;
             c->votes_bytes = 0;
@@ -1080,7 +1097,8 @@
         }
         votes_buf = c->d_votes_scratch;
     }
-    a.votes = votes_buf;
+    a.votes = votes16 ? nullptr : votes_buf;
+    a.votes16 = votes16 ? reinterpret_cast<uint16_t *>(votes_buf) : nullptr;
     a.slots = c->d_slots;
     a.n_reads = n_reads;
     a.n_rows_ptr = d_n_rows;
@@ -1089,10 +1107,9 @@
     a.k = c->k;
     a.wide = c->k == 32;
     a.m = c->m;
-    a.max_pos = read_len >= (uint32_t)c->k ? read_len - c->k + 1 : 0;
+    a.max_pos = max_pos;
     a.mh_stride = read_len >= (uint32_t)c->m ? read_len - c->m + 1 : 0;
     a.w64 = (read_len + 31) / 32;
-    hipStream_t hs = s ? (hipStream_t)s : c->stream;
     if (c->use_filter)
         if (hast_status st = ensure_filter(c, hs)) return st;
     const bool filt = c->use_filter;
@@ -1142,7 +1159,7 @@
     HAST_HIP_TRY(filt ? launch_classify_f(a, grid, smem, (c->kernel_geo ? 1 : 0) | (c->kernel_rl ? 2 : 0), hs) : launch_classify(a, grid, smem, hs));
     if (ev) HAST_HIP_TRY(hipEventRecord(ev[1], hs));
     if (d_barcode_ids) {
-        if (hast_status st = commit_votes(c, votes_buf, d_barcode_ids, n_reads, a.max_pos, d_seg_read != nullptr, hs)) return st;
+        if (hast_status st = commit_run(c, votes_buf, votes16, d_barcode_ids, n_reads, pl, partitioned, hs)) return st;
     }
     if (ev) {
         HAST_HIP_TRY(hipEventRecord(ev[2], hs));
@@ -1176,6 +1193,9 @@
     if (!strcmp(name, "commit")) {
         if (value < 0 || value > 2) return set_error(HAST_ERR_INVALID, "commit: 0 = by batch size, 1 = atomic, 2 = partitioned");
         c->commit_mode = (int)value;
+    } else if (!strcmp(name, "part_span")) {
+        if (value && (value < (long)commit::kMinSpanBits || value > (long)commit::kMaxSpanBits)) return set_error(HAST_ERR_INVALID, "part_span %ld out of [8, 13]", value);
+        c->part_span = (uint32_t)value;
     } else if (!strcmp(name, "kernel_geo")) c->kernel_geo = value != 0;
     else if (!strcmp(name, "kernel_rl")) c->kernel_rl = value != 0;
     else if (!strcmp(name, "tile_lds")) {
@@ -1199,6 +1219,7 @@
     if (c->filter_t) add("filter_t", c->filter_t);
     if (c->filter_kp) add("filter_kp", c->filter_kp);
     if (c->commit_mode) add("commit", c->commit_mode);
+    if (c->part_span) add("part_span", (long)c->part_span);
     if (!c->kernel_geo) add("kernel_geo", 0);
     if (!c->kernel_rl) add("kernel_rl", 0);
     if (c->tile_lds) add("tile_lds", (long)c->tile_lds);
diff --git a/hast_amd/csrc/hast_device.h b/hast_amd/csrc/hast_device.h
--- a/hast_amd/csrc/hast_device.h
+++ b/hast_amd/csrc/hast_device.h
@@ -2,6 +2,7 @@
 #include <hip/hip_runtime.h>
 #include <stddef.h>
 #include <stdint.h>
+#include "commit_plan.h"
 #include "hast_common.h"
 
 namespace hast {
@@ -20,6 +21,7 @@
     const uint32_t *lens;
     const uint32_t *seg_read;
     uint32_t *votes;
+    uint16_t *votes16;
     unsigned long long *tile_queue;
     const uint64_t *slots;
     uint64_t n_reads;
@@ -63,10 +65,14 @@
 hipError_t launch_scan_n(const uint8_t *d_bases, const uint64_t *d_offsets, const uint32_t *d_lens, uint64_t fixed_len, size_t n_reads, uint8_t *d_has_n, hipStream_t s);
 hipError_t launch_commit_votes(const uint32_t *d_votes, const uint32_t *d_barcode_ids, unsigned long long *d_counts, uint32_t *d_votes_out,
                                size_t n_reads, hipStream_t s);
-bool commit_partition_usable(size_t n_reads, size_t n_barcodes, uint32_t max_votes, bool forced);
-size_t commit_partition_scratch_bytes(size_t n_reads, size_t n_barcodes, uint32_t *n_bins_out, uint32_t *cap_out);
-hipError_t launch_commit_partitioned(const uint32_t *d_votes, const uint32_t *d_barcode_ids, unsigned long long *d_counts, size_t n_barcodes, size_t n_reads,
-                                     void *d_scratch, hipStream_t s);
+struct CommitScratch {
+    void *d = nullptr;
+    size_t bytes = 0;
+    uint32_t n_bins = 0, cap = 0;
+    uint32_t parity = 0;
+};
+hipError_t launch_commit_partitioned(const void *d_votes, bool votes16, const uint32_t *d_barcode_ids, unsigned long long *d_counts, size_t n_barcodes,
+                                     size_t n_reads, const commit::Plan &pl, CommitScratch &sc, hipStream_t s);
 hipError_t launch_add_u64(unsigned long long *d_dst, const unsigned long long *d_src, size_t n, hipStream_t s);
 hipError_t launch_counts_pack(const unsigned long long *d_counts, unsigned long long *d_packed, size_t n, hipStream_t s);
 hipError_t launch_counts_unpack(unsigned long long *d_counts, const unsigned long long *d_packed, size_t n, hipStream_t s);
diff --git a/hast_amd/csrc/hast_filter.hip b/hast_amd/csrc/hast_filter.hip
--- a/hast_amd/csrc/hast_filter.hip
+++ b/hast_amd/csrc/hast_filter.hip
@@ -453,7 +453,9 @@
 
         if (tid < tra) {
             const unsigned long long v = s_vote[tid];
-            if (a.votes) {
+            if (a.votes16) {
+                a.votes16[r0 + tid] = (uint16_t)((uint32_t)v | (uint32_t)(v >> 32) << 8);
+            } else if (a.votes) {
                 if (a.seg_read) {
                     uint32_t *row = a.votes + 2 * (size_t)a.seg_read[r0 + tid];
                     if ((uint32_t)v) atomicAdd(row, (uint32_t)v);
diff --git a/hast_amd/csrc/hast_kernels.hip b/hast_amd/csrc/hast_kernels.hip
--- a/hast_amd/csrc/hast_kernels.hip
+++ b/hast_amd/csrc/hast_kernels.hip
@@ -1,6 +1,8 @@
 #include "hast_common.h"
 #include "hast_device.h"
 #include "hast_devutil.h"
+
+#include <atomic>
 
 namespace hast {
 
@@ -433,7 +435,9 @@
 
         if (tid < tra) {
             const unsigned long long v = s_vote[tid];
-            if (a.votes) {
+            if (a.votes16) {
+                a.votes16[r0 + tid] = (uint16_t)((uint32_t)v | (uint32_t)(v >> 32) << 8);
+            } else if (a.votes) {
                 if (a.seg_read) {
                     uint32_t *row = a.votes + 2 * (size_t)a.seg_read[r0 + tid];
                     if ((uint32_t)v) atomicAdd(row, (uint32_t)v);
@@ -662,12 +666,13 @@
         }
     }
 }
-constexpr uint32_t kPartMaxSpanBits = 13;
-constexpr uint32_t kPartRecs = 16384;
+constexpr uint32_t kPartRecs = commit::kGroupRecs;
 constexpr int kPartThreads = 1024;
-constexpr uint32_t kPartMaxBins = 4096;
-__global__ void __launch_bounds__(kPartThreads) k_commit_partition(const unsigned long long *votes, const uint32_t *ids, size_t n, uint32_t n_bins,
-                                                                  uint32_t span_bits, uint32_t cap, uint32_t *bin_fill, uint32_t *bin_valid, uint32_t *bin_recs,
+constexpr uint32_t kPartLineWords = (uint32_t)commit::kLineWords;
+static_assert(commit::kMaxBins == 4 * kPartThreads, "the scan of k_commit_partition takes 4 bins per thread");
+template <bool V16>
+__global__ void __launch_bounds__(kPartThreads) __attribute__((amdgpu_waves_per_eu(8, 8))) k_commit_partition(const void *votes_in, const uint32_t *ids, size_t n, uint32_t n_bins,
+                                                                  uint32_t span_bits, uint32_t cap, uint32_t *bin_lines, uint32_t *bin_recs,
                                                                   unsigned long long *over_n, uint32_t *over_ids, unsigned long long *over_votes) {
     extern __shared__ __align__(16) unsigned char smem[];
     uint32_t *s_cnt = reinterpret_cast<uint32_t *>(smem);
@@ -682,30 +687,42 @@
     for (uint32_t b = tid; b < n_bins; b += kPartThreads) s_cnt[b] = 0;
     __syncthreads();
     constexpr int PER = kPartRecs / kPartThreads;
-    uint32_t rec[PER], rank[PER];
-    uint32_t bin_of[PER];
+    constexpr uint32_t kRankBits = 14, kNoRec = 0xFFFFFFFFu;
+    static_assert(kPartRecs <= (1u << kRankBits) && commit::kMaxBins <= (1u << (32 - kRankBits - 1)), "bin and rank share a word");
+    uint32_t rec[PER], slot[PER];
 #pragma unroll
     for (int q = 0; q < PER; ++q) {
         const uint32_t i = (uint32_t)q * kPartThreads + tid;
-        bin_of[q] = 0xFFFFFFFFu;
+        slot[q] = kNoRec;
         if (i < nr) {
             const uint32_t id = ids[r0 + i];
-            const unsigned long long v = votes[r0 + i];
-            bin_of[q] = id >> kPartSpanBits;
-            if (bin_of[q] >= n_bins) { bin_of[q] = 0xFFFFFFFFu; continue; }
-            rec[q] = (id & (kPartSpan - 1)) | ((uint32_t)v & 0xFFu) << 13 | ((uint32_t)(v >> 32) & 0xFFu) << 21;
-            rank[q] = atomicAdd(&s_cnt[bin_of[q]], 1u);
+            uint32_t v0, v1;
+            if (V16) {
+                const uint32_t v = reinterpret_cast<const uint16_t *>(votes_in)[r0 + i];
+                v0 = v & 0xFFu;
+                v1 = v >> 8;
+            } else {
+                const unsigned long long v = reinterpret_cast<const unsigned long long *>(votes_in)[r0 + i];
+                v0 = (uint32_t)v & 0xFFu;
+                v1 = (uint32_t)(v >> 32) & 0xFFu;
+            }
+            const uint32_t bin = id >> kPartSpanBits;
+            if (bin >= n_bins) continue;
+            rec[q] = (id & (kPartSpan - 1)) | v0 << 13 | v1 << 21;
+            slot[q] = bin << kRankBits | atomicAdd(&s_cnt[bin], 1u);
         }
     }
     __syncthreads();
     {
-        uint32_t c[4], sum = 0;
+        uint32_t c[4], g[4], sum = 0;
 #pragma unroll
         for (int q = 0; q < 4; ++q) {
             const uint32_t b = tid * 4 + q;
             c[q] = b < n_bins ? s_cnt[b] : 0;
             sum += c[q];
         }
+#pragma unroll
+        for (int q = 0; q < 4; ++q) g[q] = c[q] ? atomicAdd(&bin_lines[(size_t)(tid * 4 + q) * kPartLineWords], c[q]) : 0;
         uint32_t incl = sum;
         const uint32_t lane = tid & 63;
         for (int off = 1; off < 64; off <<= 1) {
@@ -724,10 +741,9 @@
                 base += c[q];
                 uint32_t dst = 0;
                 if (c[q]) {
-                    const uint32_t g = atomicAdd(&bin_fill[b], c[q]);
-                    if (g + c[q] <= cap) dst = g;
+                    if (g[q] + c[q] <= cap) dst = g[q];
                     else {
-                        atomicMin(&bin_valid[b], g);
+                        atomicMin(&bin_lines[(size_t)b * kPartLineWords + 1], g[q]);
                         dst = 0x80000000u | (uint32_t)atomicAdd(over_n, (unsigned long long)c[q]);
                     }
                 }
@@ -738,7 +754,7 @@
     __syncthreads();
 #pragma unroll
     for (int q = 0; q < PER; ++q)
-        if (bin_of[q] != 0xFFFFFFFFu) s_rec[s_off[bin_of[q]] + rank[q]] = rec[q] | 0u;
+        if (slot[q] != kNoRec) s_rec[s_off[slot[q] >> kRankBits] + (slot[q] & ((1u << kRankBits) - 1))] = rec[q];
     __syncthreads();
     const uint32_t grp = tid >> 4, gl = tid & 15;
     for (uint32_t b = grp; b < n_bins; b += kPartThreads / 16) {
@@ -759,102 +775,126 @@
     }
 }
 
-constexpr int kBinThreads = 1024;
-__global__ void __launch_bounds__(kBinThreads) k_commit_bins(const uint32_t *bin_recs, const uint32_t *bin_fill, const uint32_t *bin_valid, uint32_t cap,
+constexpr int kBinThreads = 1024, kBinBatch = 8, kBinCounters = 4;
+__global__ void __launch_bounds__(kBinThreads) k_commit_bins(const uint32_t *__restrict__ bin_recs, uint32_t *bin_lines, unsigned long long *over_n_next, uint32_t cap,
                                                      uint32_t span_bits, unsigned long long *counts, size_t n_barcodes) {
     extern __shared__ __align__(16) unsigned char smem[];
     const uint32_t kPartSpanBits = span_bits, kPartSpan = 1u << span_bits;
     unsigned long long *s_vote = reinterpret_cast<unsigned long long *>(smem);
     uint32_t *s_neg = reinterpret_cast<uint32_t *>(s_vote + kPartSpan);
     const uint32_t b = blockIdx.x, tid = threadIdx.x;
-    const uint32_t fill = bin_fill[b], valid = bin_valid[b];
+    uint32_t *line = bin_lines + (size_t)b * kPartLineWords;
+    const uint32_t fill = line[0], valid = line[1];
     const uint32_t n = fill < valid ? (fill < cap ? fill : cap) : valid;
-    if (n == 0) return;
     for (uint32_t j = tid; j < kPartSpan; j += kBinThreads) {
         s_vote[j] = 0;
         s_neg[j] = 0;
     }
     __syncthreads();
+    if (tid == 0) {
+        line[0] = 0;
+        line[1] = 0xFFFFFFFFu;
+        if (b == 0) *over_n_next = 0;
+    }
+    if (n == 0) return;
     const uint32_t *recs = bin_recs + (size_t)b * cap;
-    for (uint32_t i = tid; i < n; i += kBinThreads) {
-        const uint32_t r = recs[i];
-        const uint32_t id = r & (kPartSpan - 1), v0 = (r >> 13) & 0xFFu, v1 = (r >> 21) & 0xFFu;
-        if (v0 | v1) atomicAdd(&s_vote[id], (unsigned long long)v0 | ((unsigned long long)v1 << 32));
-        else atomicAdd(&s_neg[id], 1u);
+    constexpr uint32_t kNoRec = 0xFFFFFFFFu;
+    for (uint32_t i0 = 0; i0 < n; i0 += kBinBatch * kBinThreads) {
+        uint32_t r[kBinBatch];
+#pragma unroll
+        for (int u = 0; u < kBinBatch; ++u) {
+            const uint32_t i = i0 + (uint32_t)u * kBinThreads + tid;
+            r[u] = i < n ? recs[i] : kNoRec;
+        }
+#pragma unroll
+        for (int u = 0; u < kBinBatch; ++u) {
+            if (r[u] == kNoRec) continue;
+            const uint32_t id = r[u] & (kPartSpan - 1), v0 = (r[u] >> 13) & 0xFFu, v1 = (r[u] >> 21) & 0xFFu;
+            if (v0 | v1) atomicAdd(&s_vote[id], (unsigned long long)v0 | ((unsigned long long)v1 << 32));
+            else atomicAdd(&s_neg[id], 1u);
+        }
     }
     __syncthreads();
     const size_t first = (size_t)b << kPartSpanBits;
-    for (uint32_t j = tid; j < kPartSpan && first + j < n_barcodes; j += kBinThreads) {
-        const unsigned long long v = s_vote[j];
-        const uint32_t g = s_neg[j];
-        if (v | g) {
-            unsigned long long *rec = counts + 4 * (first + j);
-            if (v) {
-                ulonglong2 c = *reinterpret_cast<ulonglong2 *>(rec);
-                c.x += (uint32_t)v;
-                c.y += v >> 32;
-                *reinterpret_cast<ulonglong2 *>(rec) = c;
-            }
-            if (g) rec[2] += g;
-        }
-    }
-}
-
-static uint32_t part_span_bits(size_t n_barcodes) {
-    uint32_t lg = 0;
-    while (((size_t)1 << lg) < n_barcodes) ++lg;
-    const uint32_t want = lg > 10 ? lg - 10 : 0;
-    return want < 8 ? 8u : (want > kPartMaxSpanBits ? kPartMaxSpanBits : want);
-}
-size_t commit_partition_scratch_bytes(size_t n_reads, size_t n_barcodes, uint32_t *n_bins_out, uint32_t *cap_out) {
-    const uint32_t sb = part_span_bits(n_barcodes);
-    const uint32_t n_bins = (uint32_t)((n_barcodes + ((size_t)1 << sb) - 1) >> sb);
-    const uint64_t mean = n_bins ? (n_reads + n_bins - 1) / n_bins : 0;
-    const uint32_t cap = (uint32_t)std::min<uint64_t>(0x7FFFFFFFull, mean + mean / 2 + 2048);
-    if (n_bins_out) *n_bins_out = n_bins;
-    if (cap_out) *cap_out = cap;
-    return 256 + (size_t)n_bins * 8 + 256 + (size_t)n_bins * cap * 4 + 256 + n_reads * 4 + 256 + n_reads * 8;
-}
-bool commit_partition_usable(size_t n_reads, size_t n_barcodes, uint32_t max_votes, bool forced) {
-    uint32_t n_bins, cap;
-    (void)commit_partition_scratch_bytes(n_reads, n_barcodes, &n_bins, &cap);
-    if (max_votes > 255 || n_bins < 1 || n_bins > kPartMaxBins || n_reads < 1 || n_reads >= (1ull << 31)) return false;
-    if ((uint64_t)cap * 255u >= (1ull << 32)) return false;
-    return forced || (n_bins >= 128 && n_reads >= (1u << 21));
-}
-hipError_t launch_commit_partitioned(const uint32_t *d_votes, const uint32_t *d_barcode_ids, unsigned long long *d_counts, size_t n_barcodes, size_t n_reads,
-                                     void *d_scratch, hipStream_t s) {
-    uint32_t n_bins, cap;
-    (void)commit_partition_scratch_bytes(n_reads, n_barcodes, &n_bins, &cap);
-    const uint32_t sb = part_span_bits(n_barcodes);
-    unsigned char *p = reinterpret_cast<unsigned char *>(d_scratch);
-    unsigned long long *over_n = reinterpret_cast<unsigned long long *>(p);
-    uint32_t *bin_fill = reinterpret_cast<uint32_t *>(p + 256);
-    uint32_t *bin_valid = bin_fill + n_bins;
-    size_t at = 256 + (size_t)n_bins * 8;
-    at = (at + 255) & ~(size_t)255;
-    uint32_t *bin_recs = reinterpret_cast<uint32_t *>(p + at);
-    at += (size_t)n_bins * cap * 4;
-    at = (at + 255) & ~(size_t)255;
-    uint32_t *over_ids = reinterpret_cast<uint32_t *>(p + at);
-    at += n_reads * 4;
-    at = (at + 255) & ~(size_t)255;
-    unsigned long long *over_votes = reinterpret_cast<unsigned long long *>(p + at);
-    hipError_t e = hipMemsetAsync(p, 0, 256 + (size_t)n_bins * 4, s);
+    for (uint32_t j0 = 0; j0 < kPartSpan; j0 += kBinCounters * kBinThreads) {
+        unsigned long long v[kBinCounters], neg[kBinCounters];
+        uint32_t g[kBinCounters];
+        ulonglong2 c[kBinCounters];
+#pragma unroll
+        for (int u = 0; u < kBinCounters; ++u) {
+            const uint32_t j = j0 + (uint32_t)u * kBinThreads + tid;
+            const bool in = j < kPartSpan && first + j < n_barcodes;
+            v[u] = in ? s_vote[j] : 0;
+            g[u] = in ? s_neg[j] : 0;
+            const unsigned long long *rec = counts + 4 * (first + j);
+            if (v[u]) c[u] = *reinterpret_cast<const ulonglong2 *>(rec);
+            if (g[u]) neg[u] = rec[2];
+        }
+#pragma unroll
+        for (int u = 0; u < kBinCounters; ++u) {
+            unsigned long long *rec = counts + 4 * (first + j0 + (uint32_t)u * kBinThreads + tid);
+            if (v[u]) {
+                c[u].x += (uint32_t)v[u];
+                c[u].y += v[u] >> 32;
+                *reinterpret_cast<ulonglong2 *>(rec) = c[u];
+            }
+            if (g[u]) rec[2] = neg[u] + g[u];
+        }
+    }
+}
+__global__ void __launch_bounds__(256) k_commit_scratch_init(uint32_t *bin_lines, uint32_t n_bins, unsigned long long *over_n) {
+    const uint32_t b = blockIdx.x * 256 + threadIdx.x;
+    if (b < n_bins) {
+        bin_lines[(size_t)b * kPartLineWords] = 0;
+        bin_lines[(size_t)b * kPartLineWords + 1] = 0xFFFFFFFFu;
+    }
+    if (b < 2) over_n[b] = 0;
+}
+
+static hipError_t commit_lds_attributes() {
+    static std::atomic<uint64_t> done{0};
+    int dev = 0;
+    hipError_t e = hipGetDevice(&dev);
     if (e != hipSuccess) return e;
-    e = hipMemsetAsync(bin_valid, 0xFF, (size_t)n_bins * 4, s);
+    const uint64_t bit = 1ull << (dev & 63);
+    if (done.load(std::memory_order_acquire) & bit) return hipSuccess;
+    e = hipFuncSetAttribute(reinterpret_cast<const void *>(k_commit_partition<false>), hipFuncAttributeMaxDynamicSharedMemorySize, (int)commit::kMaxLdsPartition);
     if (e != hipSuccess) return e;
-    const size_t lds1 = (size_t)n_bins * 12 + (size_t)kPartRecs * 4, lds2 = ((size_t)12 << sb);
-    e = hipFuncSetAttribute(reinterpret_cast<const void *>(k_commit_partition), hipFuncAttributeMaxDynamicSharedMemorySize, (int)lds1);
+    e = hipFuncSetAttribute(reinterpret_cast<const void *>(k_commit_partition<true>), hipFuncAttributeMaxDynamicSharedMemorySize, (int)commit::kMaxLdsPartition);
     if (e != hipSuccess) return e;
-    e = hipFuncSetAttribute(reinterpret_cast<const void *>(k_commit_bins), hipFuncAttributeMaxDynamicSharedMemorySize, (int)lds2);
+    e = hipFuncSetAttribute(reinterpret_cast<const void *>(k_commit_bins), hipFuncAttributeMaxDynamicSharedMemorySize, (int)commit::kMaxLdsBins);
     if (e != hipSuccess) return e;
-    hipLaunchKernelGGL(k_commit_partition, dim3((unsigned)((n_reads + kPartRecs - 1) / kPartRecs)), dim3(kPartThreads), lds1, s,
-                       reinterpret_cast<const unsigned long long *>(d_votes), d_barcode_ids, n_reads, n_bins, sb, cap, bin_fill, bin_valid, bin_recs,
-                       over_n, over_ids, over_votes);
-    hipLaunchKernelGGL(k_commit_bins, dim3(n_bins), dim3(kBinThreads), lds2, s, bin_recs, bin_fill, bin_valid, cap, sb, d_counts, n_barcodes);
+    done.fetch_or(bit, std::memory_order_release);
+    return hipSuccess;
+}
+hipError_t launch_commit_partitioned(const void *d_votes, bool votes16, const uint32_t *d_barcode_ids, unsigned long long *d_counts, size_t n_barcodes,
+                                     size_t n_reads, const commit::Plan &pl, CommitScratch &sc, hipStream_t s) {
+    unsigned char *p = reinterpret_cast<unsigned char *>(sc.d);
+    unsigned long long *over_n = reinterpret_cast<unsigned long long *>(p + pl.over_n_at);
+    uint32_t *bin_lines = reinterpret_cast<uint32_t *>(p + pl.lines_at);
+    uint32_t *bin_recs = reinterpret_cast<uint32_t *>(p + pl.recs_at);
+    uint32_t *over_ids = reinterpret_cast<uint32_t *>(p + pl.over_ids_at);
+    unsigned long long *over_votes = reinterpret_cast<unsigned long long *>(p + pl.over_votes_at);
+    hipError_t e = commit_lds_attributes();
+    if (e != hipSuccess) return e;
+    if (sc.n_bins != pl.n_bins || sc.cap != pl.cap) {
+        hipLaunchKernelGGL(k_commit_scratch_init, dim3((pl.n_bins + 255) / 256), dim3(256), 0, s, bin_lines, pl.n_bins, over_n);
+        sc.n_bins = pl.n_bins;
+        sc.cap = pl.cap;
+        sc.parity = 0;
+    }
+    unsigned long long *over_now = over_n + sc.parity, *over_next = over_n + (sc.parity ^ 1u);
+    sc.parity ^= 1u;
+    const dim3 grid1((unsigned)((n_reads + kPartRecs - 1) / kPartRecs));
+    if (votes16)
+        hipLaunchKernelGGL(k_commit_partition<true>, grid1, dim3(kPartThreads), pl.lds_partition, s, d_votes, d_barcode_ids, n_reads, pl.n_bins, pl.span_bits,
+                           pl.cap, bin_lines, bin_recs, over_now, over_ids, over_votes);
+    else
+        hipLaunchKernelGGL(k_commit_partition<false>, grid1, dim3(kPartThreads), pl.lds_partition, s, d_votes, d_barcode_ids, n_reads, pl.n_bins, pl.span_bits,
+                           pl.cap, bin_lines, bin_recs, over_now, over_ids, over_votes);
+    hipLaunchKernelGGL(k_commit_bins, dim3(pl.n_bins), dim3(kBinThreads), pl.lds_bins, s, bin_recs, bin_lines, over_next, pl.cap, pl.span_bits, d_counts, n_barcodes);
     hipLaunchKernelGGL(k_commit_votes, dim3((unsigned)((n_reads + kCommitSpan - 1) / kCommitSpan)), dim3(256), 0, s,
-                       reinterpret_cast<const uint32_t *>(over_votes), over_ids, d_counts, (uint32_t *)nullptr, (size_t)0, over_n);
+                       reinterpret_cast<const uint32_t *>(over_votes), over_ids, d_counts, (uint32_t *)nullptr, (size_t)0, over_now);
     return hipGetLastError();
 }
 
```

After: 391.4 billion bp/s (median of 6 runs). 2.2% higher.
